# prannaykaul/lvc

Measured on AMD Instinct MI355X. Metric: img/s COCO 800x1333 R50-FPN inference (GeneralizedRCNN.forward(batched_inputs) -> Instances, 1000 proposals, 100 detections), higher is better.
Workload: dtype f32 (conv/GEMM inner products on the fp16 / bf16 matrix cores through fp32-accurate operand splits: two-way fp16 with main + cross fp32 accumulators for the 3x3 and wide 1x1 / FC layers, three-way bf16 for the rest; final boxes/scores closer to the fp64 evaluation than the reference's fp32 CPU path,; 1 GPU; COCO-detection R50-FPN inference, bs=8 synthetic 3x800x1333 per GPU, 1000 pre/post-NMS proposals per level/image, 80 classes, conditioned random-init weights; batch_per_gpu=8, global_batch=8, parallelism=dp1

## Files before the change

### include/lvc_amd.h

```cpp
#ifndef LVC_AMD_H
#define LVC_AMD_H

#ifdef __cplusplus
extern "C" {
#endif

#define LVC_OK 0
#define LVC_ERR_INVALID 1
#define LVC_ERR_HIP 2

int lvc_abi_version(void);
const char* lvc_last_error(void);
void lvc_set_error(const char* fmt, ...);

long long lvc_conv_workspace_bytes(void);
long long lvc_conv_range_words_offset(void);
void lvc_set_range_slot(int slot);
int lvc_range_slot(void);
int lvc_range_slots(void);
int lvc_conv2d_nhwc_f32(const float* x, const float* w_packed, const float* scale, const float* shift,
                        const float* residual, float* y, int N, int H, int W, int C, int K, int R, int S,
                        int stride, int pad, int Kg, int relu, int res_mode, int ldy, int ldr, int mode,
                        void* workspace, void* stream);

// ... 40 lines not shown
int lvc_conv1x1_nhwc_f16x2_pipe(const float* x, const unsigned short* w_split, const float* scale, const float* shift,
                                const float* residual, float* y, int N, int H, int W, int C, int K, int stride, int relu,
                                int res_mode, int ldy, int ldr, void* workspace, void* stream);
int lvc_conv1x1_nhwc_f16s1(const float* x, const unsigned short* w_split, const float* scale, const float* shift,
                           const float* residual, float* y, int N, int H, int W, int C, int K, int stride, int relu,
                           int res_mode, int ldy, int ldr, void* workspace, void* stream);
int lvc_conv3x3_nhwc_f16s1_presplit(const float* x, const unsigned short* w_split, const float* scale, const float* shift, void* y,
                                    int N, int H, int W, int C, int K, int Kg, int next_slot, void* workspace, void* stream);
int lvc_conv1x1_nhwc_f16s1_presplit(const void* x, const unsigned short* w_split, const float* scale, const float* shift,
                                    const float* residual, float* y, int N, int H, int W, int C, int K, int relu,
                                    int res_mode, int ldy, int ldr, void* workspace, void* stream);
int lvc_conv1x1_nhwc_f16s1_w2(const float* x, const unsigned short* w_split, const float* scale, const float* shift,
                              const float* residual, float* y, int N, int H, int W, int C, int K, int Kpad, int stride, int relu,
                              int res_mode, int ldy, int ldr, void* workspace, void* stream);
int lvc_conv1x1_chain_nhwc_f16s1(const float* x, int ldx, const unsigned short* wa, int wa_rows, const float* sa, const float* ta,
                                 const float* residual, int ldr, float* y1, int ldy1, int relu1, const unsigned short* wb,
                                 int wb_rows, const float* sb, const float* tb, float* y2, int ldy2, int relu2, int M, int K1,
                                 int N1, int N2, void* workspace, void* stream);
int lvc_bottleneck_nhwc_f16s1(const float* x, int ldx, float* y, int ldy, int N, int H, int W, int cin, int proj,
                              const unsigned short* w, const float* s1, const float* t1, const float* s2, const float* t2,
                              const float* s3, const float* t3, void* workspace, void* stream);
int lvc_split_weights_rowscaled(const float* wp, int rows, int Kg, void* planes_out, float* row_factor, void* stream);

int lvc_conv2d_nhwc_f16x2(const float* x, const unsigned short* w_split, const float* scale, const float* shift,
                          const float* residual, float* y, int N, int H, int W, int C, int K, int R, int S,
                          int stride, int pad, int Kg, int relu, int res_mode, int ldy, int ldr, void* workspace,
                          void* stream);
int lvc_conv2d_nhwc_f16x2_dma(const float* x, const unsigned short* w_split, const float* scale, const float* shift,
                          const float* residual, float* y, int N, int H, int W, int C, int K, int R, int S,
                          int stride, int pad, int Kg, int relu, int res_mode, int ldy, int ldr, void* workspace,
                          void* stream);

int lvc_stem_conv_pool_nhwc4_f16x2(const float* x, const unsigned short* w_split, const float* scale, const float* shift,
                                   float* y, int N, int H, int W, int Kpad, int relu, int* d_error_word,
                                   float* y2 , int ldy2, void* stream);

int lvc_preprocess_nhwc4(const void* image, int dtype, int h, int w, const float* mean3, const float* std3,
                         float* out, int Hp, int Wp, void* stream);
int lvc_preprocess_batch_nhwc4(const void* const* images, int dtype, const int* hs, const int* ws, int B, const float* mean3,
                               const float* std3, float* out, int Hp, int Wp, void* stream);

int lvc_resize_bilinear_u8(const unsigned char* image, int H, int W, int new_h, int new_w, const int* xb, const int* xk,
                           int kxs, const int* yb, const int* yk, int kys, unsigned char* tmp, unsigned char* out_u8,
                           float* out_nhwc4, int Hp, int Wp, const float* mean3, const float* std3, void* stream);
int lvc_tta_resize_u8(const unsigned char* image, int H, int W, long long sy, long long sx, long long sc, const long long* hjobs,
                      int n_h, const long long* vjobs, int n_v, const float* mean3, const float* std3, void* stream);
long long lvc_tta_merge_workspace_bytes(int B, int Nmax);
int lvc_tta_merge(const float* boxes, const float* scores, const int* classes, const int* counts, int topk_in, const float* params,
                  const int* tab, int B, int Nmax, float score_thresh, double nms_thresh, int topk_out, float* ob, float* osc, int* ocl,
                  int* ocount, void* workspace, long long workspace_bytes, void* stream);
int lvc_train_input_u8(const void* h_blob, const void* d_blob, long long blob_bytes, int B, unsigned char* tmp, long long tmp_bytes,
                       float* out, int n_slots, int Hp, int Wp, const float* mean3, const float* std3, int* launches, void* stream);
int lvc_train_input_tiles_u8(const void* h_blob, const void* d_blob, long long blob_bytes, int B, unsigned char* tmp,
                             long long tmp_bytes, float* out, int n_slots, int Hp, int Wp, const float* mean3, const float* std3,
                             int* launches, void* stream);
int lvc_train_input_lsj_u8(const void* h_blob, const void* d_blob, long long blob_bytes, int B, unsigned char* tmp,
                           long long tmp_bytes, float* out, int n_slots, int Hp, int Wp, const float* mean3, const float* std3,
                           int* launches, void* stream);
int lvc_color_jitter_tiles_u8(const void* h_blob, void* d_blob, long long blob_bytes, int B, unsigned char* out, long long out_bytes,
                              int* launches, void* stream);
int lvc_maxpool2d_nhwc(const float* x, float* y, int N, int H, int W, int C, int k, int stride, int pad,
                       void* stream);

int lvc_crop_resize_nearest(const float* image_chw, int C, int H, int W, const int* d_windows, int K, int out_size,
                            float* out, void* stream);

int lvc_rownorm(const float* x, const float* mu, float* y, int M, int D, int ldx, int ldy, float eps, int mode,
                void* stream);
int lvc_rownorm_backward(const float* x, const float* dy, float* dx, int M, int D, float eps, int accumulate, void* stream);

int lvc_roi_align_forward_nchw(const float* input, const float* rois, float* output, int B, int C, int H, int W,
                               int K, int pooled_h, int pooled_w, float spatial_scale, int sampling_ratio,
                               int aligned, int* d_status, void* stream);
int lvc_roi_align_fpn_nhwc(const float* const* feats, const int* Hs, const int* Ws, const float* scales, int L,
                           int B, int C, const float* rois, const int* levels, const int* d_num_valid, int K,
                           int pooled_h, int pooled_w, int sampling_ratio, int aligned, float* output,
                           int* d_status, void* stream);
int lvc_roi_work_order(const float* rois, const int* levels, const float* scales, int L, int K, int pooled_h, int* d_order,
                       void* stream);
int lvc_roi_work_order_xcd(const float* rois, const int* levels, int K, int B, int* d_order, void* stream);
int lvc_roi_align_fpn_nhwc_ordered(const float* const* feats, const int* Hs, const int* Ws, const float* scales, int L,
                                   int B, int C, const float* rois, const int* levels, const int* d_num_valid, int K,
                                   int pooled_h, int pooled_w, int sampling_ratio, int aligned, float* output,
                                   int* d_status, const int* d_order, void* stream);

int lvc_roi_align_backward_nchw(const float* grad, const float* rois, float* grad_input, int B, int C, int H, int W,
                                int K, int pooled_h, int pooled_w, float spatial_scale, int sampling_ratio,
                                int aligned, int* d_status, void* stream);
int lvc_roi_align_fpn_backward_nhwc(const float* grad, float* const* grad_feats, const int* Hs, const int* Ws,
                                    const float* scales, int L, int B, int C, const float* rois, const int* levels,
                                    const int* d_num_valid, int K, int pooled_h, int pooled_w, int sampling_ratio,
                                    int aligned, int* d_status, void* stream);
int lvc_roi_align_route(int backward, int nhwc, int C, int pooled_h, int pooled_w, int has_num_valid,
                        long long largest_level_elems);

long long lvc_batched_nms_workspace_bytes(int B, int Nmax);
int lvc_batched_nms(const float* boxes, const float* scores, const int* idxs, const int* d_counts, int B,
                    int Nmax, double iou_threshold, int max_keep, int* keep, int* d_num_keep, void* workspace,
                    long long workspace_bytes, void* stream);

long long lvc_rpn_proposals_workspace_bytes(int B, int L, int A, const int* Hs, const int* Ws, int pre_nms_topk);
int lvc_rpn_proposals(const float* const* logits, const int* ld_logit, const float* const* deltas,
                      const int* ld_delta, const float* const* cell_anchors, const int* Hs, const int* Ws,
                      const int* strides, int L, int A, int B, const int* d_image_sizes, int pre_nms_topk,
                      int post_nms_topk, double nms_thresh, float min_box_size, float scale_clamp,
                      float* out_boxes, float* out_logits, int* d_out_count, void* workspace,
                      long long workspace_bytes, void* stream);

long long lvc_retinanet_select_workspace_bytes(int B, int L, int A, int K, const int* Hs, const int* Ws, int topk,
                                               int max_survivors);
int lvc_retinanet_select(const float* const* logits, const int* ld_logit, const float* const* deltas, const int* ld_delta,
                         const float* const* cell_anchors, const int* Hs, const int* Ws, const int* strides,
                         float anchor_offset, int L, int A, int K, int B, int topk, float score_thresh, float wx, float wy,
                         float ww, float wh, float scale_clamp, int max_survivors, float* out_boxes, float* out_scores,
                         int* out_classes, int* out_index, int* d_count, int* d_status, void* workspace,
                         long long workspace_bytes, void* stream);

int lvc_gather_detections(const float* boxes, const float* scores, const int* classes, const int* rows, const int* keep,
                          const int* d_num_keep, int B, int Nmax, int topk, const float* d_post, float* out_boxes,
                          float* out_scores, int* out_classes, int* out_rows, int* d_out_count, void* stream);

long long lvc_retinanet_loss_workspace_bytes(int B, int L, int A, int K, const int* Hs, const int* Ws);
int lvc_retinanet_loss(const float* const* logits, const int* ld_logit, const float* const* deltas, const int* ld_delta,
                       const int* Hs, const int* Ws, int L, int A, int K, int B, const float* anchors, const int* matches,
                       const signed char* labels, const float* gt, const long long* gt_classes, const int* gt_off, double alpha,
                       double gamma, double beta, double wx, double wy, double ww, double wh, double momentum,
                       double one_minus_momentum, const double* normalizer_in, double* normalizer_out, float* out_losses,
                       double* out_sums , int* num_pos, void* workspace, long long workspace_bytes, void* stream);
int lvc_retinanet_loss_grad(const float* const* logits, const int* ld_logit, const float* const* deltas, const int* ld_delta,
                            const int* Hs, const int* Ws, int L, int A, int K, int B, const float* anchors, const int* matches,
                            const signed char* labels, const float* gt, const long long* gt_classes, const int* gt_off, double alpha,
                            double gamma, double beta, double wx, double wy, double ww, double wh, const double* normalizer,
                            const float* g_cls, const float* g_box, float* const* dlogits, const int* ld_dlogit,
                            float* const* ddeltas, const int* ld_ddelta, void* stream);

int lvc_assign_levels_rois(const float* boxes, int B, int R, int min_level, int max_level, int canonical_box_size,
                           int canonical_level, int* levels, float* rois, void* stream);

long long lvc_fast_rcnn_inference_workspace_bytes(int B, int max_candidates);
int lvc_fast_rcnn_inference(const float* cls_logits, int ld_cls, const float* deltas, int ld_delta, int K,
                            int cls_agnostic, const float* proposals, const int* d_prop_count, int B, int R,
                            const int* d_image_sizes, float wx, float wy, float ww, float wh, float scale_clamp,
                            float score_thresh, double nms_thresh, int topk, int max_candidates,
                            const float* d_post, float* out_boxes, float* out_scores, int* out_classes,
                            int* out_rows, int* d_out_count, int* d_status, void* workspace,
                            long long workspace_bytes, void* stream);

int lvc_decode_boxes(const float* deltas, int ld, const float* boxes, int M, int R, const int* d_image_sizes,
                     float wx, float wy, float ww, float wh, float scale_clamp, float* out, void* stream);

int lvc_match_boxes(const float* gt, int G, const float* boxes, int N, float t0, float t1, int nthr, int l0, int l1,
                    int l2, int allow_low_quality, long long* matches, signed char* labels, float* matched_vals,
                    unsigned int* d_gt_best, void* stream);
int lvc_match_boxes_batched(const float* gt, const int* gt_off, int Gtot, int B, const float* boxes, long long box_img_stride,
                            const int* nbox, int N, float t0, float t1, int nthr, int l0, int l1, int l2, int allow_low_quality,
                            int* matches, signed char* labels, float* vals, unsigned int* gt_best, void* stream);
long long lvc_subsample_workspace_bytes(int B);
int lvc_subsample_batched(const signed char* labels, const long long* keys , unsigned long long seed,
                          int B, int N, int nbits, int cap_pos, int bs, int* sel, int* counts, void* workspace, void* stream);
int lvc_rpn_gather_sampled(const void* const* fused, const int* ld, const void* const* cell_anchors, const int* H, const int* W,
                           const int* strides, int L, int A, int B, int bs, const int* sel, const int* counts, const int* matches,
                           const float* gt, const int* gt_off, float* logits, float* deltas, float* anchors, float* gt_boxes,
                           signed char* labels, void* stream);
int lvc_roi_build_table(const float* pboxes, const float* plogits, const int* pcount, int B, int P, const float* gt, const int* gt_off,
                        float gt_logit, int Wt, float* boxes, float* logits, int* nrow, void* stream);
int lvc_roi_gather_sampled(const float* boxes, const float* logits, const int* matches, const int* sel, const int* counts,
                           const long long* gt_classes, const int* gt_off, int B, int Wt, int bs, int K, float* s_boxes, float* s_logits,
                           long long* s_cls, long long* s_match, void* stream);
int lvc_fast_rcnn_losses(const float* logits, int ld_cls, const float* deltas, int ld_delta, int K, int cls_agnostic,
                         const float* proposals, const float* gt_boxes, const long long* gt_classes, int R, float wx,
                         float wy, float ww, float wh, float smooth_l1_beta, float* out_losses, float* dlogits,
                         float* ddeltas, double* row_terms , void* stream);
int lvc_rpn_losses(const float* logits, const float* deltas, const float* anchors, const float* gt_boxes,
                   const signed char* labels, int S, float smooth_l1_beta, float normalizer, float* out_losses,
                   void* stream);
int lvc_rpn_losses_grad(const float* logits, const float* deltas, const float* anchors, const float* gt_boxes,
                        const signed char* labels, int S, float smooth_l1_beta, float normalizer, float* out_losses,
                        float* dlogits, float* ddeltas, void* stream);

int lvc_giou_box_loss(const float* deltas, int ld_delta, const float* proposals, const float* gt_boxes,
                      const long long* gt_classes, int R, int K, float wx, float wy, float ww, float wh,
                      float scale_clamp, int iterate, float lambda, float* out_loss, float* ddeltas, void* stream);
int lvc_relu_backward(const float* dy, const float* y, long long n, float* out, void* stream);
int lvc_colsum(const float* x, int M, int N, int ldx, float* out, void* stream);

int lvc_pack_conv_weights(const float* w, const float* scale, float* wp, int K, int C, int R, int S, int rows_pad,
                          int cin_pad, int mode, void* stream);
int lvc_split_weights(const float* wp, long long n, int planes, void* out, int* err_word, void* stream);
int lvc_pack_split_conv_weights(const float* w, const float* scale, float* wp, void* planes_out, int planes, int* err_word,
                                int K, int C, int R, int S, int rows_pad, int cin_pad, int mode, void* stream);
int lvc_pack_group(int njobs, const void* const* ptrs, const int* shapes, int* err_word, void* stream);
int lvc_conv_wgrad_nhwc(const float* x, const float* dy, const float* scale, float* dw, int N, int H, int W, int C,
                        int K, int R, int S, int stride, int pad, int lddy, void* stream);
int lvc_conv_wgrad_nhwc_bf16x3(const float* x, const float* dy, const float* scale, float* dw, int N, int H, int W, int C,
                               int K, int R, int S, int stride, int pad, int lddy, void* stream);
int lvc_conv_wgrad_nhwc_f16x2(const float* x, const float* dy, const float* scale, float* dw, int N, int H, int W, int C,
                              int K, int R, int S, int stride, int pad, int lddy, int* err_word, void* stream);
int lvc_conv_wgrad_group_bf16x3(int njobs, const float* const* x, const float* const* dy, const float* const* scale,
                                float* const* dw, const int* shapes, void* stream);
int lvc_wgrad_finalize_group(int njobs, const float* const* src, float* const* dst, const int* shapes, void* stream);
int lvc_scatter_stride2_nhwc(const float* x, float* y, int N, int H, int W, int C, void* stream);
int lvc_conv3x3_grouped_nhwc(const float* x, const float* wp, const float* scale, const float* shift, const float* residual,
                             float* y, int N, int H, int W, int C, int K, int groups, int stride, int relu, int res_mode, int ldy,
                             int ldr, void* workspace, void* stream);
long long lvc_conv3x3_grouped_packed_floats(int K, int groups);
int lvc_pack_conv3x3_grouped(const float* w, const float* scale, float* wp, int K, int groups, int mode, void* stream);
long long lvc_conv3x3_grouped_wgrad_workspace_bytes(int N, int H, int W, int K, int groups, int stride);
int lvc_conv3x3_grouped_wgrad_nhwc(const float* x, const float* dy, const float* scale, float* dw, int N, int H, int W, int C,
                                   int groups, int stride, int lddy, void* scratch, void* stream);
int lvc_subsample2_nhwc(const float* x, float* y, int N, int H, int W, int C, int ldy, void* stream);
int lvc_downsum2x2_nhwc(const float* x, float* y, int N, int Hs, int Ws, int C, void* stream);
int lvc_avgpool2_nhwc(const float* x, float* y, int N, int H, int W, int C, int ldo, void* stream);
int lvc_avgpool2_bwd_nhwc(const float* dy, float* dx, int N, int H, int W, int C, int ldi, void* stream);
int lvc_colsum_atomic(const float* x, int M, int N, int ldx, float* out, void* stream);

int lvc_colmean(const float* x, float* mu, int M, int D, int ld, void* stream);
int lvc_knn_topk_candidates(const float* sims, int ld, int Q, int S, int idx_base, float* cand_val, int* cand_idx, void* stream);
int lvc_knn_merge_vote(const float* cand_val, const int* cand_idx, int nlists, int Q, const long long* shot_classes,
                       const long long* det_classes, int kvote, long long* top_classes, long long* keep, void* stream);
int lvc_max_f32(const float* x, long long n, float* out, void* stream);
int lvc_knn_topk_vote(const float* sims, int ld, int Q, int S, const long long* shot_classes,
                      const long long* det_classes, int kvote, long long* top_classes, long long* keep,
                      void* stream);
int lvc_rownorm_h(const float* x, const float* mu, float* y, unsigned short* yh, float* den, float* resid, int M, int D, int ldx,
                  float eps, int mode, void* stream);
int lvc_gemm_f16(const unsigned short* a, const unsigned short* b, int ldb, float* y, int M, int N, int C, int ldy,
                 void* stream);
int lvc_knn_verify_topk_vote(const float* approx, int ld, int Q, int S, const float* q, int ldq, const float* mu,
                             const float* den, const float* sn, int D, float margin, const float* margins,
// ... 87 lines not shown
```

### lvc_amd/csrc/boxes.hip

```cpp
#include "common.h"
#include "select_common.h"
#include <stdlib.h>


#define MAXL 8


__device__ __forceinline__ int block_excl_scan_1024(int v, int* sh, int* total) {
  const int lane = threadIdx.x & 63, wave = threadIdx.x >> 6;
  int x = v;
#pragma unroll
  for (int o = 1; o < 64; o <<= 1) {
    int t = __shfl_up(x, o);
    if (lane >= o) x += t;
  }
  __syncthreads();
  if (lane == 63) sh[wave] = x;
  __syncthreads();
  if (threadIdx.x == 0) {
    int s = 0;
    for (int w = 0; w < 16; ++w) { int t = sh[w]; sh[w] = s; s += t; }
    sh[16] = s;
  }
  __syncthreads();
  *total = sh[16];
  return sh[wave] + x - v;
}


struct RpnLevels {
  const float* logits[MAXL];
  const float* deltas[MAXL];
  int ld_logit[MAXL], ld_delta[MAXL];
  int H[MAXL], W[MAXL], stride[MAXL];
  int cand_off[MAXL + 1];
  long long key_off[MAXL + 1];
  const float* cell_anchors[MAXL];
  int L, A;
};


#define TOPK_PAD 2048
__global__ __launch_bounds__(1024) void rpn_topk_kernel(RpnLevels lv, int topk, unsigned int* __restrict__ wkeys,
                                                        float* __restrict__ cand_score,
                                                        int* __restrict__ cand_idx, int Ntot, int small_only) {
  __shared__ u64 sortbuf[TOPK_PAD];
  __shared__ int hist[256];
  __shared__ int sh[20];
  __shared__ int s_nlt;
  const int l = blockIdx.x, b = blockIdx.y, tid = threadIdx.x;
  const int A = lv.A, HW = lv.H[l] * lv.W[l], n = HW * A;
  if (n > small_only) return;
  const int k = topk < n ? topk : n;
  const int ld = lv.ld_logit[l];
  const float* lg = lv.logits[l] + (size_t)b * HW * ld;
  unsigned int* keys = wkeys + (size_t)b * lv.key_off[lv.L] + lv.key_off[l];
  const int npad = k <= 1024 ? 1024 : TOPK_PAD;

  if (tid < 256) hist[tid] = 0;
  __syncthreads();
  for (int i = tid; i < n; i += 1024) {
    int p = i / A, a = i - p * A;
    unsigned int key = desc_key(lg[(size_t)p * ld + a]);
    keys[i] = key;
    atomicAdd(&hist[key >> 24], 1);
  }
  __syncthreads();
  unsigned int prefix = 0, pmask = 0;
  int krem = k;
  for (int pass = 0; pass < 4; ++pass) {
    const int shift = 24 - 8 * pass;
    if (pass > 0) {
      if (tid < 256) hist[tid] = 0;
      __syncthreads();
      for (int i = tid; i < n; i += 1024) {
        unsigned int key = keys[i];
        if ((key & pmask) == prefix) atomicAdd(&hist[(key >> shift) & 255], 1);
      }
      __syncthreads();
    }
    find_digit(hist, krem, sh);
    prefix |= (unsigned int)sh[8] << shift;
    pmask |= 255u << shift;
    krem -= sh[9];
// ... 550 lines not shown
  LVC_CHECK_ARG(L >= 1 && L <= MAXL, "1..8 levels");
  LVC_CHECK_ARG(B > 0 && A > 0, "bad B/A");
  LVC_CHECK_ARG(pre_nms_topk > 0 && pre_nms_topk <= TOPK_PAD, "pre_nms_topk must be in 1..2048");
  LVC_CHECK_ARG(post_nms_topk > 0, "post_nms_topk must be positive");
  LVC_CHECK_ARG(logits && deltas && cell_anchors && Hs && Ws && strides && d_image_sizes && out_boxes &&
                    out_logits && d_out_count && workspace, "null pointer");
  RpnPlan p = rpn_plan(B, L, A, Hs, Ws, pre_nms_topk);
  LVC_CHECK_ARG(workspace_bytes >= p.total, "workspace too small");
  RpnLevels lv;
  memset(&lv, 0, sizeof lv);
  lv.L = L; lv.A = A;
  for (int l = 0; l < L; ++l) {
    lv.logits[l] = logits[l]; lv.deltas[l] = deltas[l];
    lv.ld_logit[l] = ld_logit[l]; lv.ld_delta[l] = ld_delta[l];
    lv.H[l] = Hs[l]; lv.W[l] = Ws[l]; lv.stride[l] = strides[l];
    lv.cell_anchors[l] = cell_anchors[l];
    long long n = (long long)Hs[l] * Ws[l] * A;
    lv.key_off[l + 1] = lv.key_off[l] + n;
    lv.cand_off[l + 1] = lv.cand_off[l] + (int)(n < pre_nms_topk ? n : pre_nms_topk);
  }
  char* ws = (char*)workspace;
  hipStream_t st = (hipStream_t)stream;
  unsigned int* keys = (unsigned int*)(ws + p.off_keys);
  float* cand_score = (float*)(ws + p.off_cscore);
  int* cand_idx = (int*)(ws + p.off_cidx);
  const bool multi = p.max_slices > 0;
  const int sel = lvc_select_onelaunch();
  if ((sel & 1) && (sel & 4)) {
    hipLaunchKernelGGL(rpn_topk_one_kernel, dim3(L, B), dim3(1024), 0, st, lv, pre_nms_topk, keys, cand_score, cand_idx,
                       p.Ntot, (const int*)nullptr);
  } else if (sel & 1) {
    int* hist12 = (int*)(ws + p.off_hist12);
    if (hipMemsetAsync(hist12, 0, (size_t)B * L * 4096 * 4, st) != hipSuccess) {
      lvc_set_error("%s: hipMemsetAsync failed", __func__);
      return LVC_ERR_HIP;
    }
    if (p.all_slices > 0)
      hipLaunchKernelGGL(rpn_topk_keys_kernel, dim3(p.all_slices, L, B), dim3(1024), 0, st, lv, keys, hist12);
    hipLaunchKernelGGL(rpn_topk_one_kernel, dim3(L, B), dim3(1024), 0, st, lv, pre_nms_topk, keys, cand_score, cand_idx,
                       p.Ntot, (const int*)hist12);
  } else {
  if (multi) {
    int* hist = (int*)(ws + p.off_hist);
    u64* ckeys = (u64*)(ws + p.off_ckeys);
    int* ties = (int*)(ws + p.off_ties);
    if (hipMemsetAsync(hist, 0, (size_t)B * L * TK_HSTRIDE * 4, st) != hipSuccess) {
      lvc_set_error("%s: hipMemsetAsync failed", __func__);
      return LVC_ERR_HIP;
    }
    for (int phase = 0; phase <= 4; ++phase)
      hipLaunchKernelGGL(rpn_topk_phase_kernel, dim3(p.max_slices, L, B), dim3(1024), 0, st, lv, pre_nms_topk, keys,
                         hist, ckeys, ties, p.Ntot, phase);
    hipLaunchKernelGGL(rpn_topk_final_kernel, dim3(L, B), dim3(1024), 0, st, lv, pre_nms_topk, keys, hist, ckeys, ties,
                       cand_score, cand_idx, p.Ntot);
  }
  hipLaunchKernelGGL(rpn_topk_kernel, dim3(L, B), dim3(1024), 0, st, lv, pre_nms_topk, keys, cand_score,
                     cand_idx, p.Ntot, multi ? TK_SLICE : 0x7FFFFFFF);
  }
  LVC_CHECK_LAUNCH();
  float* sboxes = (float*)(ws + p.off_sboxes);
  float* sscores = (float*)(ws + p.off_sscores);
  int* scount = (int*)(ws + p.off_scount);
  int* skeep = (int*)(ws + p.off_skeep);
  int* snk = (int*)(ws + p.off_snk);
  hipLaunchKernelGGL(rpn_decode_seg_kernel, dim3(L, B), dim3(1024), 0, st, lv, cand_score, cand_idx, p.Ntot,
                     d_image_sizes, scale_clamp, min_box_size, p.SN, sboxes, sscores, scount);
  LVC_CHECK_LAUNCH();
  const int keep_per_level = post_nms_topk < p.SN ? post_nms_topk : p.SN;
  int rc = lvc_batched_nms(sboxes, sscores, nullptr, scount, B * L, p.SN, nms_thresh, keep_per_level, skeep, snk,
                           ws + p.off_snms, p.snms_bytes, stream);
  if (rc) return rc;
  hipLaunchKernelGGL(rpn_merge_levels_kernel, dim3(B), dim3(1024), 0, st, sboxes, sscores, skeep, snk, L, p.SN,
                     post_nms_topk, out_boxes, out_logits, d_out_count);
  LVC_CHECK_LAUNCH();
  return LVC_OK;
}

__global__ void assign_levels_kernel(const float* __restrict__ boxes, int R, int B, int min_level, int max_level,
                                     float canonical_box_size, float canonical_level, int* __restrict__ levels,
                                     float* __restrict__ rois) {
  const int i = blockIdx.x * blockDim.x + threadIdx.x;
  if (i >= R * B) return;
  const float4 bx = *reinterpret_cast<const float4*>(boxes + (size_t)i * 4);
  const float area = (bx.z - bx.x) * (bx.w - bx.y);
  const float size = sqrtf(area);
  float lvl = floorf(canonical_level + log2f(size / canonical_box_size + 1e-8f));
  lvl = lvl < (float)min_level ? (float)min_level : lvl;
  lvl = lvl > (float)max_level ? (float)max_level : lvl;
  levels[i] = (int)lvl - min_level;
  if (rois) {
    float* r = rois + (size_t)i * 5;
    r[0] = (float)(i / R); r[1] = bx.x; r[2] = bx.y; r[3] = bx.z; r[4] = bx.w;
  }
}

extern "C" int lvc_assign_levels_rois(const float* boxes, int B, int R, int min_level, int max_level,
                                      int canonical_box_size, int canonical_level, int* levels, float* rois,
                                      void* stream) {
  LVC_CHECK_ARG(B >= 0 && R >= 0, "negative size");
  if (B * R == 0) return LVC_OK;
  LVC_CHECK_ARG(boxes && levels, "null pointer");
  hipLaunchKernelGGL(assign_levels_kernel, dim3(lvc_cdiv(B * R, 256)), dim3(256), 0, (hipStream_t)stream, boxes, R,
                     B, min_level, max_level, (float)canonical_box_size, (float)canonical_level, levels, rois);
  LVC_CHECK_LAUNCH();
  return LVC_OK;
}

#define DET_TILE_ROWS 64
#define DET_MAX_COLS 97
__global__ __launch_bounds__(DET_TILE_ROWS) void det_row_stats_kernel(const float* __restrict__ cls_logits, int ld_cls, int K,
                                                                     int rows, float score_thresh, float* __restrict__ st_mx,
                                                                     float* __restrict__ st_inv, int* __restrict__ st_cnt,
                                                                     unsigned long long* __restrict__ st_mask) {
  __shared__ float tile[DET_TILE_ROWS * DET_MAX_COLS];
  const int r0 = blockIdx.x * DET_TILE_ROWS, tid = threadIdx.x;
  const int ncol = K + 1, pitch = ncol | 1;
  for (int i = tid; i < DET_TILE_ROWS * ncol; i += DET_TILE_ROWS) {
    const int rr = i / ncol, cc = i - rr * ncol;
    const int r = r0 + rr;
    tile[rr * pitch + cc] = r < rows ? cls_logits[(size_t)r * ld_cls + cc] : 0.f;
  }
  __syncthreads();
  const int r = r0 + tid;
  if (r >= rows) return;
  const float* lg = tile + tid * pitch;
  float mx = -INFINITY;
  for (int k = 0; k <= K; ++k) { float v = lg[k]; mx = v > mx ? v : mx; }
  float sum = 0.f;
  for (int k = 0; k <= K; ++k) sum += expf(lg[k] - mx);
  const float inv = 1.f / sum;
  int cnt = 0;
  unsigned long long m0 = 0, m1 = 0;
  for (int k = 0; k < K; ++k) {
    const bool hit = expf(lg[k] - mx) * inv > score_thresh;
    cnt += hit ? 1 : 0;
    if (hit) { if (k < 64) m0 |= 1ull << k; else m1 |= 1ull << (k - 64); }
  }
  st_mx[r] = mx; st_inv[r] = inv; st_cnt[r] = cnt;
  st_mask[2 * (size_t)r] = m0; st_mask[2 * (size_t)r + 1] = m1;
}

__global__ __launch_bounds__(1024) void det_candidates_kernel(
    const float* __restrict__ cls_logits, int ld_cls, const float* __restrict__ deltas, int ld_delta,
    int K, int cls_agnostic, const float* __restrict__ proposals, const int* __restrict__ prop_count, int R,
    const int* __restrict__ image_sizes, float wx, float wy, float ww, float wh, float scale_clamp,
    float score_thresh, int Nmax, float* __restrict__ cboxes, float* __restrict__ cscores,
    int* __restrict__ cclass, int* __restrict__ crow, int* __restrict__ ccount, int* __restrict__ status,
    const float* __restrict__ st_mx, const float* __restrict__ st_inv, const int* __restrict__ st_cnt,
    const unsigned long long* __restrict__ st_mask) {
  __shared__ int sh[20];
  const int b = blockIdx.x, tid = threadIdx.x;
  const int nrow = prop_count ? min(prop_count[b], R) : R;
  const float img_h = (float)image_sizes[b * 2 + 0], img_w = (float)image_sizes[b * 2 + 1];
  int base = 0;
  for (int r0 = 0; r0 < nrow; r0 += 1024) {
    const int r = r0 + tid;
    int cnt = 0;
    float mx = -INFINITY, inv = 0.f;
    const float* lg = cls_logits + ((size_t)b * R + (r < nrow ? r : 0)) * ld_cls;
    if (r < nrow && st_cnt) {
      const size_t gr = (size_t)b * R + r;
      mx = st_mx[gr]; inv = st_inv[gr]; cnt = st_cnt[gr];
    } else if (r < nrow) {
      for (int k = 0; k <= K; ++k) { float v = lg[k]; mx = v > mx ? v : mx; }
      float sum = 0.f;
      for (int k = 0; k <= K; ++k) sum += expf(lg[k] - mx);
      inv = 1.f / sum;
      for (int k = 0; k < K; ++k) cnt += (expf(lg[k] - mx) * inv > score_thresh) ? 1 : 0;
    }
    int tot;
    int pos = base + block_excl_scan_1024(cnt, sh, &tot);
    if (r < nrow && cnt > 0) {
      const float4 pb = *reinterpret_cast<const float4*>(proposals + ((size_t)b * R + r) * 4);
      const float* dl = deltas + ((size_t)b * R + r) * ld_delta;
      auto emit = [&](int k) {
        const float pr = expf(lg[k] - mx) * inv;
        if (pr > score_thresh) {
          if (pos < Nmax) {
            const float* d = dl + (cls_agnostic ? 0 : k * 4);
            float box[4];
            apply_deltas(pb.x, pb.y, pb.z, pb.w, d[0], d[1], d[2], d[3], wx, wy, ww, wh, scale_clamp, box);
            float* o = cboxes + ((size_t)b * Nmax + pos) * 4;
            o[0] = clampf(box[0], 0.f, img_w); o[1] = clampf(box[1], 0.f, img_h);
            o[2] = clampf(box[2], 0.f, img_w); o[3] = clampf(box[3], 0.f, img_h);
            cscores[(size_t)b * Nmax + pos] = pr;
            cclass[(size_t)b * Nmax + pos] = k;
            crow[(size_t)b * Nmax + pos] = r;
          }
          ++pos;
        }
      };
      if (st_mask) {
        for (int w = 0; w < 2; ++w) {
          unsigned long long m = st_mask[2 * ((size_t)b * R + r) + w];
          while (m) {
            emit(w * 64 + __ffsll((long long)m) - 1);
            m &= m - 1;
          }
        }
      } else {
        for (int k = 0; k < K; ++k) emit(k);
      }
    }
    base += tot;
  }
  if (tid == 0) {
    if (base > Nmax) { atomicOr(status, 2); base = Nmax; }
    ccount[b] = base;
  }
}

__global__ __launch_bounds__(256) void det_gather_kernel(
    const float* __restrict__ cboxes, const float* __restrict__ cscores, const int* __restrict__ cclass,
    const int* __restrict__ crow, const int* __restrict__ keep, const int* __restrict__ num_keep, int Nmax,
    int topk, const float* __restrict__ post, float* __restrict__ oboxes, float* __restrict__ oscores,
    int* __restrict__ oclasses, int* __restrict__ orows, int* __restrict__ ocount) {
  __shared__ int wsum[4];
  const int b = blockIdx.x, tid = threadIdx.x;
  const int nk = min(num_keep[b], topk);
  int base = 0;
  for (int r0 = 0; r0 < topk; r0 += 256) {
    const int r = r0 + tid;
    bool ok = false;
    float4 bx = {0, 0, 0, 0};
    float s = 0.f; int c = 0, row = 0;
    if (r < nk) {
      const int i = keep[(size_t)b * Nmax + r];
      bx = *reinterpret_cast<const float4*>(cboxes + ((size_t)b * Nmax + i) * 4);
      s = cscores[(size_t)b * Nmax + i]; c = cclass[(size_t)b * Nmax + i]; row = crow[(size_t)b * Nmax + i];
      ok = true;
      if (post) {
        const float sx = post[b * 4 + 0], sy = post[b * 4 + 1], oh = post[b * 4 + 2], ow = post[b * 4 + 3];
        bx.x = clampf(bx.x * sx, 0.f, ow); bx.y = clampf(bx.y * sy, 0.f, oh);
        bx.z = clampf(bx.z * sx, 0.f, ow); bx.w = clampf(bx.w * sy, 0.f, oh);
        ok = (bx.z - bx.x > 0.f) && (bx.w - bx.y > 0.f);
      }
    }
    const u64 bal = __ballot(ok);
    const int lane = tid & 63, wave = tid >> 6;
    __syncthreads();
    if (lane == 0) wsum[wave] = __popcll(bal);
    __syncthreads();
    int wbase = 0, tot = 0;
    for (int w = 0; w < 4; ++w) { if (w < wave) wbase += wsum[w]; tot += wsum[w]; }
    const int pos = base + wbase + __popcll(bal & ((1ull << lane) - 1ull));
    if (ok) {
      *reinterpret_cast<float4*>(oboxes + ((size_t)b * topk + pos) * 4) = bx;
      oscores[(size_t)b * topk + pos] = s; oclasses[(size_t)b * topk + pos] = c; orows[(size_t)b * topk + pos] = row;
    }
    base += tot;
  }
  __syncthreads();
  for (int r = base + tid; r < topk; r += 256) {
    float4 z = {0, 0, 0, 0};
    *reinterpret_cast<float4*>(oboxes + ((size_t)b * topk + r) * 4) = z;
    oscores[(size_t)b * topk + r] = 0.f; oclasses[(size_t)b * topk + r] = 0; orows[(size_t)b * topk + r] = 0;
  }
  if (tid == 0) ocount[b] = base;
}

struct DetPlan { long long off_cboxes, off_cscores, off_cclass, off_crow, off_ccount, off_keep, off_nk, off_nms, total; };
static DetPlan det_plan(int B, int Nmax) {
  DetPlan p; long long o = 0;
  p.off_cboxes = o; o = align16(o + (long long)B * Nmax * 16);
  p.off_cscores = o; o = align16(o + (long long)B * Nmax * 4);
  p.off_cclass = o; o = align16(o + (long long)B * Nmax * 4);
  p.off_crow = o; o = align16(o + (long long)B * Nmax * 4);
  p.off_ccount = o; o = align16(o + (long long)B * 4);
  p.off_keep = o; o = align16(o + (long long)B * Nmax * 4);
  p.off_nk = o; o = align16(o + (long long)B * 4);
  p.off_nms = o; o = align16(o + lvc_batched_nms_workspace_bytes(B, Nmax));
  p.total = o;
  return p;
}
extern "C" long long lvc_fast_rcnn_inference_workspace_bytes(int B, int max_candidates) {
  return det_plan(B, max_candidates).total;
}

extern "C" int lvc_fast_rcnn_inference(const float* cls_logits, int ld_cls, const float* deltas, int ld_delta,
                                       int K, int cls_agnostic, const float* proposals,
                                       const int* d_prop_count, int B, int R, const int* d_image_sizes,
                                       float wx, float wy, float ww, float wh, float scale_clamp,
                                       float score_thresh, double nms_thresh, int topk, int max_candidates,
                                       const float* d_post, float* out_boxes, float* out_scores,
                                       int* out_classes, int* out_rows, int* d_out_count, int* d_status,
                                       void* workspace, long long workspace_bytes, void* stream) {
  LVC_CHECK_ARG(B > 0 && R > 0 && K > 0 && topk > 0, "bad sizes");
  LVC_CHECK_ARG(max_candidates > 0, "max_candidates must be positive");
  LVC_CHECK_ARG(cls_logits && deltas && proposals && d_image_sizes && out_boxes && out_scores && out_classes &&
                    out_rows && d_out_count && d_status && workspace, "null pointer");
  DetPlan p = det_plan(B, max_candidates);
  LVC_CHECK_ARG(workspace_bytes >= p.total, "workspace too small");
  char* ws = (char*)workspace;
  hipStream_t st = (hipStream_t)stream;
  float* cboxes = (float*)(ws + p.off_cboxes);
  float* cscores = (float*)(ws + p.off_cscores);
  int* cclass = (int*)(ws + p.off_cclass);
  int* crow = (int*)(ws + p.off_crow);
  int* ccount = (int*)(ws + p.off_ccount);
  int* keep = (int*)(ws + p.off_keep);
  int* nk = (int*)(ws + p.off_nk);
  const long long rows = (long long)B * R;
  float* st_mx = nullptr; float* st_inv = nullptr; int* st_cnt = nullptr;
  unsigned long long* st_mask = nullptr;
  if (K + 1 < DET_MAX_COLS && rows * 28 + 64 <= p.total - p.off_nms) {
    st_mask = (unsigned long long*)(ws + p.off_nms);
    st_mx = (float*)(st_mask + 2 * rows);
    st_inv = st_mx + rows;
    st_cnt = (int*)(st_inv + rows);
    hipLaunchKernelGGL(det_row_stats_kernel, dim3((unsigned)lvc_cdiv64(rows, DET_TILE_ROWS)), dim3(DET_TILE_ROWS), 0, st,
                       cls_logits, ld_cls, K, (int)rows, score_thresh, st_mx, st_inv, st_cnt, st_mask);
    LVC_CHECK_LAUNCH();
  }
  hipLaunchKernelGGL(det_candidates_kernel, dim3(B), dim3(1024), 0, st, cls_logits, ld_cls, deltas, ld_delta, K,
                     cls_agnostic, proposals, d_prop_count, R, d_image_sizes, wx, wy, ww, wh, scale_clamp,
                     score_thresh, max_candidates, cboxes, cscores, cclass, crow, ccount, d_status, st_mx, st_inv, st_cnt, st_mask);
  LVC_CHECK_LAUNCH();
  int rc = lvc_batched_nms(cboxes, cscores, cclass, ccount, B, max_candidates, nms_thresh, topk, keep, nk,
                           ws + p.off_nms, p.total - p.off_nms, stream);
  if (rc) return rc;
  hipLaunchKernelGGL(det_gather_kernel, dim3(B), dim3(256), 0, st, cboxes, cscores, cclass, crow, keep, nk,
                     max_candidates, topk, d_post, out_boxes, out_scores, out_classes, out_rows, d_out_count);
  LVC_CHECK_LAUNCH();
  return LVC_OK;
}

extern "C" int lvc_gather_detections(const float* boxes, const float* scores, const int* classes, const int* rows,
                                     const int* keep, const int* d_num_keep, int B, int Nmax, int topk, const float* d_post,
                                     float* out_boxes, float* out_scores, int* out_classes, int* out_rows, int* d_out_count,
                                     void* stream) {
  LVC_CHECK_ARG(B > 0 && Nmax > 0 && topk > 0, "bad B / Nmax / topk");
  LVC_CHECK_ARG(boxes && scores && classes && rows && keep && d_num_keep && out_boxes && out_scores && out_classes && out_rows &&
                    d_out_count, "null pointer");
  LVC_CHECK_ARG(((uintptr_t)boxes & 15) == 0 && ((uintptr_t)out_boxes & 15) == 0, "box pointers must be 16-byte aligned");
  hipLaunchKernelGGL(det_gather_kernel, dim3(B), dim3(256), 0, (hipStream_t)stream, boxes, scores, classes, rows, keep,
                     d_num_keep, Nmax, topk, d_post, out_boxes, out_scores, out_classes, out_rows, d_out_count);
  LVC_CHECK_LAUNCH();
  return LVC_OK;
}

__global__ void decode_boxes_kernel(const float* __restrict__ deltas, int ld, const float* __restrict__ boxes, int M,
                                    int R, const int* __restrict__ image_sizes, float wx, float wy, float ww, float wh,
                                    float scale_clamp, float* __restrict__ out) {
  const int i = blockIdx.x * blockDim.x + threadIdx.x;
  if (i >= M) return;
  const float4 b = *reinterpret_cast<const float4*>(boxes + (size_t)i * 4);
  const float* d = deltas + (size_t)i * ld;
  float o[4];
  apply_deltas(b.x, b.y, b.z, b.w, d[0], d[1], d[2], d[3], wx, wy, ww, wh, scale_clamp, o);
  if (image_sizes) {
    const int img = i / R;
    const float h = (float)image_sizes[img * 2], w = (float)image_sizes[img * 2 + 1];
    o[0] = clampf(o[0], 0.f, w); o[1] = clampf(o[1], 0.f, h); o[2] = clampf(o[2], 0.f, w); o[3] = clampf(o[3], 0.f, h);
  }
  float4 r = {o[0], o[1], o[2], o[3]};
  *reinterpret_cast<float4*>(out + (size_t)i * 4) = r;
}

extern "C" int lvc_decode_boxes(const float* deltas, int ld, const float* boxes, int M, int R, const int* d_image_sizes,
                                float wx, float wy, float ww, float wh, float scale_clamp, float* out, void* stream) {
  LVC_CHECK_ARG(M >= 0 && R > 0 && ld >= 4, "bad shape");
  if (M == 0) return LVC_OK;
  LVC_CHECK_ARG(deltas && boxes && out, "null pointer");
  hipLaunchKernelGGL(decode_boxes_kernel, dim3(lvc_cdiv(M, 256)), dim3(256), 0, (hipStream_t)stream, deltas, ld, boxes, M, R,
                     d_image_sizes, wx, wy, ww, wh, scale_clamp, out);
  LVC_CHECK_LAUNCH();
  return LVC_OK;
}
```

### lvc_amd/csrc/conv_common.h

```cpp
#pragma once
#include "common.h"

typedef float f32x16 __attribute__((ext_vector_type(16)));
typedef float f32x4 __attribute__((ext_vector_type(4)));
typedef _Float16 f16;
typedef _Float16 f16x8 __attribute__((ext_vector_type(8)));
typedef _Float16 f16x4 __attribute__((ext_vector_type(4)));
typedef __bf16 bf16x8 __attribute__((ext_vector_type(8)));
typedef __bf16 bf16x4 __attribute__((ext_vector_type(4)));
typedef unsigned u32x4 __attribute__((ext_vector_type(4)));
typedef __attribute__((address_space(3))) void* lds_ptr_t;
typedef const __attribute__((address_space(1))) void* glb_ptr_t;

#define LVC_MAX_WORKERS 1024
#define LVC_RANGE_SLOTS 1024
#define LVC_WS_PARTIAL_BYTES (256 * 128 * 4)
#define LVC_WS_FLAGS_OFFSET ((size_t)LVC_MAX_WORKERS * LVC_WS_PARTIAL_BYTES)
#define LVC_WS_RANGE_OFFSET (LVC_WS_FLAGS_OFFSET + (size_t)LVC_MAX_WORKERS * 4)
#define LVC_WS_BYTES (LVC_WS_RANGE_OFFSET + (size_t)LVC_RANGE_SLOTS * 4 + 256)
#define LVC_WS_DIAG_OFFSET ((size_t)(LVC_MAX_WORKERS / 2) * LVC_WS_PARTIAL_BYTES)
static inline int* lvc_ws_flags(void* workspace) { return (int*)((char*)workspace + LVC_WS_FLAGS_OFFSET); }
static inline int lvc_ws_range_index(int slot) { return LVC_MAX_WORKERS + slot; }

extern "C" int lvc_cu_count(void);

static inline void lvc_plan_workers(long long units, int cap, int min_units, int* units_per_worker, int* nworkers) {
  long long workers = (units + min_units - 1) / min_units;
  if (workers > cap) workers = cap;
  if (workers < 1) workers = 1;
  *units_per_worker = (int)((units + workers - 1) / workers);
  *nworkers = (int)((units + *units_per_worker - 1) / *units_per_worker);
}

#define LVC_ACT_SCALE 16.f
#define LVC_ACT_MAX 4094.f
#define LVC_F16_MAX 65504.f
#define lvc_report_range(flags, index, big, limit)                                             \
  do {                                                                                         \
    if (!((big) <= (limit))) atomicOr((flags) + (index), (big) < INFINITY ? 2 : 4);            \
  } while (0)

#define LVC_SPIN_LIMIT (1 << 24)
__device__ __forceinline__ void lvc_publish_partial(int* flags, int worker) {
  __builtin_amdgcn_fence(__ATOMIC_RELEASE, "agent");
  asm volatile("s_waitcnt vmcnt(0)" ::: "memory");
  __hip_atomic_store(flags + worker, 1, __ATOMIC_RELAXED, __HIP_MEMORY_SCOPE_AGENT);
}
__device__ __forceinline__ void lvc_wait_partial(int* flags, int worker, int err_index) {
  int spins = 0;
  while (__hip_atomic_load(flags + worker, __ATOMIC_RELAXED, __HIP_MEMORY_SCOPE_AGENT) == 0) {
    __builtin_amdgcn_s_sleep(4);
    if (++spins > LVC_SPIN_LIMIT) { atomicOr(flags + err_index, 1); break; }
  }
  __builtin_amdgcn_fence(__ATOMIC_ACQUIRE, "agent");
}
__device__ __forceinline__ void lvc_release_partial(int* flags, int worker) {
  __hip_atomic_store(flags + worker, 0, __ATOMIC_RELAXED, __HIP_MEMORY_SCOPE_AGENT);
}

__device__ __forceinline__ void glds16(const void* g, void* l) {
  __builtin_amdgcn_global_load_lds((glb_ptr_t)g, (lds_ptr_t)l, 16, 0, 0);
}
template <int N> __device__ __forceinline__ void wait_vm() { asm volatile("s_waitcnt vmcnt(%0)" ::"n"(N) : "memory"); }
template <int N> __device__ __forceinline__ void wait_vm_lds() { asm volatile("s_waitcnt vmcnt(%0) lgkmcnt(0)" ::"n"(N) : "memory"); }

__device__ __forceinline__ f32x4 load_untracked(u32x4 rsrc, unsigned voff, unsigned soff) {
  f32x4 v;
  asm volatile("buffer_load_dwordx4 %0, %1, %2, %3 offen" : "=v"(v) : "v"(voff), "s"(rsrc), "s"(soff) : "memory");
  return v;
}
template <int IMM> __device__ __forceinline__ f32x4 load_untracked(u32x4 rsrc, unsigned voff, unsigned soff) {
  f32x4 v;
  asm volatile("buffer_load_dwordx4 %0, %1, %2, %3 offen offset:%4" : "=v"(v) : "v"(voff), "s"(rsrc), "s"(soff), "n"(IMM) : "memory");
  return v;
}
template <int N> __device__ __forceinline__ void wait_tied(f32x4& a, f32x4& b) {
  asm volatile("s_waitcnt vmcnt(%2)" : "+v"(a), "+v"(b) : "n"(N) : "memory");
}
template <int N> __device__ __forceinline__ void wait_tied(f32x4& a, f32x4& b, f32x4& c, f32x4& d) {
  asm volatile("s_waitcnt vmcnt(%4)" : "+v"(a), "+v"(b), "+v"(c), "+v"(d) : "n"(N) : "memory");
}
__device__ __forceinline__ u32x4 make_rsrc(const void* base, unsigned bytes) {
  const unsigned long long b = (unsigned long long)base;
  return u32x4{(unsigned)__builtin_amdgcn_readfirstlane((unsigned)b), (unsigned)__builtin_amdgcn_readfirstlane((unsigned)(b >> 32) & 0xffffu),
               (unsigned)__builtin_amdgcn_readfirstlane(bytes), 0x00020000u};
}
__device__ __forceinline__ void store_b128(f32x4 v, __amdgpu_buffer_rsrc_t rsrc, unsigned voff) {
  __builtin_amdgcn_raw_buffer_store_b128(__builtin_bit_cast(u32x4, v), rsrc, voff, 0, 0);
}
__device__ __forceinline__ void track_abs(float& big, float a, float b) {
  asm volatile("v_max3_f32 %0, %0, |%1|, |%2|" : "+v"(big) : "v"(a), "v"(b));
}
__device__ __forceinline__ void split2h(float a, f16& h, f16& m) {
  h = (f16)a;
  m = (f16)((a - (float)h) * 2048.f);
}
```

### lvc_amd/csrc/conv_pw_s1.hip

```cpp
#include "conv_common.h"
#include <type_traits>
#include <stdlib.h>

#define PM 256
#define AROW 64
#define NJ 4
#define NT 512

struct PwArgsS {
  const float* x;
  const unsigned short* w;
  const float* scale;
  const float* shift;
  const float* res;
  float* y;
  float* partials;
  int* flags;
  int H, W, C, K, stride, Ho, Wo, M, relu, res_mode, ldy, ldr;
  int tiles_n, nk, total_units, units_per_worker, nworkers, err_index, ngroup;
  int x_bytes;
  long long w_plane_elems;
  unsigned short* planes;
  int* pl_err;
  long long pl_PS;
  int pl_N, pl_Npad, pl_H;
  float pl_qscale;
};

template <int NI, bool ONEACC, bool PLANES = false, bool PRE = false>
__global__ __launch_bounds__(NT, 2) void conv_pw_s1_kernel(PwArgsS p) {
  constexpr int HN = 64 * NI;
  constexpr int PLANE_A = PM * AROW;
  constexpr int A_BUF = 2 * PLANE_A;
  constexpr int A_BYTES = 3 * A_BUF;
  constexpr int PLANE_B = HN * 64;
  constexpr int B_BUF = 2 * PLANE_B;
  constexpr int RING_BYTES = A_BYTES + 3 * B_BUF;
  constexpr int CS_STRIDE = HN + 4;
  constexpr int CS_BYTES = PM * CS_STRIDE * 4;
  constexpr int SMEM_BYTES = RING_BYTES > CS_BYTES ? RING_BYTES : CS_BYTES;
  constexpr int RBLK = HN / 16;
  __shared__ __attribute__((aligned(1024))) unsigned char smem_raw[SMEM_BYTES];
  unsigned char* sA = smem_raw;
  unsigned char* sB = smem_raw + A_BYTES;

  const int tid = threadIdx.x;
  const int lane = tid & 63;
  const int wave = __builtin_amdgcn_readfirstlane(tid >> 6);
  const int wm = wave >> 1, wn = wave & 1;
  const int fi = lane & 31, fh = lane >> 5;
  const int q = PRE ? ((tid >> 4) & 1) * 4 + (tid & 3) : tid & 7;
  const int arid = PRE ? (tid >> 5) * 4 + ((tid >> 2) & 3) : tid >> 3;
  const int hrow = arid;

  const int lw = lvc_xcd_remap(blockIdx.x, p.nworkers);
  const int wq = p.ngroup > 1 ? lw / p.ngroup : lw;
  const int wsel = p.ngroup > 1 ? lw - wq * p.ngroup : 0;
  int u = wq * p.units_per_worker;
  const int u_end = min(u + p.units_per_worker, p.total_units);

  const unsigned long long xbase = (unsigned long long)p.x;
  const u32x4 xres = {(unsigned)__builtin_amdgcn_readfirstlane((unsigned)xbase), (unsigned)__builtin_amdgcn_readfirstlane((unsigned)(xbase >> 32) & 0xffffu),
                      (unsigned)p.x_bytes, 0x00020000u};
  const int fx3 = (fi >> 2) & 3;
  const int a_row[2] = {(wm * 64 + fi) * AROW, (wm * 64 + 32 + fi) * AROW};
  const int b_row = (wn * 32 * NI + fi) * 64;
  const int b_g[2] = {((0 + fh) ^ fx3) * 16, ((2 + fh) ^ fx3) * 16};
  int a_lds[NJ];
#pragma unroll
  for (int j = 0; j < NJ; ++j) {
    const int row = hrow + 64 * j;
    a_lds[j] = row * AROW + (((q >> 1) ^ ((row >> 2) & 3)) << 4) + (q & 1) * 8;
  }
  float big = 0.f;
  int a_pre[NJ];
#pragma unroll
  for (int j = 0; j < NJ; ++j) {
    const int row = hrow + 64 * j;
    a_pre[j] = (q >> 2) * (PM * AROW) + row * AROW + (((q & 3) ^ ((row >> 2) & 3)) << 4);
  }
#ifdef PW_TIMELINE
  unsigned long long tl_pro = 0, tl_loop = 0, tl_hand = 0, tl_cs = 0, tl_rows = 0, tl_t0 = __builtin_readcyclecounter();
  unsigned long long tl_wa = 0, tl_wv = 0, tl_wb = 0;
  unsigned tl_tiles = 0, tl_chunks = 0;
#endif

  while (u < u_end) {
#ifdef PW_TIMELINE
    const unsigned long long tl_a = __builtin_readcyclecounter();
#endif
    const int tile = u / p.nk;
    const int cc0 = u - tile * p.nk;
    const int cc1 = min(p.nk, cc0 + (u_end - u));
    const int tile_n = p.ngroup > 1 ? wsel : tile % p.tiles_n;
    const int tile_m = p.ngroup > 1 ? tile : tile / p.tiles_n;
    const int m0 = tile_m * PM;
    const int n0 = tile_n * HN;

    unsigned a_off[NJ];
#pragma unroll
    for (int j = 0; j < NJ; ++j) {
      const int m = m0 + hrow + 64 * j;
      const int n = m / (p.Ho * p.Wo);
      const int rem = m - n * (p.Ho * p.Wo);
      const int ho = rem / p.Wo, wo = rem - ho * p.Wo;
      a_off[j] = m < p.M ? (unsigned)(((n * p.H + ho * p.stride) * p.W + wo * p.stride) * p.C + q * 4) * 4u : 0x80000000u;
    }
    const unsigned short* bsrc[NI];
    int bdst[NI];
#pragma unroll
    for (int j = 0; j < NI; ++j) {
      const int idx = wave * NI + j;
// ... 357 lines not shown
      constexpr int C4 = HN / 4;
      constexpr int RPI = NT / C4;
      constexpr int NIT = PM / RPI;
      constexpr int NG = 4;
      const int c4 = tid % C4, rsub = tid / C4;
      const int col = n0 + c4 * 4;
      const bool col_ok = col < p.K;
      const bool has_res = p.res_mode != 0 && col_ok;
      auto res_load = [&](int it) {
        const int m = m0 + it * RPI + rsub;
        f32x4 v = {0.f, 0.f, 0.f, 0.f};
        if (m < p.M) {
          size_t ro = (size_t)m;
          if (p.res_mode == 2) {
            const int n = m / (p.Ho * p.Wo);
            const int rem = m - n * (p.Ho * p.Wo);
            const int ho = rem / p.Wo, wo = rem - ho * p.Wo;
            ro = ((size_t)(n * (p.Ho >> 1) + (ho >> 1)) * (p.Wo >> 1) + (wo >> 1));
          }
          v = *reinterpret_cast<const f32x4*>(p.res + ro * p.ldr + col);
        }
        return v;
      };
      f32x4 rv[NG];
#pragma unroll
      for (int i = 0; i < NG; ++i) rv[i] = f32x4{0.f, 0.f, 0.f, 0.f};
      if (has_res) {
#pragma unroll
        for (int i = 0; i < NG; ++i) rv[i] = res_load(i);
      }
      float* Cs = reinterpret_cast<float*>(smem_raw);
#pragma unroll
      for (int mi = 0; mi < 2; ++mi)
#pragma unroll
        for (int ni = 0; ni < NI; ++ni)
#pragma unroll
          for (int e = 0; e < 16; ++e) {
            const int row = wm * 64 + mi * 32 + (e & 3) + 8 * (e >> 2) + 4 * fh;
            const int colc = wn * 32 * NI + ni * 32 + fi;
            Cs[row * CS_STRIDE + colc] = acc[mi][ni][e];
          }
      __syncthreads();
#ifdef PW_TIMELINE
      tl_e = __builtin_readcyclecounter();
      tl_cs += tl_e - tl_d;
#endif
      if (col_ok) {
        f32x4 sc = {1.f, 1.f, 1.f, 1.f}, sh = {0.f, 0.f, 0.f, 0.f};
        if (p.scale) sc = *reinterpret_cast<const f32x4*>(p.scale + col);
        if (p.shift) sh = *reinterpret_cast<const f32x4*>(p.shift + col);
        const float* cs = Cs + rsub * CS_STRIDE + c4 * 4;
        float* const yb = p.y + (size_t)(m0 + rsub) * p.ldy + col;
        auto rows = [&](auto res_tag, auto act_tag) {
          constexpr bool RES = decltype(res_tag)::value;
          constexpr int ACT = decltype(act_tag)::value;
#pragma unroll 1
          for (int g = 0; g < NIT; g += NG) {
            f32x4 rn[NG];
            if (RES) {
#pragma unroll
              for (int i = 0; i < NG; ++i) rn[i] = f32x4{0.f, 0.f, 0.f, 0.f};
              if (g + NG < NIT) {
#pragma unroll
                for (int i = 0; i < NG; ++i) rn[i] = res_load(g + NG + i);
              }
            }
            f32x4 v[NG];
#pragma unroll
            for (int i = 0; i < NG; ++i) v[i] = *reinterpret_cast<const f32x4*>(cs + (g + i) * RPI * CS_STRIDE);
#pragma unroll
            for (int i = 0; i < NG; ++i) {
              const int m = m0 + (g + i) * RPI + rsub;
              if (m < p.M) {
                f32x4 o = v[i] * sc + sh;
                if (RES) o += rv[i];
                if (ACT == 1) {
                  o[0] = o[0] > 0.f ? o[0] : 0.f; o[1] = o[1] > 0.f ? o[1] : 0.f;
                  o[2] = o[2] > 0.f ? o[2] : 0.f; o[3] = o[3] > 0.f ? o[3] : 0.f;
                } else if (ACT == 2) {
#pragma unroll
                  for (int e = 0; e < 4; ++e) o[e] = o[e] * 0.5f * (1.f + erff(o[e] * 0.70710678118654752440f));
                }
                *reinterpret_cast<f32x4*>(yb + (size_t)((g + i) * RPI) * p.ldy) = o;
              }
            }
            if (RES) {
#pragma unroll
              for (int i = 0; i < NG; ++i) rv[i] = rn[i];
            }
          }
        };
        using A0 = std::integral_constant<int, 0>; using A1 = std::integral_constant<int, 1>; using A2 = std::integral_constant<int, 2>;
        if (has_res) {
          if (p.relu == 1) rows(std::true_type{}, A1{}); else if (p.relu == 2) rows(std::true_type{}, A2{}); else rows(std::true_type{}, A0{});
        } else {
          if (p.relu == 1) rows(std::false_type{}, A1{}); else if (p.relu == 2) rows(std::false_type{}, A2{}); else rows(std::false_type{}, A0{});
        }
      }
    }
    __syncthreads();
#ifdef PW_TIMELINE
    tl_rows += __builtin_readcyclecounter() - tl_e;
#endif
  }
#ifdef PW_TIMELINE
  if (lane == 0 && (blockIdx.x & 15) == 0) {
    unsigned long long* d = reinterpret_cast<unsigned long long*>(reinterpret_cast<char*>(p.partials) + LVC_WS_DIAG_OFFSET) + ((blockIdx.x >> 4) * 8 + wave) * 16;
    d[0] = tl_pro; d[1] = tl_loop; d[2] = tl_hand; d[3] = tl_cs; d[4] = tl_rows; d[5] = tl_tiles; d[6] = tl_chunks; d[7] = __builtin_readcyclecounter() - tl_t0; d[8] = 1; d[9] = tl_wa; d[10] = tl_wv; d[11] = tl_wb;
  }
#endif
  if (PRE) return;
  lvc_report_range(p.flags, p.err_index, big, ONEACC ? LVC_ACT_MAX : LVC_F16_MAX);
}

struct PwPlanes { unsigned short* planes; int* err; long long PS; int N, Npad, H; float qscale; };

static int pw_s1_launch(bool oneacc, const float* x, const unsigned short* w_split, const float* scale, const float* shift,
                        const float* residual, float* y, int N, int H, int W, int C, int K, int stride, int relu, int res_mode,
                        int ldy, int ldr, void* workspace, void* stream, const PwPlanes* pl = nullptr, bool pre = false) {
  LVC_CHECK_ARG(x && w_split && y && workspace, "null pointer");
  LVC_CHECK_ARG(!oneacc || scale, "the single-accumulator form needs the row factors in `scale`");
  LVC_CHECK_ARG(N > 0 && H > 0 && W > 0 && C > 0 && K > 0 && stride >= 1, "non-positive dimension");
  LVC_CHECK_ARG(C % 32 == 0, "needs C % 32 == 0");
  LVC_CHECK_ARG(relu >= 0 && relu <= 2, "relu: 0 none, 1 ReLU, 2 GELU");
  LVC_CHECK_ARG(res_mode >= 0 && res_mode <= 2 && (res_mode == 0 || residual), "bad residual");
  const int Ho = (H - 1) / stride + 1, Wo = (W - 1) / stride + 1;
  if (res_mode == 2) LVC_CHECK_ARG(Ho % 2 == 0 && Wo % 2 == 0, "upsample-add needs even output size");
  PwArgsS a;
  a.x = x; a.w = w_split; a.scale = scale; a.shift = shift; a.res = residual; a.y = y;
  a.H = H; a.W = W; a.C = C; a.K = K; a.stride = stride; a.Ho = Ho; a.Wo = Wo;
  const long long Mll = (long long)N * Ho * Wo;
  LVC_CHECK_ARG(Mll < (1ll << 31), "too many output pixels");
  a.M = (int)Mll; a.relu = relu; a.res_mode = res_mode;
  a.ldy = ldy > 0 ? ldy : K; a.ldr = ldr > 0 ? ldr : K;
  LVC_CHECK_ARG((K & 3) == 0 && (a.ldy & 3) == 0 && (res_mode == 0 || (a.ldr & 3) == 0), "K, ldy, ldr must be multiples of 4");
  LVC_CHECK_ARG(((uintptr_t)x & 15) == 0 && ((uintptr_t)w_split & 15) == 0 && ((uintptr_t)y & 15) == 0 && ((uintptr_t)workspace & 15) == 0 &&
                    ((uintptr_t)scale & 15) == 0 && ((uintptr_t)shift & 15) == 0 && ((uintptr_t)residual & 15) == 0,
                "pointers must be 16-byte aligned");
  const long long xb = (long long)N * H * W * C * 4;
  LVC_CHECK_ARG(xb < (1ll << 31), "input tensor must be smaller than 2 GiB");
  a.x_bytes = (int)xb;
  const int ni = K <= 64 ? 1 : 2;
  const int HN = 64 * ni;
  a.tiles_n = lvc_cdiv(K, HN);
  a.nk = C / 32;
  const int tiles_m = lvc_cdiv(a.M, PM);
  long long units = (long long)tiles_m * a.tiles_n * a.nk;
  LVC_CHECK_ARG(units < (1ll << 31), "iteration space too large");
  a.total_units = (int)units;
  a.w_plane_elems = (long long)(lvc_cdiv(K, 128) * 128) * C;
  int cap = lvc_cu_count();
  if (cap > LVC_MAX_WORKERS) cap = LVC_MAX_WORKERS;
  a.ngroup = 1;
  if ((a.tiles_n == 2 || a.tiles_n == 4 || a.tiles_n == 8 || a.tiles_n == 16) && cap % a.tiles_n == 0 && units / a.tiles_n >= (long long)(cap / a.tiles_n) * 4) {
    a.ngroup = a.tiles_n;
    units /= a.tiles_n;
    cap /= a.tiles_n;
    a.total_units = (int)units;
  }
  const int min_units = 4;
  lvc_plan_workers(units, cap, min_units, &a.units_per_worker, &a.nworkers);
  a.nworkers *= a.ngroup;
  a.partials = (float*)workspace;
  a.flags = lvc_ws_flags(workspace);
  a.err_index = lvc_ws_range_index(lvc_range_slot());
  hipStream_t st = (hipStream_t)stream;
  a.planes = nullptr; a.pl_err = nullptr; a.pl_PS = 0; a.pl_N = a.pl_Npad = a.pl_H = 0; a.pl_qscale = 1.f;
  if (pl) {
    LVC_CHECK_ARG(oneacc && ni == 2 && res_mode == 0 && relu == 0, "the planes epilogue exists for the single-accumulator 128-column tile");
    a.planes = pl->planes; a.pl_err = pl->err; a.pl_PS = pl->PS; a.pl_N = pl->N; a.pl_Npad = pl->Npad; a.pl_H = pl->H; a.pl_qscale = pl->qscale;
    hipLaunchKernelGGL((conv_pw_s1_kernel<2, true, true>), dim3(a.nworkers), dim3(NT), 0, st, a);
    LVC_CHECK_LAUNCH();
    return LVC_OK;
  }
  if (pre) {
    LVC_CHECK_ARG(oneacc && ni == 2 && stride == 1, "pre-split input: the single-accumulator 128-column tile, stride 1");
    hipLaunchKernelGGL((conv_pw_s1_kernel<2, true, false, true>), dim3(a.nworkers), dim3(NT), 0, st, a);
    LVC_CHECK_LAUNCH();
    return LVC_OK;
  }
  if (oneacc) {
    if (ni == 1) hipLaunchKernelGGL((conv_pw_s1_kernel<1, true>), dim3(a.nworkers), dim3(NT), 0, st, a);
    else hipLaunchKernelGGL((conv_pw_s1_kernel<2, true>), dim3(a.nworkers), dim3(NT), 0, st, a);
  } else {
    if (ni == 1) hipLaunchKernelGGL((conv_pw_s1_kernel<1, false>), dim3(a.nworkers), dim3(NT), 0, st, a);
    else hipLaunchKernelGGL((conv_pw_s1_kernel<2, false>), dim3(a.nworkers), dim3(NT), 0, st, a);
  }
  LVC_CHECK_LAUNCH();
  return LVC_OK;
}

extern "C" int lvc_conv1x1_nhwc_f16x2_pipe(const float* x, const unsigned short* w_split, const float* scale, const float* shift,
                                            const float* residual, float* y, int N, int H, int W, int C, int K, int stride, int relu,
                                            int res_mode, int ldy, int ldr, void* workspace, void* stream) {
  return pw_s1_launch(false, x, w_split, scale, shift, residual, y, N, H, W, C, K, stride, relu, res_mode, ldy, ldr, workspace, stream);
}

extern "C" int lvc_conv1x1_nhwc_f16s1(const float* x, const unsigned short* w_split, const float* scale, const float* shift,
                                       const float* residual, float* y, int N, int H, int W, int C, int K, int stride, int relu,
                                       int res_mode, int ldy, int ldr, void* workspace, void* stream) {
  return pw_s1_launch(true, x, w_split, scale, shift, residual, y, N, H, W, C, K, stride, relu, res_mode, ldy, ldr, workspace, stream);
}

extern "C" int lvc_conv1x1_nhwc_f16s1_presplit(const void* x, const unsigned short* w_split, const float* scale, const float* shift,
                                                const float* residual, float* y, int N, int H, int W, int C, int K, int relu,
                                                int res_mode, int ldy, int ldr, void* workspace, void* stream) {
  return pw_s1_launch(true, (const float*)x, w_split, scale, shift, residual, y, N, H, W, C, K, 1, relu, res_mode, ldy, ldr, workspace, stream, nullptr, true);
}

extern "C" int lvc_conv1x1_qkv_planes_f16s1(const float* x, const unsigned short* w_split, const float* scale, const float* shift, void* planes,
                                            int B, int N, int C, int H, float softmax_scale, int* err_word, void* workspace, void* stream) {
  LVC_CHECK_ARG(planes && B > 0 && N > 0 && H > 0, "bad arguments");
  const int Npad = (N + 127) / 128 * 128;
  PwPlanes pl;
  pl.planes = (unsigned short*)planes; pl.err = err_word; pl.N = N; pl.Npad = Npad; pl.H = H; pl.qscale = softmax_scale * 1.44269504088896340736f;
  pl.PS = (long long)B * H * Npad * 64;
  return pw_s1_launch(true, x, w_split, scale, shift, nullptr, (float*)planes, B * N, 1, 1, C, 3 * H * 64, 1, 0, 0, 0, 0, workspace, stream, &pl);
}
```

### lvc_amd/csrc/roi_align.hip

```cpp
#include "common.h"
#include <stdlib.h>
#include <type_traits>

#define LVC_MAX_LEVELS 8

struct RoiAlignArgs {
  const float* feat[LVC_MAX_LEVELS];
  int H[LVC_MAX_LEVELS], W[LVC_MAX_LEVELS];
  float scale[LVC_MAX_LEVELS];
  long long sb[LVC_MAX_LEVELS];
  long long sc, sh_mul_w;
  int nhwc;
  int C;
  const float* rois;
  const int* levels;
  const int* num_valid;
  int K, ph, pw, sampling_ratio, aligned;
  float* out;
  long long so_k, so_c, so_h, so_w;
  int* status;
  const int* order;
};

__global__ __launch_bounds__(256) void roi_align_fwd_kernel(RoiAlignArgs p) {
  const int k = blockIdx.x;
  const int c = blockIdx.y * 256 + threadIdx.x;
  const bool c_ok = c < p.C;
  float* outk = p.out + (long long)k * p.so_k + (long long)c * p.so_c;
  if (p.num_valid && k >= *p.num_valid) {
    if (c_ok)
      for (int a = 0; a < p.ph; ++a)
        for (int b = 0; b < p.pw; ++b) outk[a * p.so_h + b * p.so_w] = 0.f;
    return;
  }
  const float* r = p.rois + (long long)k * 5;
  const int lvl = p.levels ? p.levels[k] : 0;
  const int H = p.H[lvl], W = p.W[lvl];
  const float spatial_scale = p.scale[lvl];
  const int b = (int)r[0];
  const float offset = p.aligned ? 0.5f : 0.0f;
  const float roi_start_w = r[1] * spatial_scale - offset;
  const float roi_start_h = r[2] * spatial_scale - offset;
  const float roi_end_w = r[3] * spatial_scale - offset;
  const float roi_end_h = r[4] * spatial_scale - offset;
  float roi_width = roi_end_w - roi_start_w;
  float roi_height = roi_end_h - roi_start_h;
  if (p.aligned) {
    if (!(roi_width >= 0 && roi_height >= 0)) {
      if (p.status && threadIdx.x == 0 && blockIdx.y == 0) atomicOr(p.status, 1);
    }
  } else {
    roi_width = roi_width > 1.f ? roi_width : 1.f;
    roi_height = roi_height > 1.f ? roi_height : 1.f;
  }
  const float bin_h = roi_height / (float)p.ph;
  const float bin_w = roi_width / (float)p.pw;
  const int gh = p.sampling_ratio > 0 ? p.sampling_ratio : (int)ceilf(roi_height / (float)p.ph);
  const int gw = p.sampling_ratio > 0 ? p.sampling_ratio : (int)ceilf(roi_width / (float)p.pw);
  const int cnt = gh * gw > 1 ? gh * gw : 1;
  const float count = (float)cnt;

  long long s_pix, s_c;
  if (p.nhwc) { s_pix = p.C; s_c = 1; } else { s_pix = 1; s_c = (long long)H * W; }
  const float* in = p.feat[lvl] + (long long)b * p.sb[lvl] + (long long)(c_ok ? c : 0) * s_c;

  for (int ph = 0; ph < p.ph; ++ph) {
    for (int pw = 0; pw < p.pw; ++pw) {
      float acc = 0.f;
      for (int iy = 0; iy < gh; ++iy) {
        const float yy = roi_start_h + ph * bin_h + (float)(iy + .5f) * bin_h / (float)gh;
        for (int ix = 0; ix < gw; ++ix) {
          const float xx = roi_start_w + pw * bin_w + (float)(ix + .5f) * bin_w / (float)gw;
          float x = xx, y = yy;
          if (y < -1.0f || y > (float)H || x < -1.0f || x > (float)W) continue;
          if (y <= 0) y = 0;
          if (x <= 0) x = 0;
          int y_low = (int)y, x_low = (int)x, y_high, x_high;
          if (y_low >= H - 1) { y_high = y_low = H - 1; y = (float)y_low; } else y_high = y_low + 1;
          if (x_low >= W - 1) { x_high = x_low = W - 1; x = (float)x_low; } else x_high = x_low + 1;
          const float ly = y - y_low, lx = x - x_low;
          const float hy = 1.f - ly, hx = 1.f - lx;
          const float w1 = hy * hx, w2 = hy * lx, w3 = ly * hx, w4 = ly * lx;
          const float v1 = in[(long long)(y_low * W + x_low) * s_pix];
          const float v2 = in[(long long)(y_low * W + x_high) * s_pix];
          const float v3 = in[(long long)(y_high * W + x_low) * s_pix];
          const float v4 = in[(long long)(y_high * W + x_high) * s_pix];
          acc += w1 * v1 + w2 * v2 + w3 * v3 + w4 * v4;
        }
      }
      if (c_ok) outk[ph * p.so_h + pw * p.so_w] = acc / count;
    }
  }
}

__global__ __launch_bounds__(64) void roi_align_fwd_nhwc4_kernel(RoiAlignArgs p) {
  const int lane = threadIdx.x;
  const int nb = p.ph * p.pw;
  const int k = blockIdx.x / nb;
  const int bin = blockIdx.x - k * nb;
  const int ph = bin / p.pw, pw = bin - ph * p.pw;
  const int c = blockIdx.y * 256 + lane * 4;
  const bool c_ok = c < p.C;
  float* outk = p.out + (long long)k * p.so_k + c;
  const float* r = p.rois + (long long)k * 5;
  const int lvl = p.levels ? p.levels[k] : 0;
  const int H = p.H[lvl], W = p.W[lvl];
  const float spatial_scale = p.scale[lvl];
  const int b = (int)r[0];
  const float offset = p.aligned ? 0.5f : 0.0f;
  const float roi_start_w = r[1] * spatial_scale - offset;
  const float roi_start_h = r[2] * spatial_scale - offset;
  const float roi_end_w = r[3] * spatial_scale - offset;
  const float roi_end_h = r[4] * spatial_scale - offset;
  float roi_width = roi_end_w - roi_start_w;
  float roi_height = roi_end_h - roi_start_h;
  if (p.aligned) {
    if (!(roi_width >= 0 && roi_height >= 0)) {
      if (p.status && lane == 0 && blockIdx.y == 0) atomicOr(p.status, 1);
    }
  } else {
    roi_width = roi_width > 1.f ? roi_width : 1.f;
    roi_height = roi_height > 1.f ? roi_height : 1.f;
  }
  const float bin_h = roi_height / (float)p.ph;
  const float bin_w = roi_width / (float)p.pw;
  const int gh = p.sampling_ratio > 0 ? p.sampling_ratio : (int)ceilf(roi_height / (float)p.ph);
  const int gw = p.sampling_ratio > 0 ? p.sampling_ratio : (int)ceilf(roi_width / (float)p.pw);
  const int cnt = gh * gw > 1 ? gh * gw : 1;
  const float count = (float)cnt;
  const float* in = p.feat[lvl] + (long long)b * p.sb[lvl] + (c_ok ? c : 0);
  const long long C = p.C;
  {
    {
      float4 acc = {0.f, 0.f, 0.f, 0.f};
      for (int iy = 0; iy < gh; ++iy) {
        const float yy = roi_start_h + ph * bin_h + (float)(iy + .5f) * bin_h / (float)gh;
        for (int ix = 0; ix < gw; ++ix) {
          const float xx = roi_start_w + pw * bin_w + (float)(ix + .5f) * bin_w / (float)gw;
          float x = xx, y = yy;
          if (y < -1.0f || y > (float)H || x < -1.0f || x > (float)W) continue;
          if (y <= 0) y = 0;
          if (x <= 0) x = 0;
          int y_low = (int)y, x_low = (int)x, y_high, x_high;
          if (y_low >= H - 1) { y_high = y_low = H - 1; y = (float)y_low; } else y_high = y_low + 1;
          if (x_low >= W - 1) { x_high = x_low = W - 1; x = (float)x_low; } else x_high = x_low + 1;
          const float ly = y - y_low, lx = x - x_low;
          const float hy = 1.f - ly, hx = 1.f - lx;
          const float w1 = hy * hx, w2 = hy * lx, w3 = ly * hx, w4 = ly * lx;
          const float4 v1 = *reinterpret_cast<const float4*>(in + (long long)(y_low * W + x_low) * C);
          const float4 v2 = *reinterpret_cast<const float4*>(in + (long long)(y_low * W + x_high) * C);
          const float4 v3 = *reinterpret_cast<const float4*>(in + (long long)(y_high * W + x_low) * C);
          const float4 v4 = *reinterpret_cast<const float4*>(in + (long long)(y_high * W + x_high) * C);
          acc.x += w1 * v1.x + w2 * v2.x + w3 * v3.x + w4 * v4.x;
          acc.y += w1 * v1.y + w2 * v2.y + w3 * v3.y + w4 * v4.y;
          acc.z += w1 * v1.z + w2 * v2.z + w3 * v3.z + w4 * v4.z;
          acc.w += w1 * v1.w + w2 * v2.w + w3 * v3.w + w4 * v4.w;
        }
      }
      if (c_ok) {
        float4 o = {acc.x / count, acc.y / count, acc.z / count, acc.w / count};
        *reinterpret_cast<float4*>(outk + ph * p.so_h + pw * p.so_w) = o;
      }
    }
  }
}

#define ROI_UNI(x) __builtin_amdgcn_readfirstlane(x)
#ifndef ROI_RB4
#define ROI_RB4 2
#endif
#ifndef ROI_RB8
#define ROI_RB8 1
#endif
#ifndef ROI_WAVE_MLP
#define ROI_WAVE_MLP 8
#endif
template <int PW>
__global__ __launch_bounds__(512) void roi_align_fwd_nhwc_wave_kernel(RoiAlignArgs p) {
  const int lane = threadIdx.x & 63;
  const int ph = ROI_UNI((int)(threadIdx.x >> 6));
  const int k = p.order ? p.order[blockIdx.x] : (int)blockIdx.x;
  if (ph >= p.ph) return;
  const int cbase = blockIdx.y * 256;
  const float* r = p.rois + (long long)k * 5;
  const int lvl = p.levels ? p.levels[k] : 0;
  const int H = p.H[lvl], W = p.W[lvl];
  const float spatial_scale = p.scale[lvl];
  const int b = (int)r[0];
  const float offset = p.aligned ? 0.5f : 0.0f;
  const float roi_start_w = r[1] * spatial_scale - offset;
  const float roi_start_h = r[2] * spatial_scale - offset;
  const float roi_end_w = r[3] * spatial_scale - offset;
  const float roi_end_h = r[4] * spatial_scale - offset;
  float roi_width = roi_end_w - roi_start_w;
  float roi_height = roi_end_h - roi_start_h;
  if (p.aligned) {
    if (!(roi_width >= 0 && roi_height >= 0)) {
      if (p.status && lane == 0 && blockIdx.y == 0 && ph == 0) atomicOr(p.status, 1);
    }
  } else {
    roi_width = roi_width > 1.f ? roi_width : 1.f;
    roi_height = roi_height > 1.f ? roi_height : 1.f;
  }
  const float bin_h = roi_height / (float)p.ph;
  const float bin_w = roi_width / (float)p.pw;
  const int gh = ROI_UNI(p.sampling_ratio > 0 ? p.sampling_ratio : (int)ceilf(roi_height / (float)p.ph));
  const int gw = ROI_UNI(p.sampling_ratio > 0 ? p.sampling_ratio : (int)ceilf(roi_width / (float)p.pw));
  const int cnt = gh * gw > 1 ? gh * gw : 1;
  const float count = (float)cnt;
  const long long C = p.C;
  const bool c_ok = cbase + lane * 4 < p.C;
  const float* in = p.feat[lvl] + (long long)b * p.sb[lvl] + (c_ok ? cbase + lane * 4 : 0);
  float* outp = p.out + (long long)k * p.so_k + ph * p.so_h + cbase + lane * 4;

  const float yf = roi_start_h + ph * bin_h, yl = roi_start_h + (ph + 1) * bin_h;
  const int y0 = ROI_UNI(min((int)floorf(fmaxf(yf, 0.f)), H - 1)), y1 = ROI_UNI(min((int)floorf(fmaxf(yl, 0.f)) + 1, H - 1));
  const int x0 = ROI_UNI(min((int)floorf(fmaxf(roi_start_w, 0.f)), W - 1));
  const int x1 = ROI_UNI(min((int)floorf(fmaxf(roi_start_w + roi_width, 0.f)) + 1, W - 1));
  const int nrows = y1 - y0 + 1, ncols = x1 - x0 + 1;
  const bool sep = gh > 0 && gw > 0 && nrows >= 1 && nrows <= 64 && ncols >= 1 && ncols <= 64;
  if (!sep) {
    for (int pw = 0; pw < p.pw; ++pw) {
      float4 acc = {0.f, 0.f, 0.f, 0.f};
      for (int iy = 0; iy < gh; ++iy) {
        const float yy = roi_start_h + ph * bin_h + (float)(iy + .5f) * bin_h / (float)gh;
        for (int ix = 0; ix < gw; ++ix) {
          const float xx = roi_start_w + pw * bin_w + (float)(ix + .5f) * bin_w / (float)gw;
          float x = xx, y = yy;
          if (y < -1.0f || y > (float)H || x < -1.0f || x > (float)W) continue;
          if (y <= 0) y = 0;
          if (x <= 0) x = 0;
          int y_low = (int)y, x_low = (int)x, y_high, x_high;
          if (y_low >= H - 1) { y_high = y_low = H - 1; y = (float)y_low; } else y_high = y_low + 1;
          if (x_low >= W - 1) { x_high = x_low = W - 1; x = (float)x_low; } else x_high = x_low + 1;
          const float ly = y - y_low, lx = x - x_low;
          const float hy = 1.f - ly, hx = 1.f - lx;
          const float w1 = hy * hx, w2 = hy * lx, w3 = ly * hx, w4 = ly * lx;
          const float4 v1 = *reinterpret_cast<const float4*>(in + (long long)(y_low * W + x_low) * C);
          const float4 v2 = *reinterpret_cast<const float4*>(in + (long long)(y_low * W + x_high) * C);
          const float4 v3 = *reinterpret_cast<const float4*>(in + (long long)(y_high * W + x_low) * C);
          const float4 v4 = *reinterpret_cast<const float4*>(in + (long long)(y_high * W + x_high) * C);
          acc.x += w1 * v1.x + w2 * v2.x + w3 * v3.x + w4 * v4.x;
          acc.y += w1 * v1.y + w2 * v2.y + w3 * v3.y + w4 * v4.y;
          acc.z += w1 * v1.z + w2 * v2.z + w3 * v3.z + w4 * v4.z;
          acc.w += w1 * v1.w + w2 * v2.w + w3 * v3.w + w4 * v4.w;
        }
      }
      if (c_ok) *reinterpret_cast<float4*>(outp + pw * p.so_w) = float4{acc.x / count, acc.y / count, acc.z / count, acc.w / count};
    }
    return;
  }
  float wy = 0.f;
  {
    const int ymine = y0 + lane;
    for (int iy = 0; iy < gh; ++iy) {
      const float yy = roi_start_h + ph * bin_h + (float)(iy + .5f) * bin_h / (float)gh;
      if (yy < -1.0f || yy > (float)H) continue;
      float y = yy <= 0 ? 0.f : yy;
      int y_low = (int)y, y_high;
      if (y_low >= H - 1) { y_high = y_low = H - 1; y = (float)y_low; } else y_high = y_low + 1;
      const float ly = y - y_low, hy = 1.f - ly;
      wy += (y_low == ymine ? hy : 0.f) + (y_high == ymine ? ly : 0.f);
    }
  }
  float wx[PW];
#pragma unroll
  for (int pw = 0; pw < PW; ++pw) {
    const int xmine = x0 + lane;
    float a = 0.f;
    for (int ix = 0; ix < gw; ++ix) {
      const float xx = roi_start_w + pw * bin_w + (float)(ix + .5f) * bin_w / (float)gw;
      if (xx < -1.0f || xx > (float)W) continue;
      float x = xx <= 0 ? 0.f : xx;
      int x_low = (int)x, x_high;
      if (x_low >= W - 1) { x_high = x_low = W - 1; x = (float)x_low; } else x_high = x_low + 1;
      const float lx = x - x_low, hx = 1.f - lx;
      a += (x_low == xmine ? hx : 0.f) + (x_high == xmine ? lx : 0.f);
    }
    wx[pw] = a;
  }
  unsigned amask = 0;
#pragma unroll
  for (int pw = 0; pw < PW; ++pw) amask |= wx[pw] != 0.f ? 1u << pw : 0u;
  float4 acc[PW];
#pragma unroll
  for (int pw = 0; pw < PW; ++pw) acc[pw] = float4{0.f, 0.f, 0.f, 0.f};
  const float* base = in + ((long long)y0 * W + x0) * C;
  const int Ci = (int)C, rowstep = W * Ci;
  auto chunk = [&](auto cw_tag, auto rb_tag, int c0) {
    constexpr int CW = decltype(cw_tag)::value, RB = decltype(rb_tag)::value;
    const int ncw = min(CW, ncols - c0);
    float4 T[CW];
#pragma unroll
    for (int u = 0; u < CW; ++u) T[u] = float4{0.f, 0.f, 0.f, 0.f};
    for (int r0 = 0; r0 < nrows; r0 += RB) {
      float4 v[RB][CW];
#pragma unroll
      for (int rb = 0; rb < RB; ++rb)
#pragma unroll
        for (int u = 0; u < CW; ++u) {
          const bool live = u < ncw && r0 + rb < nrows;
          v[rb][u] = *reinterpret_cast<const float4*>(base + (live ? (r0 + rb) * rowstep + (c0 + u) * Ci : 0));
        }
#pragma unroll
      for (int rb = 0; rb < RB; ++rb) {
        if (r0 + rb >= nrows) continue;
        const float wyr = __uint_as_float(__builtin_amdgcn_readlane(__float_as_uint(wy), r0 + rb));
#pragma unroll
        for (int u = 0; u < CW; ++u) {
          if (u >= ncw) continue;
          T[u].x = __builtin_fmaf(wyr, v[rb][u].x, T[u].x); T[u].y = __builtin_fmaf(wyr, v[rb][u].y, T[u].y);
          T[u].z = __builtin_fmaf(wyr, v[rb][u].z, T[u].z); T[u].w = __builtin_fmaf(wyr, v[rb][u].w, T[u].w);
        }
      }
    }
#pragma unroll
    for (int u = 0; u < CW; ++u) {
      if (u >= ncw) continue;
      const unsigned am = __builtin_amdgcn_readlane(amask, c0 + u);
#pragma unroll
      for (int pw = 0; pw < PW; ++pw) {
        if (am & (1u << pw)) {
          const float w = __uint_as_float(__builtin_amdgcn_readlane(__float_as_uint(wx[pw]), c0 + u));
          acc[pw].x = __builtin_fmaf(w, T[u].x, acc[pw].x); acc[pw].y = __builtin_fmaf(w, T[u].y, acc[pw].y);
          acc[pw].z = __builtin_fmaf(w, T[u].z, acc[pw].z); acc[pw].w = __builtin_fmaf(w, T[u].w, acc[pw].w);
        }
      }
    }
  };
  if (ncols <= 4) {
    chunk(std::integral_constant<int, 4>{}, std::integral_constant<int, ROI_RB4>{}, 0);
  } else {
    for (int c0 = 0; c0 < ncols; c0 += 8) chunk(std::integral_constant<int, 8>{}, std::integral_constant<int, ROI_RB8>{}, c0);
  }
  if (c_ok) {
    const float inv = 1.f / count;
#pragma unroll
    for (int pw = 0; pw < PW; ++pw)
      *reinterpret_cast<float4*>(outp + pw * p.so_w) = float4{acc[pw].x * inv, acc[pw].y * inv, acc[pw].z * inv, acc[pw].w * inv};
  }
}

extern "C" int lvc_roi_align_route(int backward, int nhwc, int C, int pooled_h, int pooled_w, int has_num_valid,
                                   long long largest_level_elems) {
  if (backward) return nhwc && pooled_h == 7 && pooled_w == 7 ? 1 : 0;
  if (!nhwc || (C & 3) != 0 || has_num_valid) return 0;
  if (pooled_h <= 8 && pooled_w == 7 && largest_level_elems < (1ll << 31)) return 2;
  return 1;
}

static int launch(RoiAlignArgs& a, void* stream) {
  if (a.K == 0) return LVC_OK;
  long long largest = 0;
  for (int l = 0; l < LVC_MAX_LEVELS; ++l)
    if (a.feat[l] && (long long)a.H[l] * a.W[l] * a.C > largest) largest = (long long)a.H[l] * a.W[l] * a.C;
  const int route = lvc_roi_align_route(0, a.nhwc && a.so_c == 1, a.C, a.ph, a.pw, a.num_valid != nullptr, largest);
  if (route == 2) {
    hipLaunchKernelGGL(roi_align_fwd_nhwc_wave_kernel<7>, dim3(a.K, lvc_cdiv(a.C, 256)), dim3(64 * a.ph), 0, (hipStream_t)stream, a);
    LVC_CHECK_LAUNCH();
    return LVC_OK;
  }
  if (route == 1) {
    dim3 grid4(a.K * a.ph * a.pw, lvc_cdiv(a.C, 256)), block4(64);
    hipLaunchKernelGGL(roi_align_fwd_nhwc4_kernel, grid4, block4, 0, (hipStream_t)stream, a);
    LVC_CHECK_LAUNCH();
    return LVC_OK;
  }
  dim3 grid(a.K, lvc_cdiv(a.C, 256)), block(256);
  hipLaunchKernelGGL(roi_align_fwd_kernel, grid, block, 0, (hipStream_t)stream, a);
  LVC_CHECK_LAUNCH();
  return LVC_OK;
}

__global__ __launch_bounds__(256) void roi_align_bwd_kernel(RoiAlignArgs p) {
  const int k = blockIdx.x;
  const int c = blockIdx.y * 256 + threadIdx.x;
  if (p.num_valid && k >= *p.num_valid) return;
  const bool c_ok = c < p.C;
  const float* gk = p.out + (long long)k * p.so_k + (long long)(c_ok ? c : 0) * p.so_c;
  const float* r = p.rois + (long long)k * 5;
  const int lvl = p.levels ? p.levels[k] : 0;
  const int H = p.H[lvl], W = p.W[lvl];
  const float spatial_scale = p.scale[lvl];
  const int b = (int)r[0];
  const float offset = p.aligned ? 0.5f : 0.0f;
  const float roi_start_w = r[1] * spatial_scale - offset;
  const float roi_start_h = r[2] * spatial_scale - offset;
  const float roi_end_w = r[3] * spatial_scale - offset;
  const float roi_end_h = r[4] * spatial_scale - offset;
  float roi_width = roi_end_w - roi_start_w;
  float roi_height = roi_end_h - roi_start_h;
  if (p.aligned) {
    if (!(roi_width >= 0 && roi_height >= 0)) {
      if (p.status && threadIdx.x == 0 && blockIdx.y == 0) atomicOr(p.status, 1);
    }
  } else {
    roi_width = roi_width > 1.f ? roi_width : 1.f;
    roi_height = roi_height > 1.f ? roi_height : 1.f;
  }
  const float bin_h = roi_height / (float)p.ph;
  const float bin_w = roi_width / (float)p.pw;
  const int gh = p.sampling_ratio > 0 ? p.sampling_ratio : (int)ceilf(roi_height / (float)p.ph);
  const int gw = p.sampling_ratio > 0 ? p.sampling_ratio : (int)ceilf(roi_width / (float)p.pw);
  const float count = (float)(gh * gw);

  long long s_pix, s_c;
  if (p.nhwc) { s_pix = p.C; s_c = 1; } else { s_pix = 1; s_c = (long long)H * W; }
  float* gin = const_cast<float*>(p.feat[lvl]) + (long long)b * p.sb[lvl] + (long long)(c_ok ? c : 0) * s_c;

  for (int ph = 0; ph < p.ph; ++ph) {
    for (int pw = 0; pw < p.pw; ++pw) {
      const float g = c_ok ? gk[ph * p.so_h + pw * p.so_w] : 0.f;
      for (int iy = 0; iy < gh; ++iy) {
        const float yy = roi_start_h + ph * bin_h + (float)(iy + .5f) * bin_h / (float)gh;
        for (int ix = 0; ix < gw; ++ix) {
          const float xx = roi_start_w + pw * bin_w + (float)(ix + .5f) * bin_w / (float)gw;
          float x = xx, y = yy;
          if (y < -1.0f || y > (float)H || x < -1.0f || x > (float)W) continue;
          if (y <= 0) y = 0;
          if (x <= 0) x = 0;
          int y_low = (int)y, x_low = (int)x, y_high, x_high;
          if (y_low >= H - 1) { y_high = y_low = H - 1; y = (float)y_low; } else y_high = y_low + 1;
          if (x_low >= W - 1) { x_high = x_low = W - 1; x = (float)x_low; } else x_high = x_low + 1;
          const float ly = y - y_low, lx = x - x_low;
          const float hy = 1.f - ly, hx = 1.f - lx;
          const float w1 = hy * hx, w2 = hy * lx, w3 = ly * hx, w4 = ly * lx;
          if (c_ok) {
            unsafeAtomicAdd(gin + (long long)(y_low * W + x_low) * s_pix, g * w1 / count);
            unsafeAtomicAdd(gin + (long long)(y_low * W + x_high) * s_pix, g * w2 / count);
            unsafeAtomicAdd(gin + (long long)(y_high * W + x_low) * s_pix, g * w3 / count);
            unsafeAtomicAdd(gin + (long long)(y_high * W + x_high) * s_pix, g * w4 / count);
          }
        }
      }
    }
  }
}

#define RB_MAXF 192
// ... 249 lines not shown
  for (int k = tid; k < p.K; k += 1024) atomicAdd(&hist[bucket(k)], 1);
  __syncthreads();
  if (tid == 0) {
    int run = 0;
    for (int i = 0; i < 64; ++i) { const int n = hist[i]; hist[i] = run; run += n; }
  }
  __syncthreads();
  for (int k = tid; k < p.K; k += 1024) p.order[atomicAdd(&hist[bucket(k)], 1)] = k;
}

extern "C" int lvc_roi_work_order(const float* rois, const int* levels, const float* scales, int L, int K, int pooled_h,
                                  int* d_order, void* stream) {
  LVC_CHECK_ARG(L >= 1 && L <= LVC_MAX_LEVELS && K >= 0 && pooled_h > 0, "bad shape");
  if (K == 0) return LVC_OK;
  LVC_CHECK_ARG(rois && scales && d_order && (L == 1 || levels), "null pointer");
  RoiOrderArgs a;
  memset(&a, 0, sizeof a);
  a.rois = rois; a.levels = levels; a.K = K; a.ph = pooled_h; a.order = d_order;
  for (int l = 0; l < L; ++l) a.scale[l] = scales[l];
  hipLaunchKernelGGL(roi_work_order_kernel, dim3(1), dim3(1024), 0, (hipStream_t)stream, a);
  LVC_CHECK_LAUNCH();
  return LVC_OK;
}

#define ROI_XCD_MAX_B 16
struct RoiOrderXcdArgs {
  const float* rois;
  const int* levels;
  int K, B;
  int* order;
};
__global__ __launch_bounds__(1024) void roi_work_order_xcd_kernel(RoiOrderXcdArgs p) {
  __shared__ int hist[ROI_XCD_MAX_B][256];
  __shared__ int cnt[ROI_XCD_MAX_B], tail0[ROI_XCD_MAX_B], s_min;
  const int tid = threadIdx.x;
  for (int i = tid; i < ROI_XCD_MAX_B * 256; i += 1024) (&hist[0][0])[i] = 0;
  __syncthreads();
  auto key = [&](int k, int& b) {
    const float* r = p.rois + (long long)k * 5;
    const float bf = r[0];
    b = bf >= 0.f && bf < (float)p.B ? (int)bf : 0;
    const int lv = p.levels ? (p.levels[k] & 3) : 0;
    const float yc = (r[2] + r[4]) * 0.5f;
    int band = yc == yc ? (int)(fminf(fmaxf(yc, 0.f), 1e6f) * (1.f / 16.f)) : 0;
    band = band > 63 ? 63 : band;
    return lv * 64 + band;
  };
  for (int k = tid; k < p.K; k += 1024) { int b; const int ky = key(k, b); atomicAdd(&hist[b][ky], 1); }
  __syncthreads();
  if (tid < p.B) {
    int run = 0;
    for (int i = 0; i < 256; ++i) { const int n = hist[tid][i]; hist[tid][i] = run; run += n; }
    cnt[tid] = run;
  }
  __syncthreads();
  if (tid == 0) {
    int m = cnt[0];
    for (int b = 1; b < p.B; ++b) m = cnt[b] < m ? cnt[b] : m;
    s_min = m;
    int run = 0;
    for (int b = 0; b < p.B; ++b) { tail0[b] = run; run += cnt[b] - m; }
  }
  __syncthreads();
  const int m = s_min;
  for (int k = tid; k < p.K; k += 1024) {
    int b;
    const int ky = key(k, b);
    const int r = atomicAdd(&hist[b][ky], 1);
    p.order[r < m ? r * p.B + b : m * p.B + tail0[b] + (r - m)] = k;
  }
}

extern "C" int lvc_roi_work_order_xcd(const float* rois, const int* levels, int K, int B, int* d_order, void* stream) {
  LVC_CHECK_ARG(K >= 0 && B >= 1 && B <= ROI_XCD_MAX_B, "1..16 images");
  if (K == 0) return LVC_OK;
  LVC_CHECK_ARG(rois && d_order, "null pointer");
  RoiOrderXcdArgs a;
  a.rois = rois; a.levels = levels; a.K = K; a.B = B; a.order = d_order;
  hipLaunchKernelGGL(roi_work_order_xcd_kernel, dim3(1), dim3(1024), 0, (hipStream_t)stream, a);
  LVC_CHECK_LAUNCH();
  return LVC_OK;
}

static int roi_align_fpn_nhwc_impl(const float* const* feats, const int* Hs, const int* Ws,
                                      const float* scales, int L, int B, int C, const float* rois,
                                      const int* levels, const int* d_num_valid, int K, int pooled_h,
                                      int pooled_w, int sampling_ratio, int aligned, float* output,
                                      int* d_status, const int* d_order, void* stream) {
  LVC_CHECK_ARG(L >= 1 && L <= LVC_MAX_LEVELS, "1..8 levels");
  LVC_CHECK_ARG(K == 0 || (feats && Hs && Ws && scales && rois && output), "null pointer");
  LVC_CHECK_ARG(B > 0 && C > 0 && pooled_h > 0 && pooled_w > 0 && K >= 0, "bad shape");
  LVC_CHECK_ARG(L == 1 || K == 0 || levels, "levels required when L > 1");
  RoiAlignArgs a;
  memset(&a, 0, sizeof a);
  for (int l = 0; l < L; ++l) {
    a.feat[l] = feats[l]; a.H[l] = Hs[l]; a.W[l] = Ws[l]; a.scale[l] = scales[l];
    a.sb[l] = (long long)C * Hs[l] * Ws[l];
  }
  a.nhwc = 1; a.C = C; a.rois = rois; a.levels = levels; a.num_valid = d_num_valid;
  a.K = K; a.ph = pooled_h; a.pw = pooled_w; a.sampling_ratio = sampling_ratio; a.aligned = aligned;
  a.out = output;
  a.so_k = (long long)C * pooled_h * pooled_w; a.so_c = 1;
  a.so_h = (long long)pooled_w * C; a.so_w = C;
  a.status = d_status;
  a.order = d_order;
  return launch(a, stream);
}

extern "C" int lvc_roi_align_fpn_nhwc(const float* const* feats, const int* Hs, const int* Ws,
                                      const float* scales, int L, int B, int C, const float* rois,
                                      const int* levels, const int* d_num_valid, int K, int pooled_h,
                                      int pooled_w, int sampling_ratio, int aligned, float* output,
                                      int* d_status, void* stream) {
  return roi_align_fpn_nhwc_impl(feats, Hs, Ws, scales, L, B, C, rois, levels, d_num_valid, K, pooled_h, pooled_w, sampling_ratio, aligned,
                                 output, d_status, nullptr, stream);
}

extern "C" int lvc_roi_align_fpn_nhwc_ordered(const float* const* feats, const int* Hs, const int* Ws,
                                      const float* scales, int L, int B, int C, const float* rois,
                                      const int* levels, const int* d_num_valid, int K, int pooled_h,
                                      int pooled_w, int sampling_ratio, int aligned, float* output,
                                      int* d_status, const int* d_order, void* stream) {
  return roi_align_fpn_nhwc_impl(feats, Hs, Ws, scales, L, B, C, rois, levels, d_num_valid, K, pooled_h, pooled_w, sampling_ratio, aligned,
                                 output, d_status, d_order, stream);
}
```

### lvc_amd/kernels.py

```python
import collections
import ctypes

import torch

from . import _lib
from ._lib import LvcNativeError, c_float, c_int, c_longlong, c_void_p, check, ptr

BK = 32
BN = 128


def _stream(t):
    return c_void_p(torch.cuda.current_stream(t.device).cuda_stream)


def _req_cuda(*ts):
    for t in ts:
        if t is not None and not t.is_cuda:
            raise RuntimeError("lvc_amd kernels need device tensors (got a CPU tensor); there is no CPU path")


def _float3(v):
    return (c_float * 3)(*[float(x) for x in v])

# ... 1025 lines not shown
        check(st, "lvc_stem_conv_pool_nhwc4_f16x2")
        return out
    raise RuntimeError("the fused stem exists for the fp16 split only; BasicStem runs conv + max-pool as two launches otherwise")


def linear(x, pc, relu=False, split=None):
    M, Kin = x.shape
    y = conv2d_nhwc(x.view(M, 1, 1, Kin), pc, relu=relu, split=split)
    return y.view(M, pc.K)


def new_status(device):
    return torch.zeros(1, dtype=torch.int32, device=device)


ROI_NEGATIVE_SIZE = 1
DET_OVERFLOW = 2
RETINA_OVERFLOW = 4
MASK_BAD_CLASS = 8
KEYPOINT_BAD_TARGET = 16


def roi_align_forward(input, rois, spatial_scale, pooled_h, pooled_w, sampling_ratio, aligned, status=None):
    _req_cuda(input, rois)
    input = input.contiguous().float()
    rois = rois.contiguous().float()
    B, C, H, W = input.shape
    K = rois.shape[0]
    out = torch.empty(K, C, pooled_h, pooled_w, device=input.device, dtype=torch.float32)
    st = _lib.lib().lvc_roi_align_forward_nchw(
        ptr(input), ptr(rois), ptr(out), B, C, H, W, K,
        pooled_h, pooled_w, spatial_scale, sampling_ratio,
        1 if aligned else 0, ptr(status), _stream(input))
    check(st, "lvc_roi_align_forward_nchw")
    return out


ROI_FWD_ROUTES = ("scalar", "nhwc4", "wave")
ROI_BWD_ROUTES = ("scatter", "rows")


def roi_align_route(backward, nhwc, C, pooled_h, pooled_w, has_num_valid=False, largest_level_elems=0):
    r = _lib.lib().lvc_roi_align_route(1 if backward else 0, 1 if nhwc else 0, C, pooled_h, pooled_w, 1 if has_num_valid else 0,
                                       largest_level_elems)
    return (ROI_BWD_ROUTES if backward else ROI_FWD_ROUTES)[r]


ROI_ORDER_MIN = 1024


def roi_align_fpn_nhwc(feats, scales, rois, levels, pooled_h, pooled_w, sampling_ratio, aligned,
                       num_valid=None, status=None, order=None, out=None):
    _req_cuda(rois, *feats)
    L = len(feats)
    B, _, _, C = feats[0].shape
    K = rois.shape[0]
    rois = rois.contiguous().float()
    if out is None:
        out = torch.empty(K, pooled_h, pooled_w, C, device=rois.device, dtype=torch.float32)
    assert out.shape == (K, pooled_h, pooled_w, C) and out.is_contiguous() and out.dtype == torch.float32
    FP = c_void_p * L
    IP = c_int * L
    FL = c_float * L
    fp = FP(*[f.data_ptr() for f in feats])
    hs = IP(*[f.shape[1] for f in feats])
    ws = IP(*[f.shape[2] for f in feats])
    sc = FL(*[float(s) for s in scales])
    for f in feats:
        assert f.is_contiguous() and f.dtype == torch.float32 and f.shape[0] == B and f.shape[3] == C
    if levels is not None:
        assert levels.dtype == torch.int32 and levels.is_contiguous()
    if order is not None:
        assert order.dtype == torch.int32 and order.is_contiguous() and order.numel() == K
    elif K >= ROI_ORDER_MIN:
        order = torch.empty(K, device=rois.device, dtype=torch.int32)
        if B <= 16:
            check(_lib.lib().lvc_roi_work_order_xcd(ptr(rois), ptr(levels), K, B, ptr(order), _stream(rois)), "lvc_roi_work_order_xcd")
        else:
            check(_lib.lib().lvc_roi_work_order(ptr(rois), ptr(levels), sc, L, K, pooled_h, ptr(order), _stream(rois)),
                  "lvc_roi_work_order")
    st = _lib.lib().lvc_roi_align_fpn_nhwc_ordered(
        fp, hs, ws, sc, L, B, C, ptr(rois), ptr(levels), ptr(num_valid), K,
        pooled_h, pooled_w, sampling_ratio, 1 if aligned else 0, ptr(out),
        ptr(status), ptr(order), _stream(rois))
    check(st, "lvc_roi_align_fpn_nhwc")
    return out


def roi_align_backward(grad, rois, spatial_scale, pooled_h, pooled_w, batch_size, channels, height, width,
                       sampling_ratio, aligned, status=None):
    _req_cuda(grad, rois)
    grad = grad.contiguous().float()
    rois = rois.contiguous().float()
    K = rois.shape[0]
    assert grad.shape == (K, channels, pooled_h, pooled_w)
    gin = torch.empty(batch_size, channels, height, width, device=grad.device, dtype=torch.float32)
    st = _lib.lib().lvc_roi_align_backward_nchw(
        ptr(grad), ptr(rois), ptr(gin), batch_size, channels, height, width, K,
        pooled_h, pooled_w, spatial_scale, sampling_ratio,
        1 if aligned else 0, ptr(status), _stream(grad))
    check(st, "lvc_roi_align_backward_nchw")
    return gin


def roi_align_fpn_backward_nhwc(grad, shapes, scales, rois, levels, sampling_ratio, aligned, num_valid=None,
                                status=None, outs=None):
    _req_cuda(grad, rois)
    grad = grad.contiguous().float()
    rois = rois.contiguous().float()
    K, ph, pw, C = grad.shape
    L = len(shapes)
    B = shapes[0][0]
    if outs is None:
        outs = [torch.empty(*sh, device=grad.device, dtype=torch.float32) for sh in shapes]
    assert len(outs) == L
    for o, sh in zip(outs, shapes):
        assert o.shape == tuple(sh) and o.is_contiguous() and o.dtype == torch.float32 and sh[0] == B and sh[3] == C
    FP = c_void_p * L
    IP = c_int * L
    FL = c_float * L
    if levels is not None:
        assert levels.dtype == torch.int32 and levels.is_contiguous()
    st = _lib.lib().lvc_roi_align_fpn_backward_nhwc(
        ptr(grad), FP(*[o.data_ptr() for o in outs]), IP(*[sh[1] for sh in shapes]), IP(*[sh[2] for sh in shapes]),
        FL(*[float(s) for s in scales]), L, B, C, ptr(rois), ptr(levels), ptr(num_valid),
        K, ph, pw, sampling_ratio, 1 if aligned else 0, ptr(status),
        _stream(grad))
    check(st, "lvc_roi_align_fpn_backward_nhwc")
    return outs


SELECT_ONELAUNCH = int(_os.environ.get("LVC_SELECT_ONELAUNCH", "3"))


def set_select_onelaunch(mode):
    global SELECT_ONELAUNCH
    SELECT_ONELAUNCH = int(mode)
    _lib.lib().lvc_set_select_onelaunch(int(mode))


def batched_nms_batch(boxes, scores, idxs, counts, iou_threshold, max_keep=0):
    _req_cuda(boxes, scores, idxs, counts)
    B, Nmax = scores.shape
    boxes = boxes.contiguous().float()
    scores = scores.contiguous().float()
    if idxs is not None:
        idxs = idxs.contiguous()
        assert idxs.dtype == torch.int32
    keep = torch.empty(B, Nmax, dtype=torch.int32, device=boxes.device)
    num_keep = torch.empty(B, dtype=torch.int32, device=boxes.device)
    wsb = _lib.size_query("lvc_batched_nms_workspace_bytes", B, Nmax)
    ws = torch.empty(wsb, dtype=torch.uint8, device=boxes.device)
    st = _lib.lib().lvc_batched_nms(
        ptr(boxes), ptr(scores), ptr(idxs), ptr(counts), B, Nmax, iou_threshold,
        max_keep, ptr(keep), ptr(num_keep), ptr(ws), wsb, _stream(boxes))
    check(st, "lvc_batched_nms")
    return keep, num_keep


def batched_nms(boxes, scores, idxs, iou_threshold):
    n = boxes.shape[0]
    if n == 0:
        return torch.empty(0, dtype=torch.int64, device=boxes.device)
    idx32 = idxs.to(torch.int32)[None] if idxs is not None else None
    keep, nk = batched_nms_batch(boxes[None], scores[None], idx32, None, iou_threshold)
    return keep[0, : int(nk.item())].to(torch.int64)


def nms(boxes, scores, iou_threshold):
    return batched_nms(boxes, scores, None, iou_threshold)


SCALE_CLAMP = 4.135166556742356


def _arr(ctype, vals):
    return (ctype * len(vals))(*vals)


def rpn_proposals(logits, deltas, cell_anchors, strides, image_sizes, pre_nms_topk, post_nms_topk,
                  nms_thresh, min_box_size=0.0):
    L = len(logits)
    B, A = logits[0].shape[0], cell_anchors[0].shape[0]
    dev = logits[0].device
    _req_cuda(*logits, *deltas, *cell_anchors, image_sizes)
    for t in list(logits) + list(deltas):
        assert t.dtype == torch.float32 and t.stride(-1) == 1 and t.dim() == 4
        assert t.stride(2) == t.stride(3) * 0 + t.stride(2)
    Hs = [t.shape[1] for t in logits]
    Ws = [t.shape[2] for t in logits]
    for t, h, w in zip(list(logits) + list(deltas), Hs * 2, Ws * 2):
        assert t.stride(1) == w * t.stride(2) and t.stride(0) == h * w * t.stride(2), "need an NHWC channel slice"
    VP, IP = c_void_p * L, c_int * L
    lp = VP(*[t.data_ptr() for t in logits])
    dp = VP(*[t.data_ptr() for t in deltas])
    ap = VP(*[t.contiguous().data_ptr() for t in cell_anchors])
    ldl = IP(*[t.stride(2) for t in logits])
    ldd = IP(*[t.stride(2) for t in deltas])
    hs, ws_, st = IP(*Hs), IP(*Ws), IP(*strides)
    lib = _lib.lib()
    nbytes = _lib.size_query("lvc_rpn_proposals_workspace_bytes", B, L, A, hs, ws_, pre_nms_topk)
    ws = torch.empty(nbytes, dtype=torch.uint8, device=dev)
    boxes = torch.empty(B, post_nms_topk, 4, device=dev, dtype=torch.float32)
    olog = torch.empty(B, post_nms_topk, device=dev, dtype=torch.float32)
    count = torch.empty(B, dtype=torch.int32, device=dev)
    assert image_sizes.dtype == torch.int32 and image_sizes.is_contiguous()
    rc = lib.lvc_rpn_proposals(lp, ldl, dp, ldd, ap, hs, ws_, st, L, A, B, ptr(image_sizes),
                               pre_nms_topk, post_nms_topk, nms_thresh,
                               min_box_size, SCALE_CLAMP, ptr(boxes), ptr(olog), ptr(count),
                               ptr(ws), nbytes, _stream(boxes))
    check(rc, "lvc_rpn_proposals")
    return boxes, olog, count


def assign_levels_rois(boxes, min_level, max_level, canonical_box_size=224, canonical_level=4):
    _req_cuda(boxes)
    B, R, _ = boxes.shape
    boxes = boxes.contiguous()
    levels = torch.empty(B * R, dtype=torch.int32, device=boxes.device)
    rois = torch.empty(B * R, 5, dtype=torch.float32, device=boxes.device)
    rc = _lib.lib().lvc_assign_levels_rois(ptr(boxes), B, R, min_level, max_level,
                                           canonical_box_size, canonical_level, ptr(levels), ptr(rois),
                                           _stream(boxes))
    check(rc, "lvc_assign_levels_rois")
    return levels, rois


def fast_rcnn_inference(cls_logits, deltas, proposals, prop_count, image_sizes, num_classes, box_weights,
                        score_thresh, nms_thresh, topk, post=None, status=None, max_candidates=16384):
    _req_cuda(cls_logits, deltas, proposals, prop_count, image_sizes, post)
    B, R, _ = proposals.shape
    K = num_classes
    dev = proposals.device
    assert cls_logits.stride(1) == 1 and deltas.stride(1) == 1
    cls_agnostic = 1 if deltas.shape[1] == 4 else 0
    if status is None:
        status = new_status(dev)
    lib = _lib.lib()
    max_candidates = max(1, R * K) if max_candidates is None else min(max_candidates, max(1, R * K))
    nbytes = _lib.size_query("lvc_fast_rcnn_inference_workspace_bytes", B, max_candidates)
    ws = torch.empty(nbytes, dtype=torch.uint8, device=dev)
    ob = torch.empty(B, topk, 4, device=dev, dtype=torch.float32)
    osc = torch.empty(B, topk, device=dev, dtype=torch.float32)
    ocl = torch.empty(B, topk, device=dev, dtype=torch.int32)
    orow = torch.empty(B, topk, device=dev, dtype=torch.int32)
    cnt = torch.empty(B, device=dev, dtype=torch.int32)
    wx, wy, ww, wh = box_weights
    rc = lib.lvc_fast_rcnn_inference(
        ptr(cls_logits), cls_logits.stride(0), ptr(deltas), deltas.stride(0), K,
        cls_agnostic, ptr(proposals.contiguous()), ptr(prop_count), B, R, ptr(image_sizes),
        wx, wy, ww, wh, SCALE_CLAMP, score_thresh,
        nms_thresh, topk, max_candidates, ptr(post), ptr(ob), ptr(osc), ptr(ocl), ptr(orow),
        ptr(cnt), ptr(status), ptr(ws), nbytes, _stream(proposals))
    check(rc, "lvc_fast_rcnn_inference")
    return ob, osc, ocl, orow, cnt


RETINANET_MAX_SURVIVORS = 1 << 16
RETINANET_OVERFLOW = 4


def retinanet_select(logits, deltas, cell_anchors, strides, anchor_offset, num_classes, topk, score_thresh,
                     box_weights=(1.0, 1.0, 1.0, 1.0), max_survivors=RETINANET_MAX_SURVIVORS, status=None):
    L = len(logits)
    if not (L == len(deltas) == len(cell_anchors) == len(strides) and 1 <= L <= 8):
        raise ValueError("retinanet_select: 1..8 levels with logits, deltas, cell anchors and a stride each")
    _req_cuda(*logits, *deltas, *cell_anchors, status)
    B, A, K = logits[0].shape[0], cell_anchors[0].shape[0], int(num_classes)
    dev = logits[0].device
    if not (0 < topk <= 2048):
        raise ValueError("retinanet_select: topk must be in 1..2048 (got {})".format(topk))
    if any(c.shape != (A, 4) for c in cell_anchors):
        raise NotImplementedError("retinanet_select: a different number of anchors per level is not built")
    Hs = [t.shape[1] for t in logits]
    Ws = [t.shape[2] for t in logits]
    for t, d, h, w in zip(logits, deltas, Hs, Ws):
        for u, need in ((t, A * K), (d, 4 * A)):
            if not (u.dtype == torch.float32 and u.dim() == 4 and u.shape[:3] == (B, h, w) and u.shape[3] >= need and u.stride(3) == 1
                    and u.stride(1) == w * u.stride(2) and u.stride(0) == h * w * u.stride(2)):
                raise ValueError("retinanet_select: need fp32 NHWC channel slices [B,H,W,>=A*K] / [B,H,W,>=4A] of dense pixel rows")
        if h * w * A * K >= (1 << 31) or h * w * t.stride(2) >= (1 << 31):
            raise ValueError("retinanet_select: a level with 2^31 entries per image")
    full = max(h * w * A * K for h, w in zip(Hs, Ws))
    max_survivors = full if max_survivors is None else max(1, min(int(max_survivors), full))
    if status is None:
        status = new_status(dev)
    VP, IP = c_void_p * L, c_int * L
    lp = VP(*[t.data_ptr() for t in logits])
    dp = VP(*[t.data_ptr() for t in deltas])
    anchors = [t.contiguous().float() for t in cell_anchors]
    ap = VP(*[t.data_ptr() for t in anchors])
    ldl = IP(*[t.stride(2) for t in logits])
    ldd = IP(*[t.stride(2) for t in deltas])
    hs, ws_, st = IP(*Hs), IP(*Ws), IP(*[int(s) for s in strides])
    lib = _lib.lib()
    try:
        nbytes = _lib.size_query("lvc_retinanet_select_workspace_bytes", B, L, A, K, hs, ws_, topk, max_survivors)
    except _lib.LvcNativeError:
        raise ValueError("retinanet_select: shapes outside the kernel's range") from None
    ws = torch.empty(nbytes, dtype=torch.uint8, device=dev)
    rows = L * topk
    boxes = torch.empty(B, rows, 4, device=dev, dtype=torch.float32)
    scores = torch.empty(B, rows, device=dev, dtype=torch.float32)
    classes = torch.empty(B, rows, device=dev, dtype=torch.int32)
    index = torch.empty(B, rows, device=dev, dtype=torch.int32)
    count = torch.empty(B, device=dev, dtype=torch.int32)
    wx, wy, ww, wh = [float(v) for v in box_weights]
    rc = lib.lvc_retinanet_select(lp, ldl, dp, ldd, ap, hs, ws_, st, anchor_offset, L, A, K, B,
                                  topk, score_thresh, wx, wy, ww, wh,
                                  SCALE_CLAMP, max_survivors, ptr(boxes), ptr(scores), ptr(classes), ptr(index),
                                  ptr(count), ptr(status), ptr(ws), nbytes, _stream(boxes))
    check(rc, "lvc_retinanet_select")
    return boxes, scores, classes, index, count, status


def retinanet_select_checked(*args, max_survivors=RETINANET_MAX_SURVIVORS, **kw):
    out = retinanet_select(*args, max_survivors=max_survivors, **kw)
    if max_survivors is not None and int(out[5].item()) & RETINANET_OVERFLOW:
        _log_once("retinanet_overflow", "more than %d entries above the score threshold on one (image, level): the selection is "
                  "repeated with the list sized for H*W*A*K", max_survivors)
        kw.pop("status", None)
        out = retinanet_select(*args, max_survivors=None, **kw)
    return out


class RetinaNetLossArgs:

    def __init__(self, logits, deltas, num_anchors, num_classes, anchors, matches, labels, gt, gt_classes, gt_off,
                 alpha=0.25, gamma=2.0, beta=0.1, box_weights=(1.0, 1.0, 1.0, 1.0)):
        L = len(logits)
        if not (L == len(deltas) and 1 <= L <= 8):
            raise ValueError("retinanet_loss: 1..8 levels with logits and deltas each")
        if 0.0 < float(gamma) < 1.0 or float(gamma) < 0.0:
            raise NotImplementedError("MODEL.RETINANET.FOCAL_LOSS_GAMMA = {}: an exponent in (0, 1) has an unbounded derivative at "
                                      "saturation (and a negative one is no focal loss); 0 or >= 1 are built".format(gamma))
        _req_cuda(*logits, *deltas, anchors, matches, labels, gt_off, gt_classes)
        A, Kc = int(num_anchors), int(num_classes)
# ... 1901 lines not shown
```

### lvc_amd/modeling/poolers.py

```python
import math

import torch
from torch import nn

from .. import kernels as K
from ..layers.layout import to_nchw_view, to_nhwc


class _PoolAllLevels(torch.autograd.Function):

    @staticmethod
    def forward(ctx, pooler, boxes, status, *feats):
        levels, rois = K.assign_levels_rois(boxes, pooler.min_level, pooler.max_level, pooler.canonical_box_size,
                                            pooler.canonical_level)
        if len(feats) == 1:
            levels = None
        ctx.pooler, ctx.rois, ctx.levels = pooler, rois, levels
        ctx.shapes = [tuple(f.shape) for f in feats]
        return K.roi_align_fpn_nhwc(list(feats), pooler.scales, rois, levels, pooler.output_size[0], pooler.output_size[1],
                                    pooler.sampling_ratio, pooler.aligned, status=status)

    @staticmethod
    @torch.autograd.function.once_differentiable
    def backward(ctx, grad):
        pl = ctx.pooler
        grads = K.roi_align_fpn_backward_nhwc(grad, ctx.shapes, pl.scales, ctx.rois, ctx.levels, pl.sampling_ratio, pl.aligned)
        return (None, None, None) + tuple(grads)


class _PoolRois(torch.autograd.Function):

    @staticmethod
    def forward(ctx, pooler, rois, levels, num_valid, status, *feats):
        ctx.pooler, ctx.rois, ctx.levels, ctx.num_valid = pooler, rois, levels, num_valid
        ctx.shapes = [tuple(f.shape) for f in feats]
        return K.roi_align_fpn_nhwc(list(feats), pooler.scales, rois, levels, pooler.output_size[0], pooler.output_size[1],
                                    pooler.sampling_ratio, pooler.aligned, status=status)

    @staticmethod
    @torch.autograd.function.once_differentiable
    def backward(ctx, grad):
        pl = ctx.pooler
        grads = K.roi_align_fpn_backward_nhwc(grad, ctx.shapes, pl.scales, ctx.rois, ctx.levels, pl.sampling_ratio, pl.aligned,
                                              num_valid=ctx.num_valid)
        return (None, None, None, None, None) + tuple(grads)


class ROIPooler(nn.Module):
    def __init__(self, output_size, scales, sampling_ratio, pooler_type, canonical_box_size=224, canonical_level=4):
        super().__init__()
        if isinstance(output_size, int):
            output_size = (output_size, output_size)
        assert len(output_size) == 2 and isinstance(output_size[0], int) and isinstance(output_size[1], int)
        self.output_size = output_size
        if pooler_type == "ROIAlign":
            self.aligned = False
        elif pooler_type == "ROIAlignV2":
            self.aligned = True
        else:
            raise NotImplementedError("pooler type '{}' is not used by the shipped configs".format(pooler_type))
        self.scales = tuple(scales)
        self.sampling_ratio = sampling_ratio
        min_level = -(math.log2(scales[0]))
        max_level = -(math.log2(scales[-1]))
        assert math.isclose(min_level, int(min_level)) and math.isclose(max_level, int(max_level)), \
            "Featuremap stride is not power of 2!"
        self.min_level, self.max_level = int(min_level), int(max_level)
        assert len(scales) == self.max_level - self.min_level + 1, "[ROIPooler] Sizes of input featuremaps do not form a pyramid!"
        assert 0 <= self.min_level <= self.max_level
        self.canonical_level = canonical_level
        assert canonical_box_size > 0
        self.canonical_box_size = canonical_box_size

    def pool_nhwc(self, feats_nhwc, boxes, status=None):
        if torch.is_grad_enabled() and any(f.requires_grad for f in feats_nhwc):
            return _PoolAllLevels.apply(self, boxes.detach(), status, *feats_nhwc)
        levels, rois = K.assign_levels_rois(boxes, self.min_level, self.max_level, self.canonical_box_size,
                                            self.canonical_level)
        if len(feats_nhwc) == 1:
            levels = None
        return K.roi_align_fpn_nhwc(feats_nhwc, self.scales, rois, levels, self.output_size[0], self.output_size[1],
                                    self.sampling_ratio, self.aligned, status=status)

    def pool_rois_nhwc(self, feats_nhwc, rois, levels, num_valid=None, status=None):
        if torch.is_grad_enabled() and any(f.requires_grad for f in feats_nhwc):
            return _PoolRois.apply(self, rois, levels, num_valid, status, *feats_nhwc)
        return K.roi_align_fpn_nhwc(feats_nhwc, self.scales, rois, levels, self.output_size[0], self.output_size[1],
                                    self.sampling_ratio, self.aligned, status=status)

    def forward(self, x, box_lists):
        assert isinstance(x, list) and isinstance(box_lists, list), "Arguments to pooler must be lists"
        assert len(x) == len(self.scales)
        assert len(box_lists) == x[0].size(0)
        counts = [len(b) for b in box_lists]
        M = sum(counts)
        C = x[0].shape[1]
        if M == 0:
            return torch.zeros((0, C) + self.output_size, device=x[0].device, dtype=x[0].dtype)
        R = max(counts)
        boxes = torch.zeros(len(box_lists), R, 4, device=x[0].device)
        for i, b in enumerate(box_lists):
            boxes[i, : counts[i]] = b.tensor
        out = self.pool_nhwc([to_nhwc(f) for f in x], boxes)
        out = out.view(len(box_lists), R, self.output_size[0], self.output_size[1], C)
        out = torch.cat([out[i, : counts[i]] for i in range(len(box_lists))], 0)
        return out.permute(0, 3, 1, 2)
```

### lvc_amd/modeling/roi_heads/box_head.py

```python
import numpy as np
import torch
import torch.nn.functional as F
from torch import nn

from ... import kernels as K
from ...layers import Conv2d, Linear, ShapeSpec, get_norm
from ...layers.wrappers import _PackedCache, linear_fn
from ...utils import weight_init
from ...utils.registry import Registry

ROI_BOX_HEAD_REGISTRY = Registry("ROI_BOX_HEAD")


@ROI_BOX_HEAD_REGISTRY.register()
class FastRCNNConvFCHead(nn.Module):
    def __init__(self, cfg, input_shape: ShapeSpec):
        super().__init__()
        H = cfg.MODEL.ROI_BOX_HEAD
        num_conv, conv_dim, num_fc, fc_dim, norm = H.NUM_CONV, H.CONV_DIM, H.NUM_FC, H.FC_DIM, H.NORM
        dropout = H.DROPOUT
        assert num_conv + num_fc > 0
        self._output_size = (input_shape.channels, input_shape.height, input_shape.width)
        self.conv_norm_relus = []
        for k in range(num_conv):
            conv = Conv2d(self._output_size[0], conv_dim, kernel_size=3, padding=1, bias=not norm,
                          norm=get_norm(norm, conv_dim), activation=F.relu)
            self.add_module("conv{}".format(k + 1), conv)
            self.conv_norm_relus.append(conv)
            self._output_size = (conv_dim, self._output_size[1], self._output_size[2])
        self.dropout = nn.Dropout(p=dropout) if dropout else nn.Identity()
        self.fcs = []
        self._fc1_chw = self._output_size if num_fc else None
        for k in range(num_fc):
            fc = Linear(int(np.prod(self._output_size)), fc_dim)
            self.add_module("fc{}".format(k + 1), fc)
            self.fcs.append(fc)
            self._output_size = fc_dim
        for layer in self.conv_norm_relus:
            weight_init.c2_msra_fill(layer)
        for layer in self.fcs:
            weight_init.c2_xavier_fill(layer)
        self._fc1_hwc = _PackedCache()

    def _packed_fc1_hwc(self):
        fc = self.fcs[0]
        C, Hh, Ww = self._fc1_chw

        def build():
            w = fc.weight.view(fc.out_features, C, Hh, Ww).permute(0, 2, 3, 1).reshape(fc.out_features, -1)
            return K.pack_linear(w, fc.bias)

        return self._fc1_hwc.get([fc.weight, fc.bias], build)

    def forward_nhwc(self, x):
        if self.conv_norm_relus and x.shape[0] == 0:
            size = self._output_size if isinstance(self._output_size, int) else int(np.prod(self._output_size))
            return x.new_zeros((0, size))
        for layer in self.conv_norm_relus:
            x = layer.forward_nhwc(x)
        if len(self.fcs):
            M = x.shape[0]
            fc = self.fcs[0]
            C, Hh, Ww = self._fc1_chw
            x = linear_fn(
                x.reshape(M, -1), fc.weight, fc.bias, self._packed_fc1_hwc(), relu=True,
                w_packed_layout=lambda: fc.weight.detach().view(fc.out_features, C, Hh, Ww).permute(0, 2, 3, 1).reshape(fc.out_features, -1),
                w_view=lambda dw: dw.view(fc.out_features, Hh, Ww, C).permute(0, 3, 1, 2).reshape(fc.out_features, -1))
            x = self.dropout(x)
            for fc in self.fcs[1:]:
                x = self.dropout(fc(x, relu=True))
        return x

    def forward(self, x):
        if x.dim() == 4:
            from ...layers.layout import to_nhwc

            return self.forward_nhwc(to_nhwc(x))
        for fc in self.fcs:
            x = self.dropout(fc(x, relu=True))
        return x

    @property
    def output_size(self):
        return self._output_size


def build_box_head(cfg, input_shape):
    return ROI_BOX_HEAD_REGISTRY.get(cfg.MODEL.ROI_BOX_HEAD.NAME)(cfg, input_shape)
```

### lvc_amd/modeling/roi_heads/fast_rcnn.py

```python
import torch
from torch import nn

from ... import kernels as K
from ...layers import Linear, ShapeSpec
from ...layers.wrappers import _PackedCache
from ...utils.registry import Registry
from ..box_regression import Box2BoxTransform

ROI_HEADS_OUTPUT_REGISTRY = Registry("ROI_HEADS_OUTPUT")


class _OutputLayersBase(nn.Module):
    def _common(self, cfg, input_shape):
        if isinstance(input_shape, int):
            input_shape = ShapeSpec(channels=input_shape)
        self.input_size = input_shape.channels * (input_shape.width or 1) * (input_shape.height or 1)
        self.num_classes = cfg.MODEL.ROI_HEADS.NUM_CLASSES
        self.cls_agnostic_bbox_reg = cfg.MODEL.ROI_BOX_HEAD.CLS_AGNOSTIC_BBOX_REG
        self.box2box_transform = Box2BoxTransform(weights=cfg.MODEL.ROI_BOX_HEAD.BBOX_REG_WEIGHTS)
        self.smooth_l1_beta = cfg.MODEL.ROI_BOX_HEAD.SMOOTH_L1_BETA
        self.test_score_thresh = cfg.MODEL.ROI_HEADS.SCORE_THRESH_TEST
        self.test_nms_thresh = cfg.MODEL.ROI_HEADS.NMS_THRESH_TEST
        self.test_topk_per_image = cfg.TEST.DETECTIONS_PER_IMAGE
        self.box_reg_loss_type = cfg.MODEL.ROI_BOX_HEAD.BBOX_REG_LOSS_TYPE
        self.loss_weight = {"loss_box_reg": cfg.MODEL.ROI_BOX_HEAD.BBOX_REG_LOSS_WEIGHT}
        self.num_bbox_reg_classes = 1 if self.cls_agnostic_bbox_reg else self.num_classes


@ROI_HEADS_OUTPUT_REGISTRY.register()
class FastRCNNOutputLayers(_OutputLayersBase):
    def __init__(self, cfg, input_shape):
        super().__init__()
        self._common(cfg, input_shape)
        self.cls_score = Linear(self.input_size, self.num_classes + 1)
        self.bbox_pred = Linear(self.input_size, self.num_bbox_reg_classes * 4)
        nn.init.normal_(self.cls_score.weight, std=0.01)
        nn.init.normal_(self.bbox_pred.weight, std=0.001)
        for l in [self.cls_score, self.bbox_pred]:
            nn.init.constant_(l.bias, 0)
        self._fused = _PackedCache()

    def forward(self, x):
        if x.dim() > 2:
            x = torch.flatten(x, start_dim=1)
        c, b = self.cls_score, self.bbox_pred
        def build():
            w = torch.cat([c.weight, b.weight], 0)
            bias = torch.cat([c.bias, b.bias], 0)
            padk = (-w.shape[0]) % 4
            if padk:
                w = torch.cat([w, w.new_zeros(padk, w.shape[1])], 0)
                bias = torch.cat([bias, bias.new_zeros(padk)], 0)
            return K.pack_linear(w, bias)

        y = K.linear(x.contiguous(), self._fused.get([c.weight, c.bias, b.weight, b.bias], build))
        k1 = self.num_classes + 1
        return y[:, :k1], y[:, k1:k1 + self.num_bbox_reg_classes * 4]


@ROI_HEADS_OUTPUT_REGISTRY.register()
class CosineSimOutputLayers(_OutputLayersBase):
    def __init__(self, cfg, input_shape):
        super().__init__()
        self._common(cfg, input_shape)
        self.cls_score = Linear(self.input_size, self.num_classes + 1, bias=False)
        self.scale = cfg.MODEL.ROI_HEADS.COSINE_SCALE
        if self.scale == -1:
            self.scale = nn.Parameter(torch.ones(1) * 20.0)
        self.bbox_pred = Linear(self.input_size, self.num_bbox_reg_classes * 4)
        nn.init.normal_(self.cls_score.weight, std=0.01)
        nn.init.normal_(self.bbox_pred.weight, std=0.001)
        nn.init.constant_(self.bbox_pred.bias, 0)
        self._cos = _PackedCache()

    def forward(self, x):
        if x.dim() > 2:
            x = torch.flatten(x, start_dim=1)
        x = x.contiguous()
        xn = K.rownorm(x, eps=1e-5, mode=0)
        w = self.cls_score.weight
        K.rownorm(w.data, eps=1e-5, mode=0, out=w.data)
        scale = float(self.scale) if not isinstance(self.scale, nn.Parameter) else float(self.scale.item())

        def build():
            pc = K.pack_linear(w)
            pc.scale = torch.full((pc.K,), scale, device=w.device, dtype=torch.float32)
            return pc

        self._cos.key = None
        scores = K.linear(xn, self._cos.get([w], build))
        deltas = self.bbox_pred(x)
        return scores, deltas


class _BoxOnlyBase(nn.Module):

    def __init__(self, cfg, input_shape, box2box_transform=None):
        super().__init__()
        if isinstance(input_shape, int):
            input_shape = ShapeSpec(channels=input_shape)
        input_size = input_shape.channels * (input_shape.width or 1) * (input_shape.height or 1)
        self.num_classes = cfg.MODEL.ROI_HEADS.NUM_CLASSES
        self.bbox_pred = Linear(input_size, 4)
        nn.init.normal_(self.bbox_pred.weight, std=0.001)
        nn.init.constant_(self.bbox_pred.bias, 0)
        self.box2box_transform = box2box_transform or Box2BoxTransform(weights=cfg.MODEL.ROI_BOX_HEAD.BBOX_REG_WEIGHTS)
        self.lambda_ = cfg.MODEL.UBBR.LAMBDA
        self.iterate = cfg.MODEL.ROI_HEADS.NAME != "CascadeROIHeads"

    def forward(self, x):
        if x.dim() > 2:
            x = torch.flatten(x, start_dim=1)
        return self.num_classes, self.bbox_pred(x.contiguous())

    def losses(self, predictions, proposals):
        _, deltas = predictions
        gt_classes = torch.cat([p.gt_classes for p in proposals], 0)
        pboxes = torch.cat([p.proposal_boxes.tensor for p in proposals], 0)
        assert not pboxes.requires_grad, "Proposals should not require gradients"
        gboxes = torch.cat([(p.gt_boxes if p.has("gt_boxes") else p.proposal_boxes).tensor for p in proposals], 0)
        return {"loss_box_reg": _GIoUBoxLoss.apply(deltas, pboxes, gboxes, gt_classes, self)}

    def predict_boxes(self, predictions, proposals):
        _, deltas = predictions
        n = [len(p) for p in proposals]
        pboxes = torch.cat([p.proposal_boxes.tensor for p in proposals], 0)
        boxes = K.decode_boxes(deltas.detach().contiguous(), pboxes.view(1, -1, 4).contiguous(),
                               self.box2box_transform.weights, None)
        return boxes.view(-1, 4).split(n, dim=0)


@ROI_HEADS_OUTPUT_REGISTRY.register()
class BoxOnlyLayers(_BoxOnlyBase):
    pass


@ROI_HEADS_OUTPUT_REGISTRY.register()
class BoxOnlyLayersCascade(_BoxOnlyBase):
# ... 102 lines not shown
```

### lvc_amd/modeling/roi_heads/roi_heads.py

```python
import torch
from torch import nn

from ... import kernels as K
from ...layers import ShapeSpec
from ...layers.layout import require_device, to_nhwc
from ...structures import Boxes, Instances
from ...utils.events import get_event_storage
from ...utils.registry import Registry
from ..box_regression import Box2BoxTransform
from ..matcher import Matcher
from ..sampling import subsample_labels
from ..poolers import ROIPooler
from .box_head import build_box_head
from .fast_rcnn import ROI_HEADS_OUTPUT_REGISTRY
from .keypoint_head import TRAIN_REFUSAL as KEYPOINT_TRAIN_REFUSAL
from .keypoint_head import build_keypoint_head, keypoint_rcnn_inference
from .mask_head import build_mask_head, mask_rcnn_inference

ROI_HEADS_REGISTRY = Registry("ROI_HEADS")


def build_roi_heads(cfg, input_shape):
    if cfg.MODEL.KEYPOINT_ON and cfg.MODEL.ROI_HEADS.NAME != "StandardROIHeads":
        raise NotImplementedError("MODEL.KEYPOINT_ON with MODEL.ROI_HEADS.NAME = {!r}: the keypoint branch is built for StandardROIHeads"
# ... 253 lines not shown
        res = node.POOLER_RESOLUTION
        scales = tuple(1.0 / self.feature_strides[k] for k in self.in_features)
        in_channels = [self.feature_channels[f] for f in self.in_features]
        assert len(set(in_channels)) == 1, in_channels
        setattr(self, name + "_in_features", self.in_features)
        setattr(self, name + "_pooler", ROIPooler(output_size=res, scales=scales, sampling_ratio=node.POOLER_SAMPLING_RATIO,
                                                  pooler_type=node.POOLER_TYPE))
        setattr(self, name + "_head", build_head(cfg, ShapeSpec(channels=in_channels[0], height=res, width=res)))

    def _pool_branch(self, name, feats_nhwc, boxes, count, status=None):
        pl = getattr(self, name + "_pooler")
        feats = [feats_nhwc[f] for f in getattr(self, name + "_in_features")]
        rois, levels, rows, total, order = front_rows(boxes, count, pl, len(feats))
        pooled = K.roi_align_fpn_nhwc(feats, pl.scales, rois, levels, pl.output_size[0], pl.output_size[1], pl.sampling_ratio, pl.aligned,
                                      status=status)
        return pooled, rois, rows, total, order

    def pool_masks_batched(self, feats_nhwc, boxes, classes, count, status=None):
        pooled, _rois, rows, total, order = self._pool_branch("mask", feats_nhwc, boxes, count, status=status)
        return pooled, classes.reshape(-1).index_select(0, order).contiguous(), rows, total

    def _branch_loss_batched(self, name, feats_nhwc, s_boxes, s_cls, s_m, fg_count, gt, status):
        if not getattr(self, name + "_on"):
            raise RuntimeError("{}_loss_batched: the model was built with MODEL.{}_ON = False".format(name, name.upper()))
        head, pooler = getattr(self, name + "_head"), getattr(self, name + "_pooler")
        cap = max(int(self.batch_size_per_image * self.positive_sample_fraction), 1)
        R = min(cap, s_boxes.shape[1])
        boxes = s_boxes[:, :R].detach().contiguous()
        matched = s_m[:, :R].to(torch.int64).contiguous()
        count = fg_count.to(torch.int32).clamp(min=0, max=R)
        rows, target_counts = head.train_targets(boxes, matched, count, gt, head.map_scale * pooler.output_size[0])
        feats = [feats_nhwc[f] for f in getattr(self, name + "_in_features")]
        rois, levels, _rows, total, order = front_rows(boxes, count, pooler, len(feats))
        if head.loss_takes_classes:
            rows = (s_cls[:, :R].to(torch.int32).reshape(-1),) + rows
        rows = [t.index_select(0, order) for t in rows]
        pooled = pooler.pool_rois_nhwc(feats, rois, levels, num_valid=total, status=status)
        loss, counts = head.train_loss(pooled, rows, total, status, s_boxes.shape[0])
        return loss, {name + "." + k: v for k, v in dict(counts, **target_counts, status=status).items()}

    def forward_masks_batched(self, feats_nhwc, boxes, classes, count, status=None):
        if not self.mask_on:
            raise RuntimeError("forward_masks_batched: the model was built with MODEL.MASK_ON = False")
        pooled, cls, rows, total = self.pool_masks_batched(feats_nhwc, boxes, classes, count, status=status)
        prob = self.mask_head.forward_nhwc(pooled, cls, num_valid=total, status=status)
        return prob, rows

    def forward_keypoints_batched(self, feats_nhwc, boxes, count, status=None):
        if not self.keypoint_on:
            raise RuntimeError("forward_keypoints_batched: the model was built with MODEL.KEYPOINT_ON = False")
        pooled, rois, rows, total, _order = self._pool_branch("keypoint", feats_nhwc, boxes, count, status=status)
        kp = self.keypoint_head.forward_nhwc(pooled, rois[:, 1:5].contiguous(), num_valid=total, status=status)
        return kp, rows

    def forward_with_given_boxes(self, features, instances):
        assert not self.training
        assert instances[0].has("pred_boxes") and instances[0].has("pred_classes")
        if not self._branches():
            return instances
        name = self._branches()[-1]
        in_features = getattr(self, name + "_in_features")
        feats = {f: to_nhwc(features[f]) for f in in_features}
        dev = feats[in_features[0]].device
        require_device(feats[in_features[0]], "StandardROIHeads")
        boxes, counts = padded_boxes(instances, "pred_boxes", dev)
        if name == "mask":
            classes = torch.zeros(boxes.shape[:2], dtype=torch.int32, device=dev)
            for i, p in enumerate(instances):
                classes[i, : counts[i]] = p.pred_classes.to(torch.int32)
        status = K.new_status(dev)
        count = torch.tensor(counts, dtype=torch.int32, device=dev)
        if name == "mask":
            out, _rows = self.forward_masks_batched(feats, boxes, classes, count, status=status)
        else:
            out, _rows = self.forward_keypoints_batched(feats, boxes, count, status=status)
        check_status(int(status.item()))
        (mask_rcnn_inference if name == "mask" else keypoint_rcnn_inference)(out, instances)
        return instances

    def forward_batched(self, feats_nhwc, prop_boxes, prop_count, image_sizes_dev, post=None, status=None):
        if self.reg_off:
            raise NotImplementedError("ROI_HEADS.REG_OFF is not used by the shipped configs")
        feats = [feats_nhwc[f] for f in self.in_features]
        pooled = self.box_pooler.pool_nhwc(feats, prop_boxes, status=status)
        h = self.box_head.forward_nhwc(pooled)
        scores, deltas = self.box_predictor(h)
        return K.fast_rcnn_inference(scores, deltas, prop_boxes, prop_count, image_sizes_dev, self.num_classes,
                                     self.box2box_transform.weights, self.test_score_thresh, self.test_nms_thresh,
                                     self.test_detections_per_img, post=post, status=status,
                                     max_candidates=self.det_max_candidates)

    def forward(self, images, features, proposals, targets=None):
        if self.training:
            if self.mask_on and not self.__dict__.get("_mask_train_enabled", False):
                raise NotImplementedError("training the mask branch (MODEL.MASK_ON: mask_rcnn_loss, gt_masks) is not built")
            if self.keypoint_on and not self.__dict__.get("_keypoint_train_enabled", False):
                raise NotImplementedError(KEYPOINT_TRAIN_REFUSAL)
            return self._forward_train(features, proposals, targets)
        if self.rbg:
            proposals = self.label_and_sample_proposals(proposals, targets, inference=True)
        feats = {f: to_nhwc(features[f]) for f in self.in_features}
        dev = feats[self.in_features[0]].device
        require_device(feats[self.in_features[0]], "StandardROIHeads")
        boxes, counts = padded_boxes(proposals, "proposal_boxes", dev)
        sizes = torch.tensor([list(p.image_size) for p in proposals], dtype=torch.int32, device=dev)
        status = K.new_status(dev)
        ob, osc, ocl, orow, cnt = self.forward_batched(feats, boxes, torch.tensor(counts, dtype=torch.int32, device=dev),
                                                       sizes, status=status)
        prob = rows = kp = None
        if self.mask_on:
            prob, rows = self.forward_masks_batched(feats, ob, ocl, cnt, status=status)
        if self.keypoint_on:
            kp, rows = self.forward_keypoints_batched(feats, ob, cnt, status=status)
        insts = instances_from_batched(ob, osc, ocl, cnt, [p.image_size for p in proposals], status)
        if prob is not None:
            mask_rcnn_inference(prob, insts)
        if kp is not None:
            keypoint_rcnn_inference(kp, insts)
        return insts, {}

    def can_batch_train(self, targets):
        return (self.batched_sampling and self.batched_targets and self.proposal_append_gt and not self.rbg and self.batch_size_per_image <= 1024
                and type(self)._forward_train is StandardROIHeads._forward_train and targets is not None and len(targets) > 0
                and all(0 < len(t) <= 512 and not (self.relabel_ignored_gt and t.has("gt_ignores")) for t in targets)
                and len(self.proposal_matcher.user_thresholds) in (1, 2))

    def _box_stats(self, pred, gc):
        fg = (gc >= 0) & (gc < self.num_classes)
        hit = pred == gc
        return torch.stack([fg.sum(), hit.sum(), (hit & fg).sum(), ((pred == self.num_classes) & fg).sum()])

    def forward_train_batched(self, features, pboxes, plogits, pcount, gt, gt_off, targets):
        from .fast_rcnn import fast_rcnn_losses

        s_boxes, _s_logits, s_cls, s_m, s_gtb, cnt = self._sample_batched(pboxes, plogits, pcount, gt, gt_off, targets)
        feats = [to_nhwc(features[f]) for f in self.in_features]
        below = any(f.requires_grad for f in feats) or any(p.requires_grad for p in self.box_head.parameters())
        with torch.set_grad_enabled(below and torch.is_grad_enabled()):
            h = self.box_head.forward_nhwc(self.box_pooler.pool_nhwc(feats, s_boxes))
        gc = s_cls.view(-1)
        losses, pred = fast_rcnn_losses(self.box_predictor, h, s_boxes.view(-1, 4), s_gtb.view(-1, 4), gc)
        with torch.no_grad():
            stats = self._box_stats(pred, gc)
        parts = {"box": stats}
        for name in self._branches():
            bfeats = {f: to_nhwc(features[f]) for f in getattr(self, name + "_in_features")}
            loss, counts = self._branch_loss_batched(name, bfeats, s_boxes, s_cls, s_m, cnt[:, 0], self._gt_of(name, targets),
                                                     K.new_status(s_boxes.device))
            losses = dict(losses)
            losses["loss_" + name] = loss
            parts.update(counts)
        with torch.no_grad():
            return losses, cnt, pack_step_counts(parts)

    def _branches(self):
        return [name for name in ("mask", "keypoint") if getattr(self, name + "_on", False)]

    def _gt_of(self, name, targets):
        return _gt_masks_of(targets) if name == "mask" else _gt_keypoints_of(targets, self.keypoint_head.num_keypoints)

    def log_train_scalars(self, counts, values, layout, nrows):
        named = unpack_step_counts(values, layout)
        _log_sample_counts(counts)
        for name in self._branches():
            getattr(self, "_log_{}_scalars".format(name))(named)
        _log_box_accuracy(named["box"], nrows)

    def _log_mask_scalars(self, c):
        from .mask_head import log_mask_scalars

        check_status(c["mask.status"][0])
        side = self.mask_head.map_scale * self.mask_pooler.output_size[0]
        log_mask_scalars(c["mask.pixels"], c["mask.rows"][0] * side * side)
# ... 217 lines not shown
```

Baseline: 661.3 img/s.

## Fuse ROI pooling into presplit FC1 planes and predictor GEMM with row stats

ROIAlign now writes pre-split fp16 operand planes that feed the first box-head FC directly, so the FC skips its own input split pass. The class/box predictor GEMM computes the per-row softmax max, inverse sum, count and threshold mask in its epilogue, which removes the separate row-stats kernel. Level assignment and the XCD work ordering are folded into one launch. This adds kernel variants and routing conditions, plus a guard that limits classes to 127.

```diff
diff --git a/include/lvc_amd.h b/include/lvc_amd.h
--- a/include/lvc_amd.h
+++ b/include/lvc_amd.h
@@ -146,7 +146,9 @@
 int lvc_roi_align_fpn_nhwc_ordered(const float* const* feats, const int* Hs, const int* Ws, const float* scales, int L,
                                    int B, int C, const float* rois, const int* levels, const int* d_num_valid, int K,
                                    int pooled_h, int pooled_w, int sampling_ratio, int aligned, float* output,
-                                   int* d_status, const int* d_order, void* stream);
+                                   int* d_status, const int* d_order, int planes_slot, const unsigned short* fc_w,
+                                   const float* fc_scale, const float* fc_shift, float* fc_y, int fc_K, int fc_relu,
+                                   void* workspace, void* stream);
 
 int lvc_roi_align_backward_nchw(const float* grad, const float* rois, float* grad_input, int B, int C, int H, int W,
                                 int K, int pooled_h, int pooled_w, float spatial_scale, int sampling_ratio,
@@ -199,7 +201,7 @@
                             float* const* ddeltas, const int* ld_ddelta, void* stream);
 
 int lvc_assign_levels_rois(const float* boxes, int B, int R, int min_level, int max_level, int canonical_box_size,
-                           int canonical_level, int* levels, float* rois, void* stream);
+                           int canonical_level, int* levels, float* rois, int* d_order, void* stream);
 
 long long lvc_fast_rcnn_inference_workspace_bytes(int B, int max_candidates);
 int lvc_fast_rcnn_inference(const float* cls_logits, int ld_cls, const float* deltas, int ld_delta, int K,
@@ -208,7 +210,10 @@
                             float score_thresh, double nms_thresh, int topk, int max_candidates,
                             const float* d_post, float* out_boxes, float* out_scores, int* out_classes,
                             int* out_rows, int* d_out_count, int* d_status, void* workspace,
-                            long long workspace_bytes, void* stream);
+                            long long workspace_bytes, int stats_mode, float* st_mx, float* st_inv, int* st_cnt,
+                            unsigned long long* st_mask, const float* pred_x, const unsigned short* pred_w,
+                            const float* pred_scale, const float* pred_shift, int pred_C, int pred_K, void* conv_workspace,
+                            void* stream);
 
 int lvc_decode_boxes(const float* deltas, int ld, const float* boxes, int M, int R, const int* d_image_sizes,
                      float wx, float wy, float ww, float wh, float scale_clamp, float* out, void* stream);
diff --git a/lvc_amd/csrc/boxes.hip b/lvc_amd/csrc/boxes.hip
--- a/lvc_amd/csrc/boxes.hip
+++ b/lvc_amd/csrc/boxes.hip
@@ -1,5 +1,7 @@
 #include "common.h"
 #include "select_common.h"
+#include "roi_levels.h"
+#include "det_row_stats.h"
 #include <stdlib.h>
 
 
@@ -716,12 +718,7 @@
   const int i = blockIdx.x * blockDim.x + threadIdx.x;
   if (i >= R * B) return;
   const float4 bx = *reinterpret_cast<const float4*>(boxes + (size_t)i * 4);
-  const float area = (bx.z - bx.x) * (bx.w - bx.y);
-  const float size = sqrtf(area);
-  float lvl = floorf(canonical_level + log2f(size / canonical_box_size + 1e-8f));
-  lvl = lvl < (float)min_level ? (float)min_level : lvl;
-  lvl = lvl > (float)max_level ? (float)max_level : lvl;
-  levels[i] = (int)lvl - min_level;
+  levels[i] = lvc_box_level(bx, min_level, max_level, canonical_box_size, canonical_level);
   if (rois) {
     float* r = rois + (size_t)i * 5;
     r[0] = (float)(i / R); r[1] = bx.x; r[2] = bx.y; r[3] = bx.z; r[4] = bx.w;
@@ -729,11 +726,13 @@
 }
 
 extern "C" int lvc_assign_levels_rois(const float* boxes, int B, int R, int min_level, int max_level,
-                                      int canonical_box_size, int canonical_level, int* levels, float* rois,
+                                      int canonical_box_size, int canonical_level, int* levels, float* rois, int* d_order,
                                       void* stream) {
   LVC_CHECK_ARG(B >= 0 && R >= 0, "negative size");
   if (B * R == 0) return LVC_OK;
   LVC_CHECK_ARG(boxes && levels, "null pointer");
+  if (d_order)
+    return lvc_roi_levels_order_xcd(boxes, B, R, min_level, max_level, canonical_box_size, canonical_level, levels, rois, d_order, stream);
   hipLaunchKernelGGL(assign_levels_kernel, dim3(lvc_cdiv(B * R, 256)), dim3(256), 0, (hipStream_t)stream, boxes, R,
                      B, min_level, max_level, (float)canonical_box_size, (float)canonical_level, levels, rois);
   LVC_CHECK_LAUNCH();
@@ -757,21 +756,7 @@
   __syncthreads();
   const int r = r0 + tid;
   if (r >= rows) return;
-  const float* lg = tile + tid * pitch;
-  float mx = -INFINITY;
-  for (int k = 0; k <= K; ++k) { float v = lg[k]; mx = v > mx ? v : mx; }
-  float sum = 0.f;
-  for (int k = 0; k <= K; ++k) sum += expf(lg[k] - mx);
-  const float inv = 1.f / sum;
-  int cnt = 0;
-  unsigned long long m0 = 0, m1 = 0;
-  for (int k = 0; k < K; ++k) {
-    const bool hit = expf(lg[k] - mx) * inv > score_thresh;
-    cnt += hit ? 1 : 0;
-    if (hit) { if (k < 64) m0 |= 1ull << k; else m1 |= 1ull << (k - 64); }
-  }
-  st_mx[r] = mx; st_inv[r] = inv; st_cnt[r] = cnt;
-  st_mask[2 * (size_t)r] = m0; st_mask[2 * (size_t)r + 1] = m1;
+  lvc_det_row_stats(tile + tid * pitch, K, score_thresh, (size_t)r, st_mx, st_inv, st_cnt, st_mask);
 }
 
 __global__ __launch_bounds__(1024) void det_candidates_kernel(
@@ -911,14 +896,15 @@
   return det_plan(B, max_candidates).total;
 }
 
-extern "C" int lvc_fast_rcnn_inference(const float* cls_logits, int ld_cls, const float* deltas, int ld_delta,
-                                       int K, int cls_agnostic, const float* proposals,
-                                       const int* d_prop_count, int B, int R, const int* d_image_sizes,
-                                       float wx, float wy, float ww, float wh, float scale_clamp,
-                                       float score_thresh, double nms_thresh, int topk, int max_candidates,
-                                       const float* d_post, float* out_boxes, float* out_scores,
-                                       int* out_classes, int* out_rows, int* d_out_count, int* d_status,
-                                       void* workspace, long long workspace_bytes, void* stream) {
+static int fast_rcnn_inference_impl(const float* cls_logits, int ld_cls, const float* deltas, int ld_delta,
+                                    int K, int cls_agnostic, const float* proposals,
+                                    const int* d_prop_count, int B, int R, const int* d_image_sizes,
+                                    float wx, float wy, float ww, float wh, float scale_clamp,
+                                    float score_thresh, double nms_thresh, int topk, int max_candidates,
+                                    const float* d_post, float* out_boxes, float* out_scores,
+                                    int* out_classes, int* out_rows, int* d_out_count, int* d_status,
+                                    void* workspace, long long workspace_bytes, void* stream, const float* in_mx,
+                                    const float* in_inv, const int* in_cnt, const unsigned long long* in_mask) {
   LVC_CHECK_ARG(B > 0 && R > 0 && K > 0 && topk > 0, "bad sizes");
   LVC_CHECK_ARG(max_candidates > 0, "max_candidates must be positive");
   LVC_CHECK_ARG(cls_logits && deltas && proposals && d_image_sizes && out_boxes && out_scores && out_classes &&
@@ -935,16 +921,17 @@
   int* keep = (int*)(ws + p.off_keep);
   int* nk = (int*)(ws + p.off_nk);
   const long long rows = (long long)B * R;
-  float* st_mx = nullptr; float* st_inv = nullptr; int* st_cnt = nullptr;
-  unsigned long long* st_mask = nullptr;
-  if (K + 1 < DET_MAX_COLS && rows * 28 + 64 <= p.total - p.off_nms) {
-    st_mask = (unsigned long long*)(ws + p.off_nms);
-    st_mx = (float*)(st_mask + 2 * rows);
-    st_inv = st_mx + rows;
-    st_cnt = (int*)(st_inv + rows);
+  const float* st_mx = in_mx; const float* st_inv = in_inv; const int* st_cnt = in_cnt;
+  const unsigned long long* st_mask = in_mask;
+  if (!in_mx && K + 1 < DET_MAX_COLS && rows * 28 + 64 <= p.total - p.off_nms) {
+    unsigned long long* w_mask = (unsigned long long*)(ws + p.off_nms);
+    float* w_mx = (float*)(w_mask + 2 * rows);
+    float* w_inv = w_mx + rows;
+    int* w_cnt = (int*)(w_inv + rows);
     hipLaunchKernelGGL(det_row_stats_kernel, dim3((unsigned)lvc_cdiv64(rows, DET_TILE_ROWS)), dim3(DET_TILE_ROWS), 0, st,
-                       cls_logits, ld_cls, K, (int)rows, score_thresh, st_mx, st_inv, st_cnt, st_mask);
+                       cls_logits, ld_cls, K, (int)rows, score_thresh, w_mx, w_inv, w_cnt, w_mask);
     LVC_CHECK_LAUNCH();
+    st_mask = w_mask; st_mx = w_mx; st_inv = w_inv; st_cnt = w_cnt;
   }
   hipLaunchKernelGGL(det_candidates_kernel, dim3(B), dim3(1024), 0, st, cls_logits, ld_cls, deltas, ld_delta, K,
                      cls_agnostic, proposals, d_prop_count, R, d_image_sizes, wx, wy, ww, wh, scale_clamp,
@@ -957,6 +944,42 @@
                      max_candidates, topk, d_post, out_boxes, out_scores, out_classes, out_rows, d_out_count);
   LVC_CHECK_LAUNCH();
   return LVC_OK;
+}
+
+extern "C" int lvc_fast_rcnn_inference(const float* cls_logits, int ld_cls, const float* deltas, int ld_delta,
+                                       int K, int cls_agnostic, const float* proposals,
+                                       const int* d_prop_count, int B, int R, const int* d_image_sizes,
+                                       float wx, float wy, float ww, float wh, float scale_clamp,
+                                       float score_thresh, double nms_thresh, int topk, int max_candidates,
+                                       const float* d_post, float* out_boxes, float* out_scores,
+                                       int* out_classes, int* out_rows, int* d_out_count, int* d_status,
+                                       void* workspace, long long workspace_bytes, int stats_mode, float* st_mx, float* st_inv,
+                                       int* st_cnt, unsigned long long* st_mask, const float* pred_x, const unsigned short* pred_w,
+                                       const float* pred_scale, const float* pred_shift, int pred_C, int pred_K,
+                                       void* conv_workspace, void* stream) {
+  LVC_CHECK_ARG(stats_mode >= 0 && stats_mode <= 3, "stats_mode 0..3");
+  LVC_CHECK_ARG(stats_mode == 0 || (st_mx && st_inv && st_cnt && st_mask), "null row statistics");
+  LVC_CHECK_ARG(B > 0 && R > 0 && K > 0, "bad sizes");
+  if (stats_mode == 1) {
+    LVC_CHECK_ARG(K + 1 < DET_MAX_COLS && cls_logits, "statistics launch: K + 1 < 97");
+    hipLaunchKernelGGL(det_row_stats_kernel, dim3((unsigned)lvc_cdiv64((long long)B * R, DET_TILE_ROWS)), dim3(DET_TILE_ROWS), 0,
+                       (hipStream_t)stream, cls_logits, ld_cls, K, B * R, score_thresh, st_mx, st_inv, st_cnt, st_mask);
+    LVC_CHECK_LAUNCH();
+  } else if (stats_mode >= 2) {
+    LVC_CHECK_ARG(K + 1 <= LVC_DET_STATS_MAX_COLS, "row statistics hold K + 1 <= 128 classes");
+  }
+  if (stats_mode == 3) {
+    LVC_CHECK_ARG(cls_logits && pred_x && pred_w && conv_workspace && pred_C > 0 && ld_cls == pred_K, "predictor operands");
+    int rc = lvc_pw_s1_rowstats(pred_x, pred_w, pred_scale, pred_shift, const_cast<float*>(cls_logits), B * R, pred_C, pred_K, pred_K, K,
+                                score_thresh, st_mx, st_inv, st_cnt, st_mask, conv_workspace, stream);
+    if (rc) return rc;
+  }
+  const bool handed = stats_mode != 0;
+  return fast_rcnn_inference_impl(cls_logits, ld_cls, deltas, ld_delta, K, cls_agnostic, proposals, d_prop_count, B, R, d_image_sizes, wx,
+                                  wy, ww, wh, scale_clamp, score_thresh, nms_thresh, topk, max_candidates, d_post, out_boxes, out_scores,
+                                  out_classes, out_rows, d_out_count, d_status, workspace, workspace_bytes, stream,
+                                  handed ? st_mx : nullptr, handed ? st_inv : nullptr, handed ? st_cnt : nullptr,
+                                  handed ? st_mask : nullptr);
 }
 
 extern "C" int lvc_gather_detections(const float* boxes, const float* scores, const int* classes, const int* rows,
diff --git a/lvc_amd/csrc/conv_common.h b/lvc_amd/csrc/conv_common.h
--- a/lvc_amd/csrc/conv_common.h
+++ b/lvc_amd/csrc/conv_common.h
@@ -31,6 +31,9 @@
   *units_per_worker = (int)((units + workers - 1) / workers);
   *nworkers = (int)((units + *units_per_worker - 1) / *units_per_worker);
 }
+
+int lvc_pw_s1_presplit_x2(const void* x, const unsigned short* w_split, const float* scale, const float* shift, float* y, int M, int C,
+                          int K, int relu, int ldy, void* workspace, void* stream);
 
 #define LVC_ACT_SCALE 16.f
 #define LVC_ACT_MAX 4094.f
diff --git a/lvc_amd/csrc/conv_pw_s1.hip b/lvc_amd/csrc/conv_pw_s1.hip
--- a/lvc_amd/csrc/conv_pw_s1.hip
+++ b/lvc_amd/csrc/conv_pw_s1.hip
@@ -1,4 +1,5 @@
 #include "conv_common.h"
+#include "det_row_stats.h"
 #include <type_traits>
 #include <stdlib.h>
 
@@ -25,9 +26,12 @@
   long long pl_PS;
   int pl_N, pl_Npad, pl_H;
   float pl_qscale;
+  float* st_mx; float* st_inv; int* st_cnt; unsigned long long* st_mask;
+  int st_K;
+  float st_thresh;
 };
 
-template <int NI, bool ONEACC, bool PLANES = false, bool PRE = false>
+template <int NI, bool ONEACC, bool PLANES = false, bool PRE = false, bool STATS = false>
 __global__ __launch_bounds__(NT, 2) void conv_pw_s1_kernel(PwArgsS p) {
   constexpr int HN = 64 * NI;
   constexpr int PLANE_A = PM * AROW;
@@ -551,6 +555,7 @@
                   for (int e = 0; e < 4; ++e) o[e] = o[e] * 0.5f * (1.f + erff(o[e] * 0.70710678118654752440f));
                 }
                 *reinterpret_cast<f32x4*>(yb + (size_t)((g + i) * RPI) * p.ldy) = o;
+                if (STATS) *reinterpret_cast<f32x4*>(const_cast<float*>(cs) + (g + i) * RPI * CS_STRIDE) = o;
               }
             }
             if (RES) {
@@ -566,6 +571,13 @@
           if (p.relu == 1) rows(std::false_type{}, A1{}); else if (p.relu == 2) rows(std::false_type{}, A2{}); else rows(std::false_type{}, A0{});
         }
       }
+      if constexpr (STATS) {
+        if (n0 == 0) {
+          __syncthreads();
+          if (tid < PM && m0 + tid < p.M)
+            lvc_det_row_stats(Cs + tid * CS_STRIDE, p.st_K, p.st_thresh, (size_t)(m0 + tid), p.st_mx, p.st_inv, p.st_cnt, p.st_mask);
+        }
+      }
     }
     __syncthreads();
 #ifdef PW_TIMELINE
@@ -583,10 +595,12 @@
 }
 
 struct PwPlanes { unsigned short* planes; int* err; long long PS; int N, Npad, H; float qscale; };
+struct PwStats { float* mx; float* inv; int* cnt; unsigned long long* mask; int K; float thresh; };
 
 static int pw_s1_launch(bool oneacc, const float* x, const unsigned short* w_split, const float* scale, const float* shift,
                         const float* residual, float* y, int N, int H, int W, int C, int K, int stride, int relu, int res_mode,
-                        int ldy, int ldr, void* workspace, void* stream, const PwPlanes* pl = nullptr, bool pre = false) {
+                        int ldy, int ldr, void* workspace, void* stream, const PwPlanes* pl = nullptr, bool pre = false,
+                        const PwStats* stats = nullptr) {
   LVC_CHECK_ARG(x && w_split && y && workspace, "null pointer");
   LVC_CHECK_ARG(!oneacc || scale, "the single-accumulator form needs the row factors in `scale`");
   LVC_CHECK_ARG(N > 0 && H > 0 && W > 0 && C > 0 && K > 0 && stride >= 1, "non-positive dimension");
@@ -642,9 +656,20 @@
     LVC_CHECK_LAUNCH();
     return LVC_OK;
   }
+  a.st_mx = nullptr; a.st_inv = nullptr; a.st_cnt = nullptr; a.st_mask = nullptr; a.st_K = 0; a.st_thresh = 0.f;
   if (pre) {
-    LVC_CHECK_ARG(oneacc && ni == 2 && stride == 1, "pre-split input: the single-accumulator 128-column tile, stride 1");
-    hipLaunchKernelGGL((conv_pw_s1_kernel<2, true, false, true>), dim3(a.nworkers), dim3(NT), 0, st, a);
+    LVC_CHECK_ARG(ni == 2 && stride == 1, "pre-split input: the 128-column tile, stride 1");
+    if (oneacc) hipLaunchKernelGGL((conv_pw_s1_kernel<2, true, false, true>), dim3(a.nworkers), dim3(NT), 0, st, a);
+    else hipLaunchKernelGGL((conv_pw_s1_kernel<2, false, false, true>), dim3(a.nworkers), dim3(NT), 0, st, a);
+    LVC_CHECK_LAUNCH();
+    return LVC_OK;
+  }
+  if (stats) {
+    LVC_CHECK_ARG(!oneacc && ni == 2 && res_mode == 0 && relu == 0, "row statistics: the two-accumulator 128-column tile, no residual, no activation");
+    LVC_CHECK_ARG(stats->mx && stats->inv && stats->cnt && stats->mask, "null row statistics");
+    LVC_CHECK_ARG(stats->K > 0 && stats->K + 1 <= LVC_DET_STATS_MAX_COLS && stats->K + 1 <= K, "row statistics: 1 <= classes, classes + 1 <= min(128, K)");
+    a.st_mx = stats->mx; a.st_inv = stats->inv; a.st_cnt = stats->cnt; a.st_mask = stats->mask; a.st_K = stats->K; a.st_thresh = stats->thresh;
+    hipLaunchKernelGGL((conv_pw_s1_kernel<2, false, false, false, true>), dim3(a.nworkers), dim3(NT), 0, st, a);
     LVC_CHECK_LAUNCH();
     return LVC_OK;
   }
@@ -675,6 +700,19 @@
                                                 const float* residual, float* y, int N, int H, int W, int C, int K, int relu,
                                                 int res_mode, int ldy, int ldr, void* workspace, void* stream) {
   return pw_s1_launch(true, (const float*)x, w_split, scale, shift, residual, y, N, H, W, C, K, 1, relu, res_mode, ldy, ldr, workspace, stream, nullptr, true);
+}
+
+int lvc_pw_s1_presplit_x2(const void* x, const unsigned short* w_split, const float* scale, const float* shift, float* y, int M, int C,
+                          int K, int relu, int ldy, void* workspace, void* stream) {
+  return pw_s1_launch(false, (const float*)x, w_split, scale, shift, nullptr, y, M, 1, 1, C, K, 1, relu, 0, ldy, 0, workspace, stream, nullptr, true);
+}
+
+int lvc_pw_s1_rowstats(const float* x, const unsigned short* w_split, const float* scale, const float* shift, float* y, int M, int C, int K,
+                       int ldy, int num_classes, float score_thresh, float* st_mx, float* st_inv, int* st_cnt, unsigned long long* st_mask,
+                       void* workspace, void* stream) {
+  PwStats s;
+  s.mx = st_mx; s.inv = st_inv; s.cnt = st_cnt; s.mask = st_mask; s.K = num_classes; s.thresh = score_thresh;
+  return pw_s1_launch(false, x, w_split, scale, shift, nullptr, y, M, 1, 1, C, K, 1, 0, 0, ldy, 0, workspace, stream, nullptr, false, &s);
 }
 
 extern "C" int lvc_conv1x1_qkv_planes_f16s1(const float* x, const unsigned short* w_split, const float* scale, const float* shift, void* planes,
diff --git a/lvc_amd/csrc/det_row_stats.h b/lvc_amd/csrc/det_row_stats.h
--- /dev/null
+++ b/lvc_amd/csrc/det_row_stats.h
@@ -0,0 +1,28 @@
+#pragma once
+#include "common.h"
+
+#define LVC_DET_STATS_MAX_COLS 128
+
+__device__ __forceinline__ void lvc_det_row_stats(const float* lg, int K, float score_thresh, size_t r, float* __restrict__ st_mx,
+                                                  float* __restrict__ st_inv, int* __restrict__ st_cnt,
+                                                  unsigned long long* __restrict__ st_mask) {
+#pragma clang fp contract(off)
+  float mx = -INFINITY;
+  for (int k = 0; k <= K; ++k) { float v = lg[k]; mx = v > mx ? v : mx; }
+  float sum = 0.f;
+  for (int k = 0; k <= K; ++k) sum += expf(lg[k] - mx);
+  const float inv = 1.f / sum;
+  int cnt = 0;
+  unsigned long long m0 = 0, m1 = 0;
+  for (int k = 0; k < K; ++k) {
+    const bool hit = expf(lg[k] - mx) * inv > score_thresh;
+    cnt += hit ? 1 : 0;
+    if (hit) { if (k < 64) m0 |= 1ull << k; else m1 |= 1ull << (k - 64); }
+  }
+  st_mx[r] = mx; st_inv[r] = inv; st_cnt[r] = cnt;
+  st_mask[2 * r] = m0; st_mask[2 * r + 1] = m1;
+}
+
+int lvc_pw_s1_rowstats(const float* x, const unsigned short* w_split, const float* scale, const float* shift, float* y, int M, int C, int K,
+                       int ldy, int num_classes, float score_thresh, float* st_mx, float* st_inv, int* st_cnt, unsigned long long* st_mask,
+                       void* workspace, void* stream);
diff --git a/lvc_amd/csrc/roi_align.hip b/lvc_amd/csrc/roi_align.hip
--- a/lvc_amd/csrc/roi_align.hip
+++ b/lvc_amd/csrc/roi_align.hip
@@ -1,4 +1,5 @@
-#include "common.h"
+#include "conv_common.h"
+#include "roi_levels.h"
 #include <stdlib.h>
 #include <type_traits>
 
@@ -20,6 +21,8 @@
   long long so_k, so_c, so_h, so_w;
   int* status;
   const int* order;
+  int* range_flags;
+  int range_index;
 };
 
 __global__ __launch_bounds__(256) void roi_align_fwd_kernel(RoiAlignArgs p) {
@@ -175,7 +178,7 @@
 #ifndef ROI_WAVE_MLP
 #define ROI_WAVE_MLP 8
 #endif
-template <int PW>
+template <int PW, bool PLANES = false>
 __global__ __launch_bounds__(512) void roi_align_fwd_nhwc_wave_kernel(RoiAlignArgs p) {
   const int lane = threadIdx.x & 63;
   const int ph = ROI_UNI((int)(threadIdx.x >> 6));
@@ -212,6 +215,37 @@
   const bool c_ok = cbase + lane * 4 < p.C;
   const float* in = p.feat[lvl] + (long long)b * p.sb[lvl] + (c_ok ? cbase + lane * 4 : 0);
   float* outp = p.out + (long long)k * p.so_k + ph * p.so_h + cbase + lane * 4;
+  float big = 0.f;
+  auto put = [&](int pw, float4 o) {
+    if constexpr (!PLANES) {
+      if (c_ok) *reinterpret_cast<float4*>(outp + pw * p.so_w) = o;
+    } else {
+      const float a4[4] = {o.x, o.y, o.z, o.w};
+      f16x4 h, m;
+#pragma unroll
+      for (int e = 0; e < 4; ++e) {
+        const float a = a4[e];
+        f16 hh, mm;
+        split2h(a, hh, mm);
+        h[e] = hh; m[e] = mm;
+        big = fmaxf(big, fabsf(a));
+        if (a != a) big = INFINITY;
+      }
+      const uint2 hu = __builtin_bit_cast(uint2, h), mu = __builtin_bit_cast(uint2, m);
+      const bool odd = lane & 1;
+      const unsigned r0 = (unsigned)__builtin_amdgcn_mov_dpp((int)(odd ? hu.x : mu.x), 0xB1, 0xf, 0xf, false);
+      const unsigned r1 = (unsigned)__builtin_amdgcn_mov_dpp((int)(odd ? hu.y : mu.y), 0xB1, 0xf, 0xf, false);
+      const u32x4 v = odd ? u32x4{r0, r1, mu.x, mu.y} : u32x4{hu.x, hu.y, r0, r1};
+      const long long f = (long long)(ph * p.pw + pw) * p.C + cbase + (lane & ~1) * 4;
+      char* dst = reinterpret_cast<char*>(p.out + (long long)k * p.so_k) + (f >> 5) * 128 + (odd ? 64 : 0) + ((f & 31) >> 3) * 16;
+      if (c_ok) *reinterpret_cast<u32x4*>(dst) = v;
+    }
+  };
+  auto report = [&]() {
+    if constexpr (PLANES) {
+      if (c_ok) lvc_report_range(p.range_flags, p.range_index, big, LVC_F16_MAX);
+    }
+  };
 
   const float yf = roi_start_h + ph * bin_h, yl = roi_start_h + (ph + 1) * bin_h;
   const int y0 = ROI_UNI(min((int)floorf(fmaxf(yf, 0.f)), H - 1)), y1 = ROI_UNI(min((int)floorf(fmaxf(yl, 0.f)) + 1, H - 1));
@@ -246,8 +280,9 @@
           acc.w += w1 * v1.w + w2 * v2.w + w3 * v3.w + w4 * v4.w;
         }
       }
-      if (c_ok) *reinterpret_cast<float4*>(outp + pw * p.so_w) = float4{acc.x / count, acc.y / count, acc.z / count, acc.w / count};
-    }
+      put(pw, float4{acc.x / count, acc.y / count, acc.z / count, acc.w / count});
+    }
+    report();
     return;
   }
   float wy = 0.f;
@@ -333,12 +368,10 @@
   } else {
     for (int c0 = 0; c0 < ncols; c0 += 8) chunk(std::integral_constant<int, 8>{}, std::integral_constant<int, ROI_RB8>{}, c0);
   }
-  if (c_ok) {
-    const float inv = 1.f / count;
-#pragma unroll
-    for (int pw = 0; pw < PW; ++pw)
-      *reinterpret_cast<float4*>(outp + pw * p.so_w) = float4{acc[pw].x * inv, acc[pw].y * inv, acc[pw].z * inv, acc[pw].w * inv};
-  }
+  const float inv = 1.f / count;
+#pragma unroll
+  for (int pw = 0; pw < PW; ++pw) put(pw, float4{acc[pw].x * inv, acc[pw].y * inv, acc[pw].z * inv, acc[pw].w * inv});
+  report();
 }
 
 extern "C" int lvc_roi_align_route(int backward, int nhwc, int C, int pooled_h, int pooled_w, int has_num_valid,
@@ -355,6 +388,12 @@
   for (int l = 0; l < LVC_MAX_LEVELS; ++l)
     if (a.feat[l] && (long long)a.H[l] * a.W[l] * a.C > largest) largest = (long long)a.H[l] * a.W[l] * a.C;
   const int route = lvc_roi_align_route(0, a.nhwc && a.so_c == 1, a.C, a.ph, a.pw, a.num_valid != nullptr, largest);
+  if (a.range_flags) {
+    LVC_CHECK_ARG(route == 2 && a.ph == 7 && a.C % 32 == 0, "operand planes: NHWC, 7x7 bins, C % 32 == 0, levels below 2^31 elements");
+    hipLaunchKernelGGL((roi_align_fwd_nhwc_wave_kernel<7, true>), dim3(a.K, lvc_cdiv(a.C, 256)), dim3(64 * a.ph), 0, (hipStream_t)stream, a);
+    LVC_CHECK_LAUNCH();
+    return LVC_OK;
+  }
   if (route == 2) {
     hipLaunchKernelGGL(roi_align_fwd_nhwc_wave_kernel<7>, dim3(a.K, lvc_cdiv(a.C, 256)), dim3(64 * a.ph), 0, (hipStream_t)stream, a);
     LVC_CHECK_LAUNCH();
@@ -770,11 +809,81 @@
   return LVC_OK;
 }
 
+struct RoiLevelsOrderArgs {
+  const float* boxes;
+  int B, R, min_level, max_level;
+  float canonical_box_size, canonical_level;
+  int* levels;
+  float* rois;
+  int* order;
+};
+__global__ __launch_bounds__(1024) void roi_levels_order_xcd_kernel(RoiLevelsOrderArgs p) {
+  __shared__ int hist[ROI_XCD_MAX_B][256];
+  __shared__ int cnt[ROI_XCD_MAX_B], tail0[ROI_XCD_MAX_B], s_min;
+  const int tid = threadIdx.x;
+  const int K = p.B * p.R;
+  for (int i = tid; i < ROI_XCD_MAX_B * 256; i += 1024) (&hist[0][0])[i] = 0;
+  __syncthreads();
+  auto key = [&](float4 bx, int lvl) {
+    const float yc = (bx.y + bx.w) * 0.5f;
+    int band = yc == yc ? (int)(fminf(fmaxf(yc, 0.f), 1e6f) * (1.f / 16.f)) : 0;
+    band = band > 63 ? 63 : band;
+    return (lvl & 3) * 64 + band;
+  };
+  for (int k = tid; k < K; k += 1024) {
+    const float4 bx = *reinterpret_cast<const float4*>(p.boxes + (size_t)k * 4);
+    const int lvl = lvc_box_level(bx, p.min_level, p.max_level, p.canonical_box_size, p.canonical_level);
+    const int b = k / p.R;
+    p.levels[k] = lvl;
+    float* r = p.rois + (size_t)k * 5;
+    r[0] = (float)b; r[1] = bx.x; r[2] = bx.y; r[3] = bx.z; r[4] = bx.w;
+    atomicAdd(&hist[b][key(bx, lvl)], 1);
+  }
+  __syncthreads();
+  if (tid < p.B) {
+    int run = 0;
+    for (int i = 0; i < 256; ++i) { const int n = hist[tid][i]; hist[tid][i] = run; run += n; }
+    cnt[tid] = run;
+  }
+  __syncthreads();
+  if (tid == 0) {
+    int m = cnt[0];
+    for (int b = 1; b < p.B; ++b) m = cnt[b] < m ? cnt[b] : m;
+    s_min = m;
+    int run = 0;
+    for (int b = 0; b < p.B; ++b) { tail0[b] = run; run += cnt[b] - m; }
+  }
+  __syncthreads();
+  const int m = s_min;
+  for (int k = tid; k < K; k += 1024) {
+    const float4 bx = *reinterpret_cast<const float4*>(p.boxes + (size_t)k * 4);
+    const int lvl = lvc_box_level(bx, p.min_level, p.max_level, p.canonical_box_size, p.canonical_level);
+    const int b = k / p.R;
+    const int r = atomicAdd(&hist[b][key(bx, lvl)], 1);
+    p.order[r < m ? r * p.B + b : m * p.B + tail0[b] + (r - m)] = k;
+  }
+}
+
+int lvc_roi_levels_order_xcd(const float* boxes, int B, int R, int min_level, int max_level, int canonical_box_size, int canonical_level,
+                             int* levels, float* rois, int* d_order, void* stream) {
+  LVC_CHECK_ARG(B >= 1 && R >= 1 && B <= ROI_XCD_MAX_B, "the work order: 1..16 images");
+  LVC_CHECK_ARG(boxes && levels && rois && d_order, "null pointer");
+  LVC_CHECK_ARG(((uintptr_t)boxes & 15) == 0, "boxes must be 16-byte aligned");
+  RoiLevelsOrderArgs a;
+  a.boxes = boxes; a.B = B; a.R = R; a.min_level = min_level; a.max_level = max_level;
+  a.canonical_box_size = (float)canonical_box_size; a.canonical_level = (float)canonical_level;
+  a.levels = levels; a.rois = rois; a.order = d_order;
+  hipLaunchKernelGGL(roi_levels_order_xcd_kernel, dim3(1), dim3(1024), 0, (hipStream_t)stream, a);
+  LVC_CHECK_LAUNCH();
+  return LVC_OK;
+}
+
 static int roi_align_fpn_nhwc_impl(const float* const* feats, const int* Hs, const int* Ws,
                                       const float* scales, int L, int B, int C, const float* rois,
                                       const int* levels, const int* d_num_valid, int K, int pooled_h,
                                       int pooled_w, int sampling_ratio, int aligned, float* output,
-                                      int* d_status, const int* d_order, void* stream) {
+                                      int* d_status, const int* d_order, void* stream, int* range_flags = nullptr,
+                                      int range_index = 0) {
   LVC_CHECK_ARG(L >= 1 && L <= LVC_MAX_LEVELS, "1..8 levels");
   LVC_CHECK_ARG(K == 0 || (feats && Hs && Ws && scales && rois && output), "null pointer");
   LVC_CHECK_ARG(B > 0 && C > 0 && pooled_h > 0 && pooled_w > 0 && K >= 0, "bad shape");
@@ -792,6 +901,7 @@
   a.so_h = (long long)pooled_w * C; a.so_w = C;
   a.status = d_status;
   a.order = d_order;
+  a.range_flags = range_flags; a.range_index = range_index;
   return launch(a, stream);
 }
 
@@ -808,7 +918,24 @@
                                       const float* scales, int L, int B, int C, const float* rois,
                                       const int* levels, const int* d_num_valid, int K, int pooled_h,
                                       int pooled_w, int sampling_ratio, int aligned, float* output,
-                                      int* d_status, const int* d_order, void* stream) {
-  return roi_align_fpn_nhwc_impl(feats, Hs, Ws, scales, L, B, C, rois, levels, d_num_valid, K, pooled_h, pooled_w, sampling_ratio, aligned,
-                                 output, d_status, d_order, stream);
-}
+                                      int* d_status, const int* d_order, int planes_slot, const unsigned short* fc_w,
+                                      const float* fc_scale, const float* fc_shift, float* fc_y, int fc_K, int fc_relu,
+                                      void* workspace, void* stream) {
+  if (planes_slot < 0)
+    return roi_align_fpn_nhwc_impl(feats, Hs, Ws, scales, L, B, C, rois, levels, d_num_valid, K, pooled_h, pooled_w, sampling_ratio,
+                                   aligned, output, d_status, d_order, stream);
+  LVC_CHECK_ARG(workspace && planes_slot < lvc_range_slots(), "operand planes: the consumer's range slot and the conv workspace");
+  LVC_CHECK_ARG(!d_num_valid, "operand planes: no row count");
+  LVC_CHECK_ARG(((uintptr_t)output & 15) == 0, "planes must be 16-byte aligned");
+  LVC_CHECK_ARG(feats || fc_K > 0, "nothing to do");
+  if (feats) {
+    int rc = roi_align_fpn_nhwc_impl(feats, Hs, Ws, scales, L, B, C, rois, levels, nullptr, K, pooled_h, pooled_w, sampling_ratio, aligned,
+                                     output, d_status, d_order, stream, lvc_ws_flags(workspace), lvc_ws_range_index(planes_slot));
+    if (rc) return rc;
+  }
+  if (fc_K > 0 && K > 0) {
+    LVC_CHECK_ARG(C > 0 && pooled_h > 0 && pooled_w > 0 && (long long)pooled_h * pooled_w * C < (1ll << 31), "bad shape");
+    return lvc_pw_s1_presplit_x2(output, fc_w, fc_scale, fc_shift, fc_y, K, pooled_h * pooled_w * C, fc_K, fc_relu, fc_K, workspace, stream);
+  }
+  return LVC_OK;
+}
diff --git a/lvc_amd/csrc/roi_levels.h b/lvc_amd/csrc/roi_levels.h
--- /dev/null
+++ b/lvc_amd/csrc/roi_levels.h
@@ -0,0 +1,14 @@
+#pragma once
+#include "common.h"
+
+__device__ __forceinline__ int lvc_box_level(float4 bx, int min_level, int max_level, float canonical_box_size, float canonical_level) {
+  const float area = (bx.z - bx.x) * (bx.w - bx.y);
+  const float size = sqrtf(area);
+  float lvl = floorf(canonical_level + log2f(size / canonical_box_size + 1e-8f));
+  lvl = lvl < (float)min_level ? (float)min_level : lvl;
+  lvl = lvl > (float)max_level ? (float)max_level : lvl;
+  return (int)lvl - min_level;
+}
+
+int lvc_roi_levels_order_xcd(const float* boxes, int B, int R, int min_level, int max_level, int canonical_box_size, int canonical_level,
+                             int* levels, float* rois, int* d_order, void* stream);
diff --git a/lvc_amd/kernels.py b/lvc_amd/kernels.py
--- a/lvc_amd/kernels.py
+++ b/lvc_amd/kernels.py
@@ -1131,9 +1131,94 @@
     st = _lib.lib().lvc_roi_align_fpn_nhwc_ordered(
         fp, hs, ws, sc, L, B, C, ptr(rois), ptr(levels), ptr(num_valid), K,
         pooled_h, pooled_w, sampling_ratio, 1 if aligned else 0, ptr(out),
-        ptr(status), ptr(order), _stream(rois))
+        ptr(status), ptr(order), -1, ptr(None), ptr(None), ptr(None), ptr(None), 0, 0, ptr(None), _stream(rois))
     check(st, "lvc_roi_align_fpn_nhwc")
     return out
+
+
+BOX_PLANES = _os.environ.get("LVC_BOX_PLANES", "1") != "0"
+
+
+def box_planes_route(pc, rows, C, pooled_h, pooled_w, largest_level_elems, grad=False, first_is_fc=True, consumers=1, cascade=False):
+    if not BOX_PLANES or grad or cascade or not first_is_fc or pc is None or consumers != 1:
+        return "fp32"
+    if C % 32 != 0 or pc.C != pooled_h * pooled_w * C or pc.K <= 64 or rows < ROI_ORDER_MIN:
+        return "fp32"
+    if pc.state["tier"] >= 2 or conv_route(pc, rows, 1, 1).entry != "lvc_conv1x1_nhwc_f16x2_pipe":
+        return "fp32"
+    if not (C % 4 == 0 and pooled_h == 7 and pooled_w == 7 and largest_level_elems < (1 << 31)):
+        return "fp32"
+    return "planes"
+
+
+def assign_levels_rois_order(boxes, min_level, max_level, canonical_box_size=224, canonical_level=4):
+    _req_cuda(boxes)
+    B, R, _ = boxes.shape
+    boxes = boxes.contiguous()
+    levels = torch.empty(B * R, dtype=torch.int32, device=boxes.device)
+    rois = torch.empty(B * R, 5, dtype=torch.float32, device=boxes.device)
+    order = torch.empty(B * R, dtype=torch.int32, device=boxes.device)
+    rc = _lib.lib().lvc_assign_levels_rois(ptr(boxes), B, R, min_level, max_level, canonical_box_size, canonical_level,
+                                            ptr(levels), ptr(rois), ptr(order), _stream(boxes))
+    check(rc, "lvc_assign_levels_rois")
+    return levels, rois, order
+
+
+ROI_PLANES_LAUNCH = "lvc_roi_align_fpn_nhwc_ordered: operand planes"
+FC_PLANES_LAUNCH = "lvc_roi_align_fpn_nhwc_ordered: FC layer on the planes"
+PREDICTOR_STATS_LAUNCH = "lvc_fast_rcnn_inference: predictor with row statistics"
+
+
+def roi_align_fpn_nhwc_planes(feats, scales, rois, levels, pooled_h, pooled_w, sampling_ratio, aligned, slot, status=None,
+                              order=None, out=None):
+    _req_cuda(rois, *feats)
+    L = len(feats)
+    B, _, _, C = feats[0].shape
+    K = rois.shape[0]
+    rois = rois.contiguous().float()
+    if out is None:
+        out = torch.empty(K, pooled_h * pooled_w * C, device=rois.device, dtype=torch.float32)
+    assert out.numel() == K * pooled_h * pooled_w * C and out.is_contiguous() and out.dtype == torch.float32
+    for f in feats:
+        assert f.is_contiguous() and f.dtype == torch.float32 and f.shape[0] == B and f.shape[3] == C
+    if levels is not None:
+        assert levels.dtype == torch.int32 and levels.is_contiguous()
+    if order is not None:
+        assert order.dtype == torch.int32 and order.is_contiguous() and order.numel() == K
+    fp = (c_void_p * L)(*[f.data_ptr() for f in feats])
+    hs = (c_int * L)(*[f.shape[1] for f in feats])
+    ws = (c_int * L)(*[f.shape[2] for f in feats])
+    sc = (c_float * L)(*[float(s) for s in scales])
+    _launch(None, 0.0, 0.0, None, ROI_PLANES_LAUNCH, lambda: _lib.lib().lvc_roi_align_fpn_nhwc_ordered(
+        fp, hs, ws, sc, L, B, C, ptr(rois), ptr(levels), ptr(None), K, pooled_h, pooled_w, sampling_ratio, 1 if aligned else 0, ptr(out),
+        ptr(status), ptr(order), slot, ptr(None), ptr(None), ptr(None), ptr(None), 0, 0, ptr(conv_workspace(rois.device)), _stream(rois)))
+    return out
+
+
+def linear_presplit(planes, pc, relu=False):
+    M = planes.shape[0]
+    assert planes.is_contiguous() and planes.dtype == torch.float32 and planes.numel() == M * pc.C
+    y = torch.empty(M, pc.K, device=planes.device, dtype=torch.float32)
+    pc.last_one = False
+    _launch("f16x2_pws1", 2.0 * M * pc.K * pc.C, 4.0 * (M * pc.C + M * pc.K + pc.K * pc.C), pc.slot,
+            FC_PLANES_LAUNCH, lambda: _lib.lib().lvc_roi_align_fpn_nhwc_ordered(
+                ptr(None), ptr(None), ptr(None), ptr(None), 0, 0, pc.C, ptr(None), ptr(None), ptr(None), M, 1, 1, 0, 0, ptr(planes),
+                ptr(None), ptr(None), pc.slot, ptr(pc.split2h()), ptr(pc.scale), ptr(pc.shift), ptr(y), pc.K, 1 if relu else 0,
+                ptr(conv_workspace(planes.device)), _stream(planes)))
+    return y
+
+
+DET_STATS_MAX_CLASSES = 127
+
+
+def rowstats_route(pc, rows, num_classes, grad=False):
+    return (BOX_PLANES and not grad and 0 < num_classes <= DET_STATS_MAX_CLASSES and num_classes + 1 <= pc.K and pc.K > 64
+            and conv_route(pc, rows, 1, 1).entry == "lvc_conv1x1_nhwc_f16x2_pipe")
+
+
+def new_row_stats(rows, device):
+    return (torch.empty(rows, device=device), torch.empty(rows, device=device), torch.empty(rows, device=device, dtype=torch.int32),
+            torch.empty(rows, 2, device=device, dtype=torch.int64))
 
 
 def roi_align_backward(grad, rois, spatial_scale, pooled_h, pooled_w, batch_size, channels, height, width,
@@ -1269,18 +1354,37 @@
     levels = torch.empty(B * R, dtype=torch.int32, device=boxes.device)
     rois = torch.empty(B * R, 5, dtype=torch.float32, device=boxes.device)
     rc = _lib.lib().lvc_assign_levels_rois(ptr(boxes), B, R, min_level, max_level,
-                                           canonical_box_size, canonical_level, ptr(levels), ptr(rois),
+                                           canonical_box_size, canonical_level, ptr(levels), ptr(rois), ptr(None),
                                            _stream(boxes))
     check(rc, "lvc_assign_levels_rois")
     return levels, rois
 
 
 def fast_rcnn_inference(cls_logits, deltas, proposals, prop_count, image_sizes, num_classes, box_weights,
-                        score_thresh, nms_thresh, topk, post=None, status=None, max_candidates=16384):
+                        score_thresh, nms_thresh, topk, post=None, status=None, max_candidates=16384, stats=None, stats_out=None,
+                        predictor=None, logits_out=None):
     _req_cuda(cls_logits, deltas, proposals, prop_count, image_sizes, post)
     B, R, _ = proposals.shape
     K = num_classes
     dev = proposals.device
+    mode, st, px, pc = 0, (None, None, None, None), None, None
+    if predictor is not None:
+        assert cls_logits is None and deltas is None and stats is None
+        px, pc, nbox = predictor
+        _req_cuda(px)
+        assert px.shape == (B * R, pc.C) and px.is_contiguous() and px.dtype == torch.float32 and K + 1 + nbox <= pc.K
+        y = logits_out if logits_out is not None else torch.empty(B * R, pc.K, device=dev, dtype=torch.float32)
+        assert y.shape == (B * R, pc.K) and y.is_contiguous() and y.dtype == torch.float32
+        cls_logits, deltas = y[:, : K + 1], y[:, K + 1: K + 1 + nbox]
+        mode, st = 3, stats_out if stats_out is not None else new_row_stats(B * R, dev)
+    elif stats is not None:
+        mode, st = 2, stats
+    elif stats_out is not None:
+        mode, st = 1, stats_out
+    if mode:
+        mx, inv, scnt, mask = st
+        assert mx.numel() == B * R and inv.numel() == B * R and scnt.numel() == B * R and mask.numel() == 2 * B * R
+        assert scnt.dtype == torch.int32 and mask.dtype == torch.int64 and all(t.is_contiguous() and t.is_cuda for t in st)
     assert cls_logits.stride(1) == 1 and deltas.stride(1) == 1
     cls_agnostic = 1 if deltas.shape[1] == 4 else 0
     if status is None:
@@ -1295,13 +1399,24 @@
     orow = torch.empty(B, topk, device=dev, dtype=torch.int32)
     cnt = torch.empty(B, device=dev, dtype=torch.int32)
     wx, wy, ww, wh = box_weights
-    rc = lib.lvc_fast_rcnn_inference(
-        ptr(cls_logits), cls_logits.stride(0), ptr(deltas), deltas.stride(0), K,
-        cls_agnostic, ptr(proposals.contiguous()), ptr(prop_count), B, R, ptr(image_sizes),
-        wx, wy, ww, wh, SCALE_CLAMP, score_thresh,
-        nms_thresh, topk, max_candidates, ptr(post), ptr(ob), ptr(osc), ptr(ocl), ptr(orow),
-        ptr(cnt), ptr(status), ptr(ws), nbytes, _stream(proposals))
-    check(rc, "lvc_fast_rcnn_inference")
+    props = proposals.contiguous()
+
+    def call():
+        return lib.lvc_fast_rcnn_inference(
+            ptr(cls_logits), cls_logits.stride(0), ptr(deltas), deltas.stride(0), K,
+            cls_agnostic, ptr(props), ptr(prop_count), B, R, ptr(image_sizes),
+            wx, wy, ww, wh, SCALE_CLAMP, score_thresh,
+            nms_thresh, topk, max_candidates, ptr(post), ptr(ob), ptr(osc), ptr(ocl), ptr(orow),
+            ptr(cnt), ptr(status), ptr(ws), nbytes, mode, ptr(st[0]), ptr(st[1]), ptr(st[2]), ptr(st[3]), ptr(px),
+            ptr(pc.split2h() if pc is not None else None), ptr(pc.scale if pc is not None else None),
+            ptr(pc.shift if pc is not None else None), pc.C if pc is not None else 0, pc.K if pc is not None else 0,
+            ptr(conv_workspace(dev) if pc is not None else None), _stream(proposals))
+
+    if pc is not None:
+        pc.last_one = False
+        _launch(None, 0.0, 0.0, pc.slot, PREDICTOR_STATS_LAUNCH, call)
+    else:
+        check(call(), "lvc_fast_rcnn_inference")
     return ob, osc, ocl, orow, cnt
 
 
diff --git a/lvc_amd/modeling/poolers.py b/lvc_amd/modeling/poolers.py
--- a/lvc_amd/modeling/poolers.py
+++ b/lvc_amd/modeling/poolers.py
@@ -75,12 +75,25 @@
     def pool_nhwc(self, feats_nhwc, boxes, status=None):
         if torch.is_grad_enabled() and any(f.requires_grad for f in feats_nhwc):
             return _PoolAllLevels.apply(self, boxes.detach(), status, *feats_nhwc)
-        levels, rois = K.assign_levels_rois(boxes, self.min_level, self.max_level, self.canonical_box_size,
-                                            self.canonical_level)
+        levels, rois, order = self._levels_rois_order(boxes)
         if len(feats_nhwc) == 1:
             levels = None
         return K.roi_align_fpn_nhwc(feats_nhwc, self.scales, rois, levels, self.output_size[0], self.output_size[1],
-                                    self.sampling_ratio, self.aligned, status=status)
+                                    self.sampling_ratio, self.aligned, status=status, order=order)
+
+    def _levels_rois_order(self, boxes):
+        B, R, _ = boxes.shape
+        if K.BOX_PLANES and B <= 16 and B * R >= K.ROI_ORDER_MIN:
+            return K.assign_levels_rois_order(boxes, self.min_level, self.max_level, self.canonical_box_size, self.canonical_level)
+        levels, rois = K.assign_levels_rois(boxes, self.min_level, self.max_level, self.canonical_box_size, self.canonical_level)
+        return levels, rois, None
+
+    def pool_planes_nhwc(self, feats_nhwc, boxes, slot, status=None):
+        levels, rois, order = self._levels_rois_order(boxes)
+        if len(feats_nhwc) == 1:
+            levels = None
+        return K.roi_align_fpn_nhwc_planes(feats_nhwc, self.scales, rois, levels, self.output_size[0], self.output_size[1],
+                                           self.sampling_ratio, self.aligned, slot, status=status, order=order)
 
     def pool_rois_nhwc(self, feats_nhwc, rois, levels, num_valid=None, status=None):
         if torch.is_grad_enabled() and any(f.requires_grad for f in feats_nhwc):
diff --git a/lvc_amd/modeling/roi_heads/box_head.py b/lvc_amd/modeling/roi_heads/box_head.py
--- a/lvc_amd/modeling/roi_heads/box_head.py
+++ b/lvc_amd/modeling/roi_heads/box_head.py
@@ -52,6 +52,15 @@
 
         return self._fc1_hwc.get([fc.weight, fc.bias], build)
 
+    def first_fc_packed(self):
+        return self._packed_fc1_hwc() if len(self.fcs) and not self.conv_norm_relus else None
+
+    def forward_planes(self, planes):
+        x = self.dropout(K.linear_presplit(planes, self._packed_fc1_hwc(), relu=True))
+        for fc in self.fcs[1:]:
+            x = self.dropout(fc(x, relu=True))
+        return x
+
     def forward_nhwc(self, x):
         if self.conv_norm_relus and x.shape[0] == 0:
             size = self._output_size if isinstance(self._output_size, int) else int(np.prod(self._output_size))
diff --git a/lvc_amd/modeling/roi_heads/fast_rcnn.py b/lvc_amd/modeling/roi_heads/fast_rcnn.py
--- a/lvc_amd/modeling/roi_heads/fast_rcnn.py
+++ b/lvc_amd/modeling/roi_heads/fast_rcnn.py
@@ -40,9 +40,7 @@
             nn.init.constant_(l.bias, 0)
         self._fused = _PackedCache()
 
-    def forward(self, x):
-        if x.dim() > 2:
-            x = torch.flatten(x, start_dim=1)
+    def fused_packed(self):
         c, b = self.cls_score, self.bbox_pred
         def build():
             w = torch.cat([c.weight, b.weight], 0)
@@ -53,7 +51,19 @@
                 bias = torch.cat([bias, bias.new_zeros(padk)], 0)
             return K.pack_linear(w, bias)
 
-        y = K.linear(x.contiguous(), self._fused.get([c.weight, c.bias, b.weight, b.bias], build))
+        return self._fused.get([c.weight, c.bias, b.weight, b.bias], build)
+
+    def inference_predictor(self, x):
+        pc = self.fused_packed()
+        grad = torch.is_grad_enabled() and (x.requires_grad or any(p.requires_grad for p in self.parameters()))
+        if x.dim() == 2 and K.rowstats_route(pc, x.shape[0], self.num_classes, grad=grad):
+            return x.contiguous(), pc, self.num_bbox_reg_classes * 4
+        return None
+
+    def forward(self, x):
+        if x.dim() > 2:
+            x = torch.flatten(x, start_dim=1)
+        y = K.linear(x.contiguous(), self.fused_packed())
         k1 = self.num_classes + 1
         return y[:, :k1], y[:, k1:k1 + self.num_bbox_reg_classes * 4]
 
diff --git a/lvc_amd/modeling/roi_heads/roi_heads.py b/lvc_amd/modeling/roi_heads/roi_heads.py
--- a/lvc_amd/modeling/roi_heads/roi_heads.py
+++ b/lvc_amd/modeling/roi_heads/roi_heads.py
@@ -359,13 +359,21 @@
         if self.reg_off:
             raise NotImplementedError("ROI_HEADS.REG_OFF is not used by the shipped configs")
         feats = [feats_nhwc[f] for f in self.in_features]
-        pooled = self.box_pooler.pool_nhwc(feats, prop_boxes, status=status)
-        h = self.box_head.forward_nhwc(pooled)
-        scores, deltas = self.box_predictor(h)
+        head, pl = self.box_head, self.box_pooler
+        pc1 = head.first_fc_packed() if hasattr(head, "first_fc_packed") else None
+        grad = torch.is_grad_enabled() and (any(f.requires_grad for f in feats) or any(p.requires_grad for p in head.parameters()))
+        C = feats[0].shape[3]
+        if K.box_planes_route(pc1, prop_boxes.shape[0] * prop_boxes.shape[1], C, pl.output_size[0], pl.output_size[1],
+                              max(f.shape[1] * f.shape[2] * C for f in feats), grad=grad, first_is_fc=pc1 is not None) == "planes":
+            h = head.forward_planes(pl.pool_planes_nhwc(feats, prop_boxes, pc1.slot, status=status))
+        else:
+            h = head.forward_nhwc(pl.pool_nhwc(feats, prop_boxes, status=status))
+        pred = self.box_predictor.inference_predictor(h) if hasattr(self.box_predictor, "inference_predictor") else None
+        scores, deltas = (None, None) if pred is not None else self.box_predictor(h)
         return K.fast_rcnn_inference(scores, deltas, prop_boxes, prop_count, image_sizes_dev, self.num_classes,
                                      self.box2box_transform.weights, self.test_score_thresh, self.test_nms_thresh,
                                      self.test_detections_per_img, post=post, status=status,
-                                     max_candidates=self.det_max_candidates)
+                                     max_candidates=self.det_max_candidates, predictor=pred)
 
     def forward(self, images, features, proposals, targets=None):
         if self.training:
```

Measured after the change: 661.1 img/s. About the same (-0.0%).
